# gkm2708/gym-lmaze

Measured on AMD Instinct MI355X. Metric: env steps/sec (whole node), 1M parallel 11x11 mazes at 1/2/4/8 MI355X, higher is better.
Workload: dtype int32

## Files before the change

### gym-lmaze_amd/_abi.py

```python
import ctypes as C
import os

import torch

HERE = os.path.dirname(os.path.abspath(__file__))
LIB_PATH = os.environ.get("LMAZE_HIP_LIB") or os.path.join(HERE, "liblmaze_hip.so")

ABI_VERSION = 4
VARIANT_V0, VARIANT_V3 = 0, 3
VARIANT_V1, VARIANT_V2, VARIANT_V4, VARIANT_V5, VARIANT_V6 = 1, 2, 4, 5, 6
FOVEA = 5
LAYOUT_SHARED, LAYOUT_PER_ENV = 0, 1
OBS_BALL, OBS_WALL, OBS_GOAL, OBS_FREE = 1, 2, 4, 8
MAX_GRID, MAX_CHANNELS = 64, 8

SYMBOLS = ("lmaze_abi_version", "lmaze_strerror", "lmaze_device_info", "lmaze_step_v0", "lmaze_step_v3",
           "lmaze_step_v0_autoreset", "lmaze_step_v3_autoreset", "lmaze_observe", "lmaze_reset",
           "lmaze_episode_stats", "lmaze_bandwidth_probe", "lmaze_render_expanded", "lmaze_foveal_step", "lmaze_foveal_step_autoreset", "lmaze_foveal_reset", "lmaze_v1_set_foveal_goal",
           "lmaze_v5_planner_step", "lmaze_v5_hier_step", "lmaze_v6_safe_foveal_goal", "lmaze_expand_planes",
           "lmaze_foveal_visit_bytes", "lmaze_foveal_materialise_visit", "lmaze_foveal_load_visit",
           "lmaze_describe_step", "lmaze_describe_foveal_step", "lmaze_rollout",
           "lmaze_step_u8", "lmaze_observe_u8", "lmaze_foveal_rollout", "lmaze_describe_foveal_rollout",
           "lmaze_rollout_obs", "lmaze_foveal_rollout_obs", "lmaze_rollout_u8", "lmaze_rollout_obs_u8",
           "lmaze_describe_rollout", "lmaze_rollout_policy", "lmaze_rollout_policy_u8", "lmaze_describe_rollout_policy",
           "lmaze_rollout_sample", "lmaze_rollout_sample_u8", "lmaze_describe_rollout_sample", "lmaze_returns",
           "lmaze_describe_foveal_rollout_obs")


class LmazeParams(C.Structure):
    _fields_ = [("variant", C.c_int32), ("grid", C.c_int32), ("layout_mode", C.c_int32),
                ("step_limit", C.c_int32), ("reward_wall", C.c_float), ("reward_move", C.c_float),
                ("reward_goal", C.c_float), ("launch_hint", C.c_int32)]


class LmazeFovealParams(C.Structure):
    _fields_ = [("variant", C.c_int32), ("grid", C.c_int32), ("n_layouts", C.c_int32), ("step_limit", C.c_int32),
                ("foveal_step_limit", C.c_int32), ("reward_wall", C.c_float), ("reward_move", C.c_float),
                ("reward_goal", C.c_float), ("launch_hint", C.c_int32)]


FOVEAL_BUFFER_FIELDS = ("ball_xy", "goal_xy", "fgoal_xy", "layout_id", "step_count", "foveal_step_count",
                        "reward", "foveal_reward", "done", "foveal_done", "visit", "obs",
                        "ball1_xy", "fovea_xy", "last_xy", "foveal_goal", "obs_local", "visit_clock")


class LmazeFovealBuffers(C.Structure):
    _fields_ = [(n, C.c_void_p) for n in FOVEAL_BUFFER_FIELDS]


class LmazeError(RuntimeError):
    def __init__(self, fn, code):
        self.code = code
        RuntimeError.__init__(self, "%s failed: %d (%s)" % (fn, code, strerror(code)))


def _sources():
    src = os.path.join(HERE, "csrc")
    out = [os.path.join(src, f) for f in sorted(os.listdir(src)) if f.endswith((".hip", ".h"))] if os.path.isdir(src) else []
    hdr = os.path.join(os.path.dirname(HERE), "include", "lmaze.h")
    return out + ([hdr] if os.path.exists(hdr) else [])


def _load():
    if not os.path.exists(LIB_PATH):
        raise ImportError(
            "gym-lmaze_amd: %s is missing. The HIP library is the only compute path (no CPU fallback); "
            "build it with `make -C %s` (hipcc, --offload-arch=gfx950) or `python -c 'import __graft_entry__ as g; "
            "g.build()'`." % (LIB_PATH, os.path.join(HERE, "csrc")))
    if "LMAZE_HIP_LIB" not in os.environ:
        stale = [f for f in _sources() if os.path.getmtime(f) > os.path.getmtime(LIB_PATH)]
        if stale:
            import warnings
            warnings.warn("gym-lmaze_amd: %s is older than %s -- rebuild with `make -C %s`"
                          % (os.path.basename(LIB_PATH), ", ".join(os.path.basename(f) for f in stale),
                             os.path.join(HERE, "csrc")), RuntimeWarning, stacklevel=3)
    lib = C.CDLL(LIB_PATH)
    vp, i32, i64, u64 = C.c_void_p, C.c_int32, C.c_int64, C.c_uint64
    P = C.POINTER(LmazeParams)
    lib.lmaze_abi_version.restype = C.c_int
    lib.lmaze_abi_version.argtypes = []
    lib.lmaze_strerror.restype = C.c_char_p
    lib.lmaze_strerror.argtypes = [C.c_int]
    lib.lmaze_device_info.restype = C.c_int
    lib.lmaze_device_info.argtypes = [C.c_int, C.POINTER(i32), C.c_char_p, i32]
    lib.lmaze_step_v0.restype = C.c_int
    lib.lmaze_step_v0.argtypes = [P, vp, vp, vp, vp, vp, vp, vp, vp, i64, vp]
    lib.lmaze_step_v3.restype = C.c_int
    lib.lmaze_step_v3.argtypes = [P, vp, vp, vp, vp, vp, vp, vp, vp, i64, vp]
    lib.lmaze_step_v0_autoreset.restype = C.c_int
    lib.lmaze_step_v0_autoreset.argtypes = [P, vp, vp, vp, vp, vp, vp, vp, vp, i64, u64, u64, i64, vp, vp, vp]
    lib.lmaze_step_v3_autoreset.restype = C.c_int
    lib.lmaze_step_v3_autoreset.argtypes = [P, vp, vp, vp, vp, vp, vp, vp, vp, i64, u64, u64, i64, vp, vp, vp]
    lib.lmaze_observe.restype = C.c_int
    lib.lmaze_observe.argtypes = [P, vp, vp, vp, vp, i64, vp]
    lib.lmaze_reset.restype = C.c_int
    lib.lmaze_reset.argtypes = [P, vp, vp, u64, u64, i64, vp, vp, vp, vp, vp, vp, i64, vp]
    lib.lmaze_render_expanded.restype = C.c_int
    lib.lmaze_render_expanded.argtypes = [vp, i32, i32, C.POINTER(i32), i32, vp, i64, vp]
    lib.lmaze_bandwidth_probe.restype = C.c_int
    lib.lmaze_bandwidth_probe.argtypes = [vp, vp, i64, vp]
    lib.lmaze_episode_stats.restype = C.c_int
    lib.lmaze_episode_stats.argtypes = [vp, vp, vp, vp, C.c_float, i64, vp, vp]
    FP, FB = C.POINTER(LmazeFovealParams), C.POINTER(LmazeFovealBuffers)
    lib.lmaze_foveal_step.restype = C.c_int
    lib.lmaze_foveal_step.argtypes = [FP, vp, vp, FB, i64, vp]
    lib.lmaze_foveal_step_autoreset.restype = C.c_int
    lib.lmaze_foveal_step_autoreset.argtypes = [FP, vp, vp, FB, i64, u64, u64, i64, vp, vp, vp]
    lib.lmaze_foveal_reset.restype = C.c_int
    lib.lmaze_foveal_reset.argtypes = [FP, vp, vp, i32, u64, u64, i64, FB, i64, vp]
    lib.lmaze_v1_set_foveal_goal.restype = C.c_int
    lib.lmaze_v1_set_foveal_goal.argtypes = [FP, vp, vp, vp, FB, i64, vp]
    lib.lmaze_v5_planner_step.restype = C.c_int
    lib.lmaze_v5_planner_step.argtypes = [FP, vp, vp, vp, FB, i64, vp]
    lib.lmaze_v5_hier_step.restype = C.c_int
    lib.lmaze_v5_hier_step.argtypes = [FP, vp, vp, vp, FB, i64, u64, u64, i64, vp, vp, vp]
    lib.lmaze_v6_safe_foveal_goal.restype = C.c_int
    lib.lmaze_v6_safe_foveal_goal.argtypes = [FP, vp, u64, u64, i64, FB, vp, i64, vp]
    lib.lmaze_expand_planes.restype = C.c_int
    lib.lmaze_expand_planes.argtypes = [vp, i32, i32, i32, vp, i64, vp]
    lib.lmaze_foveal_visit_bytes.restype = i64
    lib.lmaze_foveal_visit_bytes.argtypes = [i32, i64]
    lib.lmaze_foveal_materialise_visit.restype = C.c_int
    lib.lmaze_foveal_materialise_visit.argtypes = [FP, FB, vp, i64, vp]
    lib.lmaze_foveal_load_visit.restype = C.c_int
    lib.lmaze_foveal_load_visit.argtypes = [FP, FB, vp, i64, vp]
    lib.lmaze_step_u8.restype = C.c_int
    lib.lmaze_step_u8.argtypes = [P, vp, vp, vp, vp, vp, vp, vp, vp, vp, i64, i32, u64, u64, i64, vp, vp, vp]
    lib.lmaze_observe_u8.restype = C.c_int
    lib.lmaze_observe_u8.argtypes = [P, vp, vp, vp, vp, vp, i64, vp]
    lib.lmaze_rollout.restype = C.c_int
    lib.lmaze_rollout.argtypes = [P, vp, vp, i32, vp, vp, vp, vp, vp, vp, vp, vp, vp, i64, i32, u64, u64, i64, vp]
    lib.lmaze_describe_step.restype = C.c_int
    lib.lmaze_describe_step.argtypes = [P, i64, i32, i32, C.c_char_p, i32]
    lib.lmaze_describe_foveal_step.restype = C.c_int
    lib.lmaze_describe_foveal_step.argtypes = [FP, i64, i32, C.c_char_p, i32]
    lib.lmaze_foveal_rollout.restype = C.c_int
    lib.lmaze_foveal_rollout.argtypes = [FP, vp, vp, vp, i32, FB, i64, i32, u64, u64, i64, vp, vp, vp, vp, vp]
    lib.lmaze_rollout_obs.restype = C.c_int
    lib.lmaze_rollout_obs.argtypes = [P, vp, vp, i32, vp, vp, vp, vp, vp, vp, vp, vp, vp, i64, i32, u64, u64, i64, vp, i32, vp]
    lib.lmaze_foveal_rollout_obs.restype = C.c_int
    lib.lmaze_foveal_rollout_obs.argtypes = [FP, vp, vp, vp, i32, FB, i64, i32, u64, u64, i64, vp, vp, vp, vp, vp, vp, i32, vp]
    lib.lmaze_rollout_u8.restype = C.c_int
    lib.lmaze_rollout_u8.argtypes = [P, vp, vp, i32, vp, vp, vp, vp, vp, vp, vp, vp, vp, i64, i32, u64, u64, i64, vp]
    lib.lmaze_rollout_obs_u8.restype = C.c_int
    lib.lmaze_rollout_obs_u8.argtypes = [P, vp, vp, i32, vp, vp, vp, vp, vp, vp, vp, vp, vp, i64, i32, u64, u64, i64, vp, i32, vp]
    lib.lmaze_describe_rollout.restype = C.c_int
    lib.lmaze_describe_rollout.argtypes = [P, i64, i32, i32, i32, i32, C.c_char_p, i32]
    for name in ("lmaze_rollout_policy", "lmaze_rollout_policy_u8"):
        getattr(lib, name).restype = C.c_int
        getattr(lib, name).argtypes = [P, vp, vp, i32, C.c_uint32, i32, vp, vp, vp, vp, vp, vp, vp, vp, vp, vp, vp, i64, i32, u64, u64,
                                       i64, vp, i32, vp]
    lib.lmaze_describe_rollout_policy.restype = C.c_int
    lib.lmaze_describe_rollout_policy.argtypes = [P, i64, i32, i32, i32, i32, i32, C.c_char_p, i32]
    for name in ("lmaze_rollout_sample", "lmaze_rollout_sample_u8"):
        getattr(lib, name).restype = C.c_int
        getattr(lib, name).argtypes = [P, vp, vp, i32, i32, vp, vp, vp, vp, vp, vp, vp, vp, vp, vp, vp, i64, i32, u64, u64, i64, vp, i32, vp]
    lib.lmaze_describe_rollout_sample.restype = C.c_int
    lib.lmaze_describe_rollout_sample.argtypes = [P, i64, i32, i32, i32, i32, i32, C.c_char_p, i32]
    lib.lmaze_returns.restype = C.c_int
    lib.lmaze_returns.argtypes = [vp, vp, vp, C.c_float, vp, i32, i64, vp]
    lib.lmaze_describe_foveal_rollout.restype = C.c_int
    lib.lmaze_describe_foveal_rollout.argtypes = [FP, i64, i32, i32, i32, C.c_char_p, i32]
    lib.lmaze_describe_foveal_rollout_obs.restype = C.c_int
    lib.lmaze_describe_foveal_rollout_obs.argtypes = [FP, i64, i32, i32, i32, i32, C.c_char_p, i32]
    if lib.lmaze_abi_version() != ABI_VERSION:
        raise ImportError("liblmaze_hip.so ABI %d != binding %d: rebuild" % (lib.lmaze_abi_version(), ABI_VERSION))
    return lib


lib = _load()


def strerror(code):
    return lib.lmaze_strerror(int(code)).decode("ascii", "replace")


def check(fn, code):
    if code != 0:
        raise LmazeError(fn, code)


def device_info(device=0):
    cu = C.c_int32(0)
    name = C.create_string_buffer(64)
    check("lmaze_device_info", lib.lmaze_device_info(int(device), C.byref(cu), name, 64))
    return {"cu_count": cu.value, "arch": name.value.decode("ascii", "replace")}


def describe_step(params, n, auto_reset=False, with_obs=True):
    buf = C.create_string_buffer(256)
    check("lmaze_describe_step", lib.lmaze_describe_step(C.byref(params), int(n), 1 if auto_reset else 0,
                                                         2 if with_obs == "u8" else (1 if with_obs else 0), buf, 256))
    return buf.value.decode("ascii", "replace")


def describe_rollout(params, n, T, auto_reset=False, with_obs=True, obs_every=None):
    buf = C.create_string_buffer(256)
    check("lmaze_describe_rollout", lib.lmaze_describe_rollout(C.byref(params), int(n), int(T), 1 if auto_reset else 0,
                                                               2 if with_obs == "u8" else (1 if with_obs else 0),
                                                               -1 if obs_every is None else int(obs_every), buf, 256))
    return buf.value.decode("ascii", "replace")


def describe_foveal_step(params, n, auto_reset=False):
    buf = C.create_string_buffer(256)
    check("lmaze_describe_foveal_step", lib.lmaze_describe_foveal_step(C.byref(params), int(n), 1 if auto_reset else 0, buf, 256))
    return buf.value.decode("ascii", "replace")


KEY_MODES = {"ball": 0, "goal": 1}


def epsilon_u32(epsilon):
    eps = float(epsilon)
    if not 0.0 <= eps <= 1.0:
        raise ValueError("epsilon must be in [0, 1]")
    return min(int(eps * 4294967296.0), 4294967295)


def describe_rollout_policy(params, n, T, auto_reset=True, with_obs=True, obs_every=0, key="ball"):
    buf = C.create_string_buffer(256)
    check("lmaze_describe_rollout_policy",
          lib.lmaze_describe_rollout_policy(C.byref(params), int(n), int(T), 1 if auto_reset else 0,
                                            2 if with_obs == "u8" else (1 if with_obs else 0), int(obs_every),
                                            KEY_MODES[key] if key in KEY_MODES else int(key), buf, 256))
    return buf.value.decode("ascii", "replace")


def describe_rollout_sample(params, n, T, auto_reset=True, with_obs=True, obs_every=0, key="ball"):
    buf = C.create_string_buffer(256)
    check("lmaze_describe_rollout_sample",
          lib.lmaze_describe_rollout_sample(C.byref(params), int(n), int(T), 1 if auto_reset else 0,
                                            2 if with_obs == "u8" else (1 if with_obs else 0), int(obs_every),
                                            KEY_MODES[key] if key in KEY_MODES else int(key), buf, 256))
    return buf.value.decode("ascii", "replace")


def sampling_thresholds(probs):
    if not (isinstance(probs, torch.Tensor) and probs.dim() == 2 and probs.shape[1] == 4 and probs.is_floating_point()):
        raise ValueError("probs must be a float tensor [S, 4]")
    p = probs.detach().to(torch.float64)
    if not bool(torch.isfinite(p).all()) or bool((p < 0).any()):
        raise ValueError("probs must be finite and non-negative")
    a0 = p[:, 0]
    a1 = a0 + p[:, 1]
    a2 = a1 + p[:, 2]
    s = a2 + p[:, 3]
    if not bool(torch.isfinite(s).all()) or bool((s <= 0).any()):
        raise ValueError("every row of probs must have a positive, finite sum")
    c = torch.stack([torch.floor(a / s * 4294967296.0 + 0.5) for a in (a0, a1, a2)] + [torch.zeros_like(s)], dim=1)
    c = c.clamp_(max=4294967295.0).to(torch.int64)
    return torch.where(c >= 2147483648, c - 4294967296, c).to(torch.int32).view(torch.uint32)


def describe_foveal_rollout(params, n, T, auto_reset=False, two_level=False, obs_every=None):
    buf = C.create_string_buffer(256)
    if obs_every is None:
        check("lmaze_describe_foveal_rollout", lib.lmaze_describe_foveal_rollout(C.byref(params), int(n), int(T),
                                                                                 1 if auto_reset else 0, 1 if two_level else 0,
                                                                                 buf, 256))
    else:
        check("lmaze_describe_foveal_rollout_obs",
              lib.lmaze_describe_foveal_rollout_obs(C.byref(params), int(n), int(T), 1 if auto_reset else 0,
                                                    1 if two_level else 0, int(obs_every), buf, 256))
    return buf.value.decode("ascii", "replace")


def make_params(variant, grid, layout_mode, step_limit, reward_wall, reward_move, reward_goal):
    return LmazeParams(int(variant), int(grid), int(layout_mode), int(step_limit), float(reward_wall),
                       float(reward_move), float(reward_goal), 0)
```

### gym-lmaze_amd/csrc/lmaze_abi.hip

```cpp
#include <stdio.h>
#include <string.h>

#include "lmaze_common.h"


using namespace lmaze;

static int check_params(const LmazeParams* p, int64_t n) {
    if (!p) return LMAZE_E_NULL;
    if (p->grid < 3 || p->grid > LMAZE_MAX_GRID) return LMAZE_E_GRID;
    if (p->layout_mode != LMAZE_LAYOUT_SHARED && p->layout_mode != LMAZE_LAYOUT_PER_ENV) return LMAZE_E_LAYOUT;
    if (n < 0 || n > LMAZE_MAX_ENVS) return LMAZE_E_COUNT;
    return 0;
}

static bool misaligned(const void* p, uintptr_t a) { return ((uintptr_t)p & (a - 1)) != 0; }

static StepArgs make_args(const LmazeParams* p, const uint8_t* layout, const int32_t* action, int32_t* ball_xy,
                          const int32_t* goal_xy, int32_t* step_count, float* reward, uint8_t* done,
                          int32_t* goal_count, int32_t* obs, int64_t n) {
    StepArgs a;
    a.layout = layout;
    a.action = action;
    a.ball = reinterpret_cast<int2*>(ball_xy);
    a.goal = reinterpret_cast<const int2*>(goal_xy);
    a.step_count = step_count;
    a.reward = reward;
    a.done = done;
    a.goal_count = goal_count;
    a.obs = obs;
    a.obs8 = nullptr;
    a.n = n;
    a.grid = p->grid;
    a.step_limit = p->step_limit;
    a.reward_wall = p->reward_wall;
    a.reward_move = p->reward_move;
    a.reward_goal = p->reward_goal;
    a.envs_per_block = 0;
    a.auto_reset = 0;
    a.seed = 0;
    a.epoch = 0;
    a.env_base = 0;
    a.epoch_in = nullptr;
    a.epoch_out = nullptr;
    a.goal_rw = nullptr;
    a.mask = nullptr;
    a.launch_hint = p->launch_hint;
    a.info = nullptr;
    return a;
}

namespace lmaze {
void describe_launch(LaunchInfo* info, const char* kernel, int epb, int per_cu, int chunks, bool nt, int64_t grid, int block, size_t lds) {
    snprintf(info->kernel, sizeof(info->kernel), "%s", kernel);
    info->envs_per_workgroup = epb;
    info->workgroups_per_cu = per_cu;
    info->chunks = chunks;
    info->non_temporal = nt ? 1 : 0;
    info->grid = grid;
    info->block = block;
    info->lds = (int64_t)lds;
}
}

static int format_launch(const LaunchInfo& i, char* text, int32_t len) {
    if (!text || len < 1) return LMAZE_E_NULL;
    snprintf(text, (size_t)len, "%s grid=%lld block=%d lds=%lld envs_per_workgroup=%d workgroups_per_cu=%d chunks=%d", i.kernel,
             (long long)i.grid, i.block, (long long)i.lds, i.envs_per_workgroup, i.workgroups_per_cu, i.chunks);
    return 0;
}

static int check_recording(int32_t T, const void* slots, int32_t every) {
    if (every < 0 || (every == 0 && slots)) return LMAZE_E_COUNT;
    if (every > 0 && T / every > 0 && !slots) return LMAZE_E_NULL;
    if (misaligned(slots, 16)) return LMAZE_E_ALIGN;
    return 0;
}

static RolloutRec recording(int32_t T, void* slots, int32_t every) {
    return RolloutRec{every > 0 && T / every > 0 ? slots : nullptr, every};
}

static StepArgs rollout_args(const LmazeParams* p, const uint8_t* layout, const int32_t* actions, int32_t* ball_xy, int32_t* goal_xy,
                             int32_t* step_count, float* reward, uint8_t* done, int32_t* goal_count, void* obs, bool u8, int64_t n,
                             int32_t auto_reset, uint64_t seed, uint64_t epoch, int64_t env_base) {
    const bool v3 = p->variant == LMAZE_VARIANT_V3;
    StepArgs a = make_args(p, layout, actions, ball_xy, v3 ? goal_xy : nullptr, step_count, reward, done, v3 ? nullptr : goal_count,
                           u8 ? nullptr : static_cast<int32_t*>(obs), n);
    a.obs8 = u8 ? static_cast<uint8_t*>(obs) : nullptr;
    a.auto_reset = auto_reset ? 1 : 0;
    a.seed = seed;
    a.epoch = epoch;
    a.env_base = env_base;
    a.goal_rw = v3 ? reinterpret_cast<int2*>(goal_xy) : nullptr;
    return a;
}

static int grid_rollout(const LmazeParams* params, const uint8_t* layout, const int32_t* actions, int32_t T, int32_t* ball_xy,
                        int32_t* goal_xy, int32_t* step_count, float* reward, uint8_t* done, int32_t* goal_count, void* obs, bool u8,
                        float* reward_t, uint8_t* done_t, int64_t n, int32_t auto_reset, uint64_t seed, uint64_t epoch,
                        int64_t env_base, const RolloutRec* rec, void* stream) {
    int rc = check_params(params, n);
    if (rc) return rc;
    const bool v3 = params->variant == LMAZE_VARIANT_V3;
    if (params->variant != LMAZE_VARIANT_V0 && !v3) return LMAZE_E_VARIANT;
    if (u8 && params->layout_mode != LMAZE_LAYOUT_SHARED) return LMAZE_E_LAYOUT;
    if (u8 && params->grid < 4) return LMAZE_E_GRID;
    if (T < 0) return LMAZE_E_COUNT;
    if (T == 0 || n == 0) return 0;
    if (!layout || !actions || !ball_xy || !step_count || !reward || !done || (v3 && !goal_xy)) return LMAZE_E_NULL;
    if (misaligned(ball_xy, 8) || misaligned(goal_xy, 8) || misaligned(obs, 16) || (!u8 && misaligned(layout, 16))) return LMAZE_E_ALIGN;
    const StepArgs a = rollout_args(params, layout, actions, ball_xy, goal_xy, step_count, reward, done, goal_count, obs, u8, n,
                                    auto_reset, seed, epoch, env_base);
    return (int)launch_rollout(params->variant, a, params->layout_mode, actions, T, reward_t, done_t, (hipStream_t)stream, rec, u8);
}

static int check_closed_loop(const LmazeParams* params, const uint8_t* layout, const void* table, uintptr_t table_align,
                             int32_t key_mode, int32_t T, const int32_t* ball_xy, const int32_t* goal_xy, const int32_t* step_count,
                             const float* reward, const uint8_t* done, const void* obs, bool u8, int64_t n, bool describing, bool* go) {
    *go = false;
    int rc = check_params(params, n);
    if (rc) return rc;
    const bool v3 = params->variant == LMAZE_VARIANT_V3;
    if (params->variant != LMAZE_VARIANT_V0 && !v3) return LMAZE_E_VARIANT;
    if (u8 && params->layout_mode != LMAZE_LAYOUT_SHARED) return LMAZE_E_LAYOUT;
    if (u8 && params->grid < 4) return LMAZE_E_GRID;
    if (T < 0) return LMAZE_E_COUNT;
    if (key_mode != 0 && key_mode != 1) return LMAZE_E_COUNT;
    if (key_mode == 1 && !v3) return LMAZE_E_VARIANT;
    if (T == 0 || n == 0) return 0;
    if (!describing) {
        if (!layout || !table || !ball_xy || !step_count || !reward || !done || (v3 && !goal_xy)) return LMAZE_E_NULL;
        if (misaligned(ball_xy, 8) || misaligned(goal_xy, 8) || misaligned(obs, 16) || (!u8 && misaligned(layout, 16)) ||
            misaligned(table, table_align))
            return LMAZE_E_ALIGN;
    }
    *go = true;
    return 0;
}

static int grid_rollout_policy(const LmazeParams* params, const uint8_t* layout, const RolloutPolicy& pol, int32_t T, int32_t* ball_xy,
                               int32_t* goal_xy, int32_t* step_count, float* reward, uint8_t* done, int32_t* goal_count, void* obs,
                               bool u8, float* reward_t, uint8_t* done_t, int64_t n, int32_t auto_reset, uint64_t seed,
                               uint64_t epoch, int64_t env_base, const RolloutRec& rec, LaunchInfo* info, void* stream) {
    bool go;
    const int rc = check_closed_loop(params, layout, pol.table, 1, pol.key_mode, T, ball_xy, goal_xy, step_count, reward, done, obs, u8,
                                     n, info != nullptr, &go);
    if (!go) return rc;
    StepArgs a = rollout_args(params, layout, nullptr, ball_xy, goal_xy, step_count, reward, done, goal_count, obs, u8, n, auto_reset,
                              seed, epoch, env_base);
    a.info = info;
    return (int)launch_rollout_policy(params->variant, a, params->layout_mode, pol, T, reward_t, done_t, (hipStream_t)stream, rec, u8);
}

static int grid_rollout_sample(const LmazeParams* params, const uint8_t* layout, const RolloutSample& smp, int32_t T, int32_t* ball_xy,
                               int32_t* goal_xy, int32_t* step_count, float* reward, uint8_t* done, int32_t* goal_count, void* obs,
                               bool u8, float* reward_t, uint8_t* done_t, int64_t n, int32_t auto_reset, uint64_t seed,
                               uint64_t epoch, int64_t env_base, const RolloutRec& rec, LaunchInfo* info, void* stream) {
    bool go;
    const int rc = check_closed_loop(params, layout, smp.thresholds, 16, smp.key_mode, T, ball_xy, goal_xy, step_count, reward, done, obs,
                                     u8, n, info != nullptr, &go);
    if (!go) return rc;
    StepArgs a = rollout_args(params, layout, nullptr, ball_xy, goal_xy, step_count, reward, done, goal_count, obs, u8, n, auto_reset,
                              seed, epoch, env_base);
    a.info = info;
    return (int)launch_rollout_sample(params->variant, a, params->layout_mode, smp, T, reward_t, done_t, (hipStream_t)stream, rec, u8);
}

extern "C" {

int lmaze_abi_version(void) { return LMAZE_ABI_VERSION; }

const char* lmaze_strerror(int code) {
    switch (code) {
        case 0: return "ok";
        case LMAZE_E_NULL: return "a required pointer is NULL";
        case LMAZE_E_GRID: return "grid outside [3, 64]";
        case LMAZE_E_VARIANT: return "params.variant does not match the entry point";
        case LMAZE_E_LAYOUT: return "unknown layout_mode";
        case LMAZE_E_COUNT: return "env count out of range";
        case LMAZE_E_ALIGN: return "buffer not aligned as documented";
        case LMAZE_E_EXPANSION: return "expansion ratio / channel count out of range";
        case LMAZE_E_NODEVICE: return "no usable HIP device";
        default: return code > 0 ? hipGetErrorString((hipError_t)code) : "unknown lmaze error";
    }
}

int lmaze_device_info(int device, int32_t* cu_count_host, char* name_host, int32_t name_len) {
    int count = 0;
    if (hipGetDeviceCount(&count) != hipSuccess || count <= 0 || device < 0 || device >= count) {
        (void)hipGetLastError();
        return LMAZE_E_NODEVICE;
    }
    hipDeviceProp_t prop;
    if (hipGetDeviceProperties(&prop, device) != hipSuccess) return LMAZE_E_NODEVICE;
    if (cu_count_host) *cu_count_host = prop.multiProcessorCount;
    if (name_host && name_len > 0) {
        strncpy(name_host, prop.gcnArchName, (size_t)name_len - 1);
        name_host[name_len - 1] = 0;
    }
    return 0;
}

int lmaze_describe_step(const LmazeParams* params, int64_t n, int32_t auto_reset, int32_t with_obs, char* text_host,
                        int32_t len) {
    int rc = check_params(params, n);
    if (rc) return rc;
    if (params->variant != LMAZE_VARIANT_V0 && params->variant != LMAZE_VARIANT_V3) return LMAZE_E_VARIANT;
    if (!text_host || len < 1) return LMAZE_E_NULL;
    text_host[0] = 0;
    if (n == 0) return 0;
    LaunchInfo info;
    memset(&info, 0, sizeof(info));
    StepArgs a = make_args(params, nullptr, nullptr, nullptr, nullptr, nullptr, nullptr, nullptr, nullptr,
                           with_obs ? reinterpret_cast<int32_t*>(16) : nullptr, n);
    a.auto_reset = auto_reset ? 1 : 0;
    a.info = &info;
    if (with_obs == 2) {
        if (params->layout_mode != LMAZE_LAYOUT_SHARED) return LMAZE_E_LAYOUT;
        if (params->grid < 4) return LMAZE_E_GRID;
        a.obs = nullptr;
        a.obs8 = reinterpret_cast<uint8_t*>(16);
        rc = (int)launch_step_u8(params->variant, true, a, nullptr);
        if (rc) return rc;
        return format_launch(info, text_host, len);
    }
    rc = (int)launch_step(params->variant, true, a, params->layout_mode, nullptr);
    if (rc) return rc;
    return format_launch(info, text_host, len);
}

int lmaze_step_v0(const LmazeParams* params, const uint8_t* layout, const int32_t* action, int32_t* ball_xy,
                  int32_t* step_count, float* reward, uint8_t* done, int32_t* goal_count, int32_t* obs,
                  int64_t n, void* stream) {
    int rc = check_params(params, n);
    if (rc) return rc;
    if (params->variant != LMAZE_VARIANT_V0) return LMAZE_E_VARIANT;
    if (!layout || !action || !ball_xy || !step_count || !reward || !done) return LMAZE_E_NULL;
    if (misaligned(ball_xy, 8) || misaligned(obs, 16) || misaligned(layout, 16)) return LMAZE_E_ALIGN;
    StepArgs a = make_args(params, layout, action, ball_xy, nullptr, step_count, reward, done, goal_count, obs, n);
    return (int)launch_step(LMAZE_VARIANT_V0, true, a, params->layout_mode, (hipStream_t)stream);
}

int lmaze_step_v3(const LmazeParams* params, const uint8_t* layout, const int32_t* action, int32_t* ball_xy,
                  const int32_t* goal_xy, int32_t* step_count, float* reward, uint8_t* done, int32_t* obs,
                  int64_t n, void* stream) {
    int rc = check_params(params, n);
    if (rc) return rc;
    if (params->variant != LMAZE_VARIANT_V3) return LMAZE_E_VARIANT;
    if (!layout || !action || !ball_xy || !goal_xy || !step_count || !reward || !done) return LMAZE_E_NULL;
    if (misaligned(ball_xy, 8) || misaligned(goal_xy, 8) || misaligned(obs, 16) || misaligned(layout, 16))
        return LMAZE_E_ALIGN;
    StepArgs a = make_args(params, layout, action, ball_xy, goal_xy, step_count, reward, done, nullptr, obs, n);
    return (int)launch_step(LMAZE_VARIANT_V3, true, a, params->layout_mode, (hipStream_t)stream);
}

int lmaze_step_v0_autoreset(const LmazeParams* params, const uint8_t* layout, const int32_t* action,
                            int32_t* ball_xy, int32_t* step_count, float* reward, uint8_t* done,
                            int32_t* goal_count, int32_t* obs, int64_t n, uint64_t seed, uint64_t epoch,
                            int64_t env_base, const uint64_t* epoch_in_dev, uint64_t* epoch_out_dev, void* stream) {
    int rc = check_params(params, n);
    if (rc) return rc;
    if (params->variant != LMAZE_VARIANT_V0) return LMAZE_E_VARIANT;
    if (!layout || !action || !ball_xy || !step_count || !reward || !done) return LMAZE_E_NULL;
    if (misaligned(ball_xy, 8) || misaligned(obs, 16) || misaligned(layout, 16)) return LMAZE_E_ALIGN;
    StepArgs a = make_args(params, layout, action, ball_xy, nullptr, step_count, reward, done, goal_count, obs, n);
    if (bad_epoch_words(epoch_in_dev, epoch_out_dev)) return LMAZE_E_ALIGN;
    a.auto_reset = 1;
    a.seed = seed;
    a.epoch = epoch;
    a.env_base = env_base;
    a.epoch_in = epoch_in_dev;
    a.epoch_out = epoch_out_dev;
    return (int)launch_step(LMAZE_VARIANT_V0, true, a, params->layout_mode, (hipStream_t)stream);
}

int lmaze_step_u8(const LmazeParams* params, const uint8_t* layout, const int32_t* action, int32_t* ball_xy, int32_t* goal_xy,
                  int32_t* step_count, float* reward, uint8_t* done, int32_t* goal_count, uint8_t* obs8, int64_t n,
                  int32_t auto_reset, uint64_t seed, uint64_t epoch, int64_t env_base, const uint64_t* epoch_in_dev,
                  uint64_t* epoch_out_dev, void* stream) {
    int rc = check_params(params, n);
    if (rc) return rc;
    const bool v3 = params->variant == LMAZE_VARIANT_V3;
    if (params->variant != LMAZE_VARIANT_V0 && !v3) return LMAZE_E_VARIANT;
    if (params->layout_mode != LMAZE_LAYOUT_SHARED) return LMAZE_E_LAYOUT;
    if (params->grid < 4) return LMAZE_E_GRID;
    if (!layout || !action || !ball_xy || !step_count || !reward || !done || (v3 && !goal_xy)) return LMAZE_E_NULL;
    if (misaligned(ball_xy, 8) || misaligned(goal_xy, 8) || misaligned(obs8, 16)) return LMAZE_E_ALIGN;
    if (bad_epoch_words(epoch_in_dev, epoch_out_dev)) return LMAZE_E_ALIGN;
    StepArgs a = make_args(params, layout, action, ball_xy, v3 ? goal_xy : nullptr, step_count, reward, done, v3 ? nullptr : goal_count, nullptr, n);
    a.obs8 = obs8;
    a.auto_reset = auto_reset ? 1 : 0;
    a.seed = seed;
    a.epoch = epoch;
    a.env_base = env_base;
    a.epoch_in = epoch_in_dev;
    a.epoch_out = epoch_out_dev;
    a.goal_rw = v3 ? reinterpret_cast<int2*>(goal_xy) : nullptr;
    return (int)launch_step_u8(params->variant, true, a, (hipStream_t)stream);
}

int lmaze_observe_u8(const LmazeParams* params, const uint8_t* layout, const int32_t* ball_xy, const int32_t* goal_xy,
                     const uint8_t* mask, uint8_t* obs8, int64_t n, void* stream) {
    int rc = check_params(params, n);
    if (rc) return rc;
    const bool v3 = params->variant == LMAZE_VARIANT_V3;
    if (params->variant != LMAZE_VARIANT_V0 && !v3) return LMAZE_E_VARIANT;
    if (params->layout_mode != LMAZE_LAYOUT_SHARED) return LMAZE_E_LAYOUT;
    if (params->grid < 4) return LMAZE_E_GRID;
    if (!layout || !ball_xy || !obs8 || (v3 && !goal_xy)) return LMAZE_E_NULL;
    if (misaligned(ball_xy, 8) || misaligned(goal_xy, 8) || misaligned(obs8, 16)) return LMAZE_E_ALIGN;
    StepArgs a = make_args(params, layout, nullptr, const_cast<int32_t*>(ball_xy), v3 ? goal_xy : nullptr, nullptr, nullptr, nullptr,
                           nullptr, nullptr, n);
    a.obs8 = obs8;
    a.mask = mask;
    return (int)launch_step_u8(params->variant, false, a, (hipStream_t)stream);
}

int lmaze_rollout(const LmazeParams* params, const uint8_t* layout, const int32_t* actions, int32_t T, int32_t* ball_xy,
                  int32_t* goal_xy, int32_t* step_count, float* reward, uint8_t* done, int32_t* goal_count, int32_t* obs,
                  float* reward_t, uint8_t* done_t, int64_t n, int32_t auto_reset, uint64_t seed, uint64_t epoch,
                  int64_t env_base, void* stream) {
    return grid_rollout(params, layout, actions, T, ball_xy, goal_xy, step_count, reward, done, goal_count, obs, false, reward_t,
                        done_t, n, auto_reset, seed, epoch, env_base, nullptr, stream);
}

int lmaze_rollout_obs(const LmazeParams* params, const uint8_t* layout, const int32_t* actions, int32_t T, int32_t* ball_xy,
                      int32_t* goal_xy, int32_t* step_count, float* reward, uint8_t* done, int32_t* goal_count, int32_t* obs,
                      float* reward_t, uint8_t* done_t, int64_t n, int32_t auto_reset, uint64_t seed, uint64_t epoch,
                      int64_t env_base, int32_t* obs_t, int32_t obs_every, void* stream) {
    const int rc = check_recording(T, obs_t, obs_every);
    const RolloutRec rec = recording(T, obs_t, obs_every);
    return rc ? rc : grid_rollout(params, layout, actions, T, ball_xy, goal_xy, step_count, reward, done, goal_count, obs, false,
                                  reward_t, done_t, n, auto_reset, seed, epoch, env_base, &rec, stream);
}

int lmaze_rollout_u8(const LmazeParams* params, const uint8_t* layout, const int32_t* actions, int32_t T, int32_t* ball_xy,
                     int32_t* goal_xy, int32_t* step_count, float* reward, uint8_t* done, int32_t* goal_count, uint8_t* obs8,
                     float* reward_t, uint8_t* done_t, int64_t n, int32_t auto_reset, uint64_t seed, uint64_t epoch,
                     int64_t env_base, void* stream) {
    return grid_rollout(params, layout, actions, T, ball_xy, goal_xy, step_count, reward, done, goal_count, obs8, true, reward_t,
                        done_t, n, auto_reset, seed, epoch, env_base, nullptr, stream);
}

int lmaze_rollout_obs_u8(const LmazeParams* params, const uint8_t* layout, const int32_t* actions, int32_t T, int32_t* ball_xy,
                         int32_t* goal_xy, int32_t* step_count, float* reward, uint8_t* done, int32_t* goal_count, uint8_t* obs8,
                         float* reward_t, uint8_t* done_t, int64_t n, int32_t auto_reset, uint64_t seed, uint64_t epoch,
                         int64_t env_base, uint8_t* obs_t8, int32_t obs_every, void* stream) {
    const int rc = check_recording(T, obs_t8, obs_every);
    const RolloutRec rec = recording(T, obs_t8, obs_every);
    return rc ? rc : grid_rollout(params, layout, actions, T, ball_xy, goal_xy, step_count, reward, done, goal_count, obs8, true,
                                  reward_t, done_t, n, auto_reset, seed, epoch, env_base, &rec, stream);
}

int lmaze_rollout_policy(const LmazeParams* params, const uint8_t* layout, const uint8_t* policy, int32_t key_mode,
                         uint32_t epsilon_u32, int32_t T, int32_t* ball_xy, int32_t* goal_xy, int32_t* step_count, float* reward,
                         uint8_t* done, int32_t* goal_count, int32_t* obs, float* reward_t, uint8_t* done_t, int32_t* actions_t,
                         int32_t* key_t, int64_t n, int32_t auto_reset, uint64_t seed, uint64_t epoch, int64_t env_base,
                         int32_t* obs_t, int32_t obs_every, void* stream) {
    const int rc = check_recording(T, obs_t, obs_every);
    const RolloutPolicy pol{policy, key_mode, epsilon_u32, actions_t, key_t};
    return rc ? rc : grid_rollout_policy(params, layout, pol, T, ball_xy, goal_xy, step_count, reward, done, goal_count, obs, false,
                                         reward_t, done_t, n, auto_reset, seed, epoch, env_base, recording(T, obs_t, obs_every),
                                         nullptr, stream);
}

int lmaze_rollout_policy_u8(const LmazeParams* params, const uint8_t* layout, const uint8_t* policy, int32_t key_mode,
                            uint32_t epsilon_u32, int32_t T, int32_t* ball_xy, int32_t* goal_xy, int32_t* step_count, float* reward,
                            uint8_t* done, int32_t* goal_count, uint8_t* obs8, float* reward_t, uint8_t* done_t, int32_t* actions_t,
                            int32_t* key_t, int64_t n, int32_t auto_reset, uint64_t seed, uint64_t epoch, int64_t env_base,
                            uint8_t* obs_t8, int32_t obs_every, void* stream) {
    const int rc = check_recording(T, obs_t8, obs_every);
    const RolloutPolicy pol{policy, key_mode, epsilon_u32, actions_t, key_t};
    return rc ? rc : grid_rollout_policy(params, layout, pol, T, ball_xy, goal_xy, step_count, reward, done, goal_count, obs8, true,
                                         reward_t, done_t, n, auto_reset, seed, epoch, env_base, recording(T, obs_t8, obs_every),
                                         nullptr, stream);
}

int lmaze_describe_rollout_policy(const LmazeParams* params, int64_t n, int32_t T, int32_t auto_reset, int32_t with_obs,
                                  int32_t obs_every, int32_t key_mode, char* text_host, int32_t len) {
    if (obs_every < 0) return LMAZE_E_COUNT;
    if (!text_host || len < 1) return LMAZE_E_NULL;
    text_host[0] = 0;
    const bool u8 = with_obs == 2;
    LaunchInfo info;
    memset(&info, 0, sizeof(info));
    const RolloutPolicy pol{nullptr, key_mode, 0, nullptr, nullptr};
    const int rc = grid_rollout_policy(params, nullptr, pol, T, nullptr, nullptr, nullptr, nullptr, nullptr, nullptr,
                                       with_obs == 1 || u8 ? reinterpret_cast<void*>(16) : nullptr, u8, nullptr, nullptr, n, auto_reset,
                                       0, 0, 0, recording(T, reinterpret_cast<void*>(32), obs_every), &info, nullptr);
    if (rc || n == 0 || T == 0) return rc;
    return format_launch(info, text_host, len);
}

int lmaze_rollout_sample(const LmazeParams* params, const uint8_t* layout, const uint32_t* thresholds, int32_t key_mode, int32_t T,
                         int32_t* ball_xy, int32_t* goal_xy, int32_t* step_count, float* reward, uint8_t* done, int32_t* goal_count,
                         int32_t* obs, float* reward_t, uint8_t* done_t, int32_t* actions_t, int32_t* key_t, int64_t n,
                         int32_t auto_reset, uint64_t seed, uint64_t epoch, int64_t env_base, int32_t* obs_t, int32_t obs_every,
                         void* stream) {
    const int rc = check_recording(T, obs_t, obs_every);
    const RolloutSample smp{thresholds, key_mode, actions_t, key_t};
    return rc ? rc : grid_rollout_sample(params, layout, smp, T, ball_xy, goal_xy, step_count, reward, done, goal_count, obs, false,
                                         reward_t, done_t, n, auto_reset, seed, epoch, env_base, recording(T, obs_t, obs_every),
                                         nullptr, stream);
}

int lmaze_rollout_sample_u8(const LmazeParams* params, const uint8_t* layout, const uint32_t* thresholds, int32_t key_mode, int32_t T,
                            int32_t* ball_xy, int32_t* goal_xy, int32_t* step_count, float* reward, uint8_t* done,
                            int32_t* goal_count, uint8_t* obs8, float* reward_t, uint8_t* done_t, int32_t* actions_t, int32_t* key_t,
                            int64_t n, int32_t auto_reset, uint64_t seed, uint64_t epoch, int64_t env_base, uint8_t* obs_t8,
                            int32_t obs_every, void* stream) {
    const int rc = check_recording(T, obs_t8, obs_every);
    const RolloutSample smp{thresholds, key_mode, actions_t, key_t};
    return rc ? rc : grid_rollout_sample(params, layout, smp, T, ball_xy, goal_xy, step_count, reward, done, goal_count, obs8, true,
                                         reward_t, done_t, n, auto_reset, seed, epoch, env_base, recording(T, obs_t8, obs_every),
                                         nullptr, stream);
}

int lmaze_describe_rollout_sample(const LmazeParams* params, int64_t n, int32_t T, int32_t auto_reset, int32_t with_obs,
                                  int32_t obs_every, int32_t key_mode, char* text_host, int32_t len) {
    if (obs_every < 0) return LMAZE_E_COUNT;
    if (!text_host || len < 1) return LMAZE_E_NULL;
    text_host[0] = 0;
    const bool u8 = with_obs == 2;
    LaunchInfo info;
    memset(&info, 0, sizeof(info));
    const RolloutSample smp{nullptr, key_mode, nullptr, nullptr};
    const int rc = grid_rollout_sample(params, nullptr, smp, T, nullptr, nullptr, nullptr, nullptr, nullptr, nullptr,
                                       with_obs == 1 || u8 ? reinterpret_cast<void*>(16) : nullptr, u8, nullptr, nullptr, n, auto_reset,
                                       0, 0, 0, recording(T, reinterpret_cast<void*>(32), obs_every), &info, nullptr);
    if (rc || n == 0 || T == 0) return rc;
    return format_launch(info, text_host, len);
}

int lmaze_returns(const float* reward_t, const uint8_t* done_t, const float* tail, float gamma, float* returns_t, int32_t T,
                  int64_t n, void* stream) {
    if (!reward_t || !done_t || !returns_t) return LMAZE_E_NULL;
    if (T < 0 || n < 0 || n > LMAZE_MAX_ENVS) return LMAZE_E_COUNT;
    return (int)launch_returns(reward_t, done_t, tail, gamma, returns_t, T, n, (hipStream_t)stream);
}

int lmaze_describe_rollout(const LmazeParams* params, int64_t n, int32_t T, int32_t auto_reset, int32_t with_obs, int32_t obs_every,
                           char* text_host, int32_t len) {
    int rc = check_params(params, n);
    if (rc) return rc;
    if (params->variant != LMAZE_VARIANT_V0 && params->variant != LMAZE_VARIANT_V3) return LMAZE_E_VARIANT;
    if (T < 0) return LMAZE_E_COUNT;
    if (!text_host || len < 1) return LMAZE_E_NULL;
    text_host[0] = 0;
    if (n == 0 || T == 0) return 0;
    const bool u8 = with_obs == 2;
    if (u8 && params->layout_mode != LMAZE_LAYOUT_SHARED) return LMAZE_E_LAYOUT;
    if (u8 && params->grid < 4) return LMAZE_E_GRID;
    LaunchInfo info;
    memset(&info, 0, sizeof(info));
    StepArgs a = rollout_args(params, nullptr, nullptr, nullptr, nullptr, nullptr, nullptr, nullptr, nullptr,
                              with_obs == 1 || u8 ? reinterpret_cast<void*>(16) : nullptr, u8, n, auto_reset, 0, 0, 0);
    a.info = &info;
    const RolloutRec rec = recording(T, reinterpret_cast<void*>(32), obs_every);
    rc = (int)launch_rollout(params->variant, a, params->layout_mode, nullptr, T, nullptr, nullptr, nullptr,
                             obs_every >= 0 ? &rec : nullptr, u8);
    if (rc) return rc;
    return format_launch(info, text_host, len);
}

int lmaze_step_v3_autoreset(const LmazeParams* params, const uint8_t* layout, const int32_t* action,
                            int32_t* ball_xy, int32_t* goal_xy, int32_t* step_count, float* reward,
                            uint8_t* done, int32_t* obs, int64_t n, uint64_t seed, uint64_t epoch,
                            int64_t env_base, const uint64_t* epoch_in_dev, uint64_t* epoch_out_dev, void* stream) {
    int rc = check_params(params, n);
    if (rc) return rc;
    if (params->variant != LMAZE_VARIANT_V3) return LMAZE_E_VARIANT;
    if (!layout || !action || !ball_xy || !goal_xy || !step_count || !reward || !done) return LMAZE_E_NULL;
    if (misaligned(ball_xy, 8) || misaligned(goal_xy, 8) || misaligned(obs, 16) || misaligned(layout, 16))
        return LMAZE_E_ALIGN;
    StepArgs a = make_args(params, layout, action, ball_xy, goal_xy, step_count, reward, done, nullptr, obs, n);
    if (bad_epoch_words(epoch_in_dev, epoch_out_dev)) return LMAZE_E_ALIGN;
    a.auto_reset = 1;
    a.seed = seed;
    a.epoch = epoch;
    a.env_base = env_base;
    a.epoch_in = epoch_in_dev;
    a.epoch_out = epoch_out_dev;
    a.goal_rw = reinterpret_cast<int2*>(goal_xy);
    return (int)launch_step(LMAZE_VARIANT_V3, true, a, params->layout_mode, (hipStream_t)stream);
}

int lmaze_observe(const LmazeParams* params, const uint8_t* layout, const int32_t* ball_xy,
                  const int32_t* goal_xy, int32_t* obs, int64_t n, void* stream) {
    int rc = check_params(params, n);
    if (rc) return rc;
    if (params->variant != LMAZE_VARIANT_V0 && params->variant != LMAZE_VARIANT_V3) return LMAZE_E_VARIANT;
    if (!layout || !ball_xy || !obs) return LMAZE_E_NULL;
    if (params->variant == LMAZE_VARIANT_V3 && !goal_xy) return LMAZE_E_NULL;
    if (misaligned(ball_xy, 8) || misaligned(goal_xy, 8) || misaligned(obs, 16) || misaligned(layout, 16))
        return LMAZE_E_ALIGN;
    StepArgs a = make_args(params, layout, nullptr, const_cast<int32_t*>(ball_xy), goal_xy, nullptr, nullptr,
                           nullptr, nullptr, obs, n);
    return (int)launch_step(params->variant, false, a, params->layout_mode, (hipStream_t)stream);
}

int lmaze_reset(const LmazeParams* params, const uint8_t* layout, const uint8_t* mask, uint64_t seed,
                uint64_t epoch, int64_t env_base, int32_t* ball_xy, int32_t* goal_xy, int32_t* step_count, float* reward,
                uint8_t* done, int32_t* obs, int64_t n, void* stream) {
    int rc = check_params(params, n);
    if (rc) return rc;
    if (params->variant != LMAZE_VARIANT_V0 && params->variant != LMAZE_VARIANT_V3) return LMAZE_E_VARIANT;
    if (!layout || !ball_xy || !step_count || !reward || !done) return LMAZE_E_NULL;
    if (params->variant == LMAZE_VARIANT_V3 && !goal_xy) return LMAZE_E_NULL;
    if (misaligned(ball_xy, 8) || misaligned(goal_xy, 8) || misaligned(obs, 16) || misaligned(layout, 16))
        return LMAZE_E_ALIGN;
    ResetArgs r;
    r.layout = layout;
    r.mask = mask;
    r.ball = reinterpret_cast<int2*>(ball_xy);
    r.goal = reinterpret_cast<int2*>(goal_xy);
    r.step_count = step_count;
    r.reward = reward;
    r.done = done;
    r.n = n;
    r.seed = seed;
    r.epoch = epoch;
    r.env_base = env_base;
    r.grid = params->grid;
    hipError_t e = launch_reset(params->variant, r, params->layout_mode, (hipStream_t)stream);
    if (e != hipSuccess || !obs) return (int)e;
    StepArgs a = make_args(params, layout, nullptr, ball_xy, goal_xy, nullptr, nullptr, nullptr, nullptr, obs, n);
    a.mask = mask;
    return (int)launch_step(params->variant, false, a, params->layout_mode, (hipStream_t)stream);
}

int lmaze_episode_stats(const uint8_t* done, const float* reward, const int32_t* step_count,
                        const int32_t* goal_count, float reward_goal, int64_t n, int64_t* out4, void* stream) {
    if (!done || !reward || !step_count || !out4) return LMAZE_E_NULL;
    if (n < 0 || n > LMAZE_MAX_ENVS) return LMAZE_E_COUNT;
    if (misaligned(out4, 8)) return LMAZE_E_ALIGN;
    return (int)launch_episode_stats(done, reward, step_count, goal_count, reward_goal, n, out4, (hipStream_t)stream);
}

int lmaze_bandwidth_probe(const void* src, void* dst, int64_t bytes, void* stream) {
    if (!dst) return LMAZE_E_NULL;
    if (bytes < 0 || bytes > ((int64_t)1 << 36) || (bytes & 15)) return LMAZE_E_COUNT;
    if (misaligned(dst, 16) || (src && misaligned(src, 16))) return LMAZE_E_ALIGN;
    return (int)launch_probe(src, dst, bytes, (hipStream_t)stream);
}

int lmaze_render_expanded(const int32_t* obs, int32_t grid, int32_t expansion, const int32_t* channel_mask_host,
                          int32_t channels, float* out, int64_t n, void* stream) {
    if (!obs || !channel_mask_host || !out) return LMAZE_E_NULL;
    if (grid < 1 || grid > LMAZE_MAX_GRID) return LMAZE_E_GRID;
    if (expansion < 1 || expansion > 16 || channels < 1 || channels > LMAZE_MAX_CHANNELS) return LMAZE_E_EXPANSION;
    if (n < 0 || n > LMAZE_MAX_ENVS) return LMAZE_E_COUNT;
    if (misaligned(out, 16) || misaligned(obs, 4)) return LMAZE_E_ALIGN;
    ExpandArgs a;
    a.obs = obs;
    a.out = out;
    a.n = n;
    a.grid = grid;
    a.expansion = expansion;
    a.channels = channels;
    a.chunk_floats = 0;
    a.inv_l = a.inv_cells = 0;
    for (int c = 0; c < LMAZE_MAX_CHANNELS; ++c) a.mask[c] = c < channels ? channel_mask_host[c] : 0;
    return (int)launch_expand(a, (hipStream_t)stream);
}

}
```

### gym-lmaze_amd/csrc/lmaze_common.h

```cpp
#ifndef LMAZE_COMMON_H_
#define LMAZE_COMMON_H_

#include <hip/hip_runtime.h>
#include <stdint.h>

#include "../../include/lmaze.h"

#define LMAZE_BLOCK 256

namespace lmaze {

template <int BITS = 0, typename V4>
__device__ __forceinline__ void stream_store16(V4* p, V4 t) {
    static_assert(sizeof(V4) == 16, "one dwordx4");
    if constexpr (BITS == 2) asm volatile("global_store_dwordx4 %0, %1, off sc0 sc1 nt" ::"v"(p), "v"(t));
    else __builtin_nontemporal_store(t, p);
}


struct LaunchInfo {
    char kernel[96];
    int32_t envs_per_workgroup, workgroups_per_cu, chunks, non_temporal, block;
    int64_t grid, lds;
};
void describe_launch(LaunchInfo* info, const char* kernel, int epb, int per_cu, int chunks, bool nt, int64_t grid, int block, size_t lds);

struct StepArgs {
    const uint8_t* layout;
    const int32_t* action;
    int2* ball;
    const int2* goal;
    int32_t* step_count;
    float* reward;
    uint8_t* done;
    int32_t* goal_count;
    int32_t* obs;
    uint8_t* obs8;
    int64_t n;
    int32_t grid;
    int32_t step_limit;
    float reward_wall, reward_move, reward_goal;
    int32_t envs_per_block;
    int32_t auto_reset;
    uint64_t seed, epoch;
    int64_t env_base;
    const uint64_t* epoch_in;
    uint64_t* epoch_out;
    int2* goal_rw;
    const uint8_t* mask;
    int32_t launch_hint;
    LaunchInfo* info;
};

struct ResetArgs {
    const uint8_t* layout;
    const uint8_t* mask;
    int2* ball;
    int2* goal;
    int32_t* step_count;
    float* reward;
    uint8_t* done;
    int64_t n;
    uint64_t seed, epoch;
    int64_t env_base;
    int32_t grid;
};

struct ExpandArgs {
    const int32_t* obs;
    float* out;
    int64_t n;
    int32_t grid, expansion, channels;
    int32_t mask[LMAZE_MAX_CHANNELS];
    int32_t chunk_floats;
    uint64_t inv_l, inv_cells;
};

inline bool bad_epoch_words(const uint64_t* in, const uint64_t* out) {
    return ((((uintptr_t)in) | ((uintptr_t)out)) & 7) != 0 || (in && in == out) || (!in && out);
}

inline bool grid_ok(int64_t blocks) { return blocks >= 1 && blocks <= (int64_t)0xFFFFFF; }

hipError_t launch_step(int variant, bool do_step, const StepArgs& a, int layout_mode, hipStream_t s);
hipError_t launch_step_u8(int variant, bool do_step, const StepArgs& a, hipStream_t s);
struct RolloutRec {
    void* obs_t;
    int32_t every;
};
hipError_t launch_rollout(int variant, const StepArgs& a, int layout_mode, const int32_t* actions, int32_t T, float* reward_t,
                          uint8_t* done_t, hipStream_t s, const RolloutRec* rec, bool u8);
struct RolloutPolicy {
    const uint8_t* table;
    int32_t key_mode;
    uint32_t epsilon;
    int32_t* actions_t;
    int32_t* key_t;
};
hipError_t launch_rollout_policy(int variant, const StepArgs& a, int layout_mode, const RolloutPolicy& pol, int32_t T,
                                 float* reward_t, uint8_t* done_t, hipStream_t s, const RolloutRec& rec, bool u8);
struct RolloutSample {
    const uint32_t* thresholds;
    int32_t key_mode;
    int32_t* actions_t;
    int32_t* key_t;
};
hipError_t launch_rollout_sample(int variant, const StepArgs& a, int layout_mode, const RolloutSample& smp, int32_t T,
                                 float* reward_t, uint8_t* done_t, hipStream_t s, const RolloutRec& rec, bool u8);
hipError_t launch_returns(const float* reward_t, const uint8_t* done_t, const float* tail, float gamma, float* returns_t,
                          int32_t T, int64_t n, hipStream_t s);
hipError_t launch_reset(int variant, const ResetArgs& a, int layout_mode, hipStream_t s);
hipError_t launch_expand(const ExpandArgs& a, hipStream_t s);
hipError_t launch_probe(const void* src, void* dst, int64_t bytes, hipStream_t s);
hipError_t launch_episode_stats(const uint8_t* done, const float* reward, const int32_t* step_count,
                                const int32_t* goal_count, float reward_goal, int64_t n, int64_t* out4, hipStream_t s);

template <int VARIANT>
__device__ __forceinline__ int cell_bits(uint8_t c) {
    if (VARIANT == LMAZE_VARIANT_V3) {
        return c == 'W' ? LMAZE_OBS_WALL : ((c == 'B' || c == 'S' || c == 'X') ? LMAZE_OBS_FREE : 0);
    }
    return c == 'W' ? LMAZE_OBS_WALL : (c == 'X' ? LMAZE_OBS_GOAL : (c == 'B' ? LMAZE_OBS_FREE : 0));
}

__device__ __forceinline__ void decode_action(int a, int& ox, int& oy) {
    ox = (a == 1) - (a == 0);
    oy = (a == 3) - (a == 2);
}

__device__ __forceinline__ int clampi(int v, int lo, int hi) { return v < lo ? lo : (v > hi ? hi : v); }

template <int VARIANT>
__device__ __forceinline__ bool transition_rule(const StepArgs& a, uint8_t c, int ox, int oy, int tx, int ty, int sc,
                                                float r_in, int gx, int gy, int& bx, int& by, float& r, bool& dn) {
    bool hit = false;
    if (VARIANT == LMAZE_VARIANT_V3) {
        r = -0.0f;
        if (c == 'W') {
            r = a.reward_wall;
        } else {
            bx = tx; by = ty;
            r = (bx + ox == gx && by + oy == gy) ? a.reward_goal : a.reward_move;
        }
        dn = (r == a.reward_goal) || (sc > a.step_limit);
    } else {
        r = r_in;
        if (c == 'W') {
            r = a.reward_wall;
        } else if (c == 'B') {
            bx = tx; by = ty;
            r = a.reward_move;
        } else if (c == 'X') {
            bx = tx; by = ty;
            r = a.reward_goal;
            hit = true;
        }
        dn = (r == a.reward_goal) || (sc == a.step_limit);
    }
    return hit;
}

__device__ __forceinline__ uint4 philox4x32_10(uint4 c, uint2 k) {
#pragma unroll
    for (int r = 0; r < 10; ++r) {
        const uint32_t hi0 = __umulhi(0xD2511F53u, c.x), lo0 = 0xD2511F53u * c.x;
        const uint32_t hi1 = __umulhi(0xCD9E8D57u, c.z), lo1 = 0xCD9E8D57u * c.z;
        c = make_uint4(hi1 ^ c.y ^ k.x, lo1, hi0 ^ c.w ^ k.y, lo0);
        k.x += 0x9E3779B9u;
        k.y += 0xBB67AE85u;
    }
    return c;
}

__device__ __forceinline__ int warm_lines(const void* p, int64_t bytes, int blocks) {
    int acc = 0;
    if (p == nullptr || (int)blockIdx.x >= blocks) return 0;
    const uintptr_t lo = reinterpret_cast<uintptr_t>(p) & ~(uintptr_t)3;
    const int64_t dwords = (int64_t)((reinterpret_cast<uintptr_t>(p) + (uintptr_t)bytes - lo) / 4);
    if (dwords < 1) return 0;
    const int64_t lines = (dwords + 15) / 16;
    const int* q = reinterpret_cast<const int*>(lo);
    for (int64_t l = (int64_t)blockIdx.x * blockDim.x + threadIdx.x; l < lines; l += (int64_t)blocks * blockDim.x)
        acc += q[min(l * 16, dwords - 1)];
    return acc;
}

__device__ __forceinline__ uint64_t launch_epoch(uint64_t epoch, const uint64_t* epoch_in) {
    return epoch_in ? epoch + *epoch_in : epoch;
}

__device__ __forceinline__ void pass_epoch_on(const uint64_t* epoch_in, uint64_t* epoch_out) {
    if (epoch_in && epoch_out && blockIdx.x == 0 && threadIdx.x == 0) *epoch_out = *epoch_in + 1;
}

__device__ __forceinline__ uint4 env_draw(uint64_t seed, uint64_t epoch, int64_t env_global) {
    const uint64_t e = (uint64_t)env_global;
    return philox4x32_10(make_uint4((uint32_t)e, (uint32_t)(e >> 32), (uint32_t)epoch, (uint32_t)(epoch >> 32)),
                         make_uint2((uint32_t)seed, (uint32_t)(seed >> 32)));
}

template <int VARIANT>
__device__ __forceinline__ bool spawn_ok(uint8_t c) {
    return VARIANT == LMAZE_VARIANT_V3 ? (c != 'W') : (c != 'W' && c != 'X');
}

__device__ __forceinline__ bool interior(int cell, int G) {
    const int x = cell / G, y = cell - x * G;
    return x >= 1 && x <= G - 2 && y >= 1 && y <= G - 2;
}

template <int VARIANT>
__device__ __forceinline__ int wave_build_spawn_list(const uint8_t* lay, int G, int CELLS, uint16_t* list, int lane) {
    int count = 0;
    for (int base = 0; base < CELLS; base += 64) {
        const int cell = base + lane;
        const bool ok = cell < CELLS && interior(cell, G) && spawn_ok<VARIANT>(lay[cell]);
        const unsigned long long m = __ballot(ok);
        if (ok) list[count + __popcll(m & ((1ull << lane) - 1ull))] = (uint16_t)cell;
        count += __popcll(m);
    }
    return count;
}

template <int VARIANT>
__device__ __forceinline__ void place_from_list(const uint16_t* list, int count, uint4 r, int& ball_cell, int& goal_cell) {
    ball_cell = -1;
    goal_cell = -1;
    if (VARIANT == LMAZE_VARIANT_V3) {
        int kg = -1;
        if (count > 0) {
            kg = (int)__umulhi(r.x, (uint32_t)count);
            goal_cell = list[kg];
        }
        if (count > 1) {
            int kb = (int)__umulhi(r.y, (uint32_t)(count - 1));
            kb += (kb >= kg);
            ball_cell = list[kb];
        }
    } else if (count > 0) {
        ball_cell = list[__umulhi(r.y, (uint32_t)count)];
    }
}

__device__ __forceinline__ int kth_set_bit(unsigned long long m, int k) {
    int pos = 0;
#pragma unroll
    for (int sh = 32; sh > 0; sh >>= 1) {
        const unsigned long long low = m & ((1ull << sh) - 1ull);
        const int c = __popcll(low);
        if (k >= c) { k -= c; m >>= sh; pos += sh; } else { m = low; }
    }
    return pos;
}

template <int NS>
__device__ __forceinline__ int kth_cell_of_masks(const unsigned long long (&m)[NS], int k) {
    unsigned long long sel = m[0];
    int base = 0;
    bool found = false;
#pragma unroll
    for (int j = 0; j < NS; ++j) {
        const int c = __popcll(m[j]);
        if (!found) {
            if (k < c) { sel = m[j]; base = j * 64; found = true; }
            else k -= c;
        }
    }
    return found ? base + kth_set_bit(sel, k) : -1;
}

template <int VARIANT, int NS>
__device__ __forceinline__ void place_from_masks(const unsigned long long (&m)[NS], int count, uint4 r, int& ball_cell, int& goal_cell) {
    ball_cell = -1;
    goal_cell = -1;
    if (VARIANT == LMAZE_VARIANT_V3) {
        int kg = -1;
        if (count > 0) {
            kg = (int)__umulhi(r.x, (uint32_t)count);
            goal_cell = kth_cell_of_masks<NS>(m, kg);
        }
        if (count > 1) {
            int kb = (int)__umulhi(r.y, (uint32_t)(count - 1));
            kb += (kb >= kg);
            ball_cell = kth_cell_of_masks<NS>(m, kb);
        }
    } else if (count > 0) {
        ball_cell = kth_cell_of_masks<NS>(m, (int)__umulhi(r.y, (uint32_t)count));
    }
}

template <int VARIANT>
__device__ __forceinline__ int wave_kth_cell(const uint8_t* lay, int G, int CELLS, int k, int lane) {
    int seen = 0, found = -1;
    for (int base = 0; base < CELLS; base += 64) {
        const int cell = base + lane;
        const bool ok = cell < CELLS && interior(cell, G) && spawn_ok<VARIANT>(lay[cell]);
        const unsigned long long m = __ballot(ok);
        const int rank = seen + __popcll(m & ((1ull << lane) - 1ull));
        const unsigned long long hit = __ballot(ok && rank == k);
        if (hit) found = base + __ffsll((long long)hit) - 1;
        seen += __popcll(m);
    }
    return found;
}

template <int VARIANT>
__device__ __forceinline__ int wave_count_cells(const uint8_t* lay, int G, int CELLS, int lane) {
    int count = 0;
    for (int base = 0; base < CELLS; base += 64) {
        const int cell = base + lane;
        const bool ok = cell < CELLS && interior(cell, G) && spawn_ok<VARIANT>(lay[cell]);
        count += __popcll(__ballot(ok));
    }
    return count;
}

template <int VARIANT>
__device__ __forceinline__ void wave_place(const uint8_t* lay, int G, int CELLS, uint4 r, int lane,
                                           int& ball_cell, int& goal_cell) {
    ball_cell = -1;
    goal_cell = -1;
    const int count = wave_count_cells<VARIANT>(lay, G, CELLS, lane);
    if (VARIANT == LMAZE_VARIANT_V3) {
        int kg = -1;
        if (count > 0) {
            kg = (int)__umulhi(r.x, (uint32_t)count);
            goal_cell = wave_kth_cell<VARIANT>(lay, G, CELLS, kg, lane);
        }
        if (count > 1) {
            int kb = (int)__umulhi(r.y, (uint32_t)(count - 1));
            kb += (kb >= kg);
            ball_cell = wave_kth_cell<VARIANT>(lay, G, CELLS, kb, lane);
        }
    } else if (count > 0) {
        ball_cell = wave_kth_cell<VARIANT>(lay, G, CELLS, (int)__umulhi(r.y, (uint32_t)count), lane);
    }
}

template <int VARIANT, int G, int NJ>
__device__ __forceinline__ void lane_spawn_masks(const uint32_t (&w)[NJ], int lane, uint32_t (&ok)[NJ]) {
#pragma unroll
    for (int j = 0; j < NJ; ++j) {
        uint32_t m = 0;
#pragma unroll
        for (int q = 0; q < 4; ++q) {
            const int cell = ((j * 64 + lane) << 2) + q;
            const int x = cell / G, y = cell - x * G;
            const bool in = x >= 1 && x <= G - 2 && y >= 1 && y <= G - 2;
            m |= (uint32_t)(in && spawn_ok<VARIANT>((uint8_t)(w[j] >> (8 * q)))) << q;
        }
        ok[j] = m;
    }
}

__device__ __forceinline__ int wave_sum(int v) {
#pragma unroll
    for (int off = 32; off > 0; off >>= 1) v += __shfl_xor(v, off, 64);
    return v;
}

template <int NJ>
__device__ __forceinline__ int wave_kth_from_masks(const uint32_t (&ok)[NJ], int k, int lane) {
    int running = 0;
#pragma unroll
    for (int j = 0; j < NJ; ++j) {
        const int c = __popc(ok[j]);
        int incl = c;
#pragma unroll
        for (int off = 1; off < 64; off <<= 1) {
            const int up = __shfl_up(incl, off, 64);
            if (lane >= off) incl += up;
        }
        const int total = __shfl(incl, 63, 64);
        if (k < running + total) {
            const int excl = incl - c;
            const bool mine = k >= running + excl && k < running + incl;
            int r = k - running - excl, cell = -1;
            if (mine) {
                uint32_t m = ok[j];
                for (; r > 0; --r) m &= m - 1;
                cell = ((j * 64 + lane) << 2) + (__ffs((int)m) - 1);
            }
            const unsigned long long who = __ballot(mine);
            return __shfl(cell, __ffsll((long long)who) - 1, 64);
        }
        running += total;
    }
    return -1;
}

template <int VARIANT, int G, int NJ>
__device__ __forceinline__ void wave_place_regs(const uint32_t (&w)[NJ], uint4 r, int lane, int& ball_cell, int& goal_cell) {
    uint32_t ok[NJ];
    lane_spawn_masks<VARIANT, G, NJ>(w, lane, ok);
    int cnt = 0;
#pragma unroll
    for (int j = 0; j < NJ; ++j) cnt += __popc(ok[j]);
    const int count = wave_sum(cnt);
    ball_cell = -1;
    goal_cell = -1;
    if (VARIANT == LMAZE_VARIANT_V3) {
        int kg = -1;
        if (count > 0) {
            kg = (int)__umulhi(r.x, (uint32_t)count);
            goal_cell = wave_kth_from_masks<NJ>(ok, kg, lane);
        }
        if (count > 1) {
            int kb = (int)__umulhi(r.y, (uint32_t)(count - 1));
            kb += (kb >= kg);
            ball_cell = wave_kth_from_masks<NJ>(ok, kb, lane);
        }
    } else if (count > 0) {
        ball_cell = wave_kth_from_masks<NJ>(ok, (int)__umulhi(r.y, (uint32_t)count), lane);
    }
}

__device__ __forceinline__ void or_at(int4& v, int d, int bit) {
    v.x |= (d == 0) ? bit : 0;
    v.y |= (d == 1) ? bit : 0;
    v.z |= (d == 2) ? bit : 0;
    v.w |= (d == 3) ? bit : 0;
}

}
#endif
```

### gym-lmaze_amd/csrc/lmaze_step.hip

```cpp
#include <cstdio>

#include <cmath>
#include <cstdlib>

#include "lmaze_common.h"
#include "lmaze_policy_table.h"

namespace lmaze {

static constexpr size_t kNonTemporalObsBytes = (size_t)192 << 20;

template <bool NT, int BITS = 0>
__device__ __forceinline__ void store16(int4* p, const int4& v) {
    typedef int v4i __attribute__((ext_vector_type(4)));
    if (NT) {
        v4i t = {v.x, v.y, v.z, v.w};
        stream_store16<BITS>(reinterpret_cast<v4i*>(p), t);
    } else {
        *p = v;
    }
}

__device__ __forceinline__ void count_goal(int32_t* p) { __hip_atomic_fetch_add(p, 1, __ATOMIC_RELAXED, __HIP_MEMORY_SCOPE_AGENT); }

// ... 211 lines not shown
                if (V3 && gc >= 0) atomicOr(&mk[NGW + gi + (gf >> 5)], 1u << (gf & 31));
            }
        }
        ballflat[le] = bf;
        if (V3) goalflat[le] = gf;
        if (masked) maskflag[le] = mf;
    }
    if (a.obs != nullptr) {
    __syncthreads();

    int32_t* obs = a.obs + (size_t)blockbase * CELLS;
    int4* obs4 = reinterpret_cast<int4*>(obs);
    const int R = nb * CELLS;
    const int nq = R >> 2;

    if (GT != 0) {
        const int V4G = PAT >> 2;
        const int4* pat4 = reinterpret_cast<const int4*>(pat);
        if (MARKS && has_next)
            for (int i = tid; i < NPL * NGW; i += LMAZE_BLOCK) marks[(buf ^ 1) * NPL * NGW + i] = 0u;
        for (int q = tid; q < nq; q += LMAZE_BLOCK) {
            const int grp = q / V4G;
            const int p = q - grp * V4G;
            int4 v = pat4[p];
            const int p4 = p << 2;
            if (masked) {
                if (GRP == 4) {
                    const int4 m = reinterpret_cast<const int4*>(maskflag)[grp];
                    if (!(m.x | m.y | m.z | m.w)) continue;
                } else if (!maskflag[grp]) {
                    continue;
                }
            }
            if (MARKS) {
                const int w = grp * WPG + (p4 >> 5), sh = p4 & 31;
                const uint32_t b4 = mk[w] >> sh, g4 = mk[NGW + w] >> sh;
                v.x |= (int)(b4 & 1u) * LMAZE_OBS_BALL | (int)(g4 & 1u) * LMAZE_OBS_GOAL;
                v.y |= (int)((b4 >> 1) & 1u) * LMAZE_OBS_BALL | (int)((g4 >> 1) & 1u) * LMAZE_OBS_GOAL;
                v.z |= (int)((b4 >> 2) & 1u) * LMAZE_OBS_BALL | (int)((g4 >> 2) & 1u) * LMAZE_OBS_GOAL;
                v.w |= (int)((b4 >> 3) & 1u) * LMAZE_OBS_BALL | (int)((g4 >> 3) & 1u) * LMAZE_OBS_GOAL;
            } else if (GRP == 4) {
                const int4 bf = reinterpret_cast<const int4*>(ballflat)[grp];
                or_at(v, bf.x - p4, LMAZE_OBS_BALL);
                or_at(v, bf.y - p4, LMAZE_OBS_BALL);
                or_at(v, bf.z - p4, LMAZE_OBS_BALL);
                or_at(v, bf.w - p4, LMAZE_OBS_BALL);
            } else {
                or_at(v, ballflat[grp] - p4, LMAZE_OBS_BALL);
            }
            store16<NT>(obs4 + q, v);
        }
    } else {
        for (int q = tid; q < nq; q += LMAZE_BLOCK) {
            const int f0 = q << 2;
            int le = f0 / CELLS;
            int c = f0 - le * CELLS;
            if (masked) {
                const int le1 = (f0 + 3) / CELLS;
                if (!(maskflag[le] | maskflag[le1 < EPB ? le1 : le])) continue;
            }
            int vals[4];
#pragma unroll
            for (int j = 0; j < 4; ++j) {
                int v = pat[c];
                v |= (ballflat[le] == c) ? LMAZE_OBS_BALL : 0;
                if (V3) v |= (goalflat[le] == c) ? LMAZE_OBS_GOAL : 0;
                vals[j] = v;
                if (++c == CELLS) { c = 0; ++le; }
            }
            store16<NT>(obs4 + q, make_int4(vals[0], vals[1], vals[2], vals[3]));
        }
    }
    const int f = (nq << 2) + tid;
    if (f < R) {
        const int le = f / CELLS;
        const int c = f - le * CELLS;
        const int off = (GT != 0) ? (le % GRP) * CELLS : 0;
        int v = pat[(GT != 0 && GRP > 1) ? off + c : c];
        v |= (ballflat[le] == off + c) ? LMAZE_OBS_BALL : 0;
        if (V3) v |= (goalflat[le] == off + c) ? LMAZE_OBS_GOAL : 0;
        if (!masked || maskflag[le]) obs[f] = v;
    }
    }
    if (!has_next) break;
    __syncthreads();
    chunk = next;
    blockbase = chunk * EPB;
    nb = nb_next;
    in = in_next;
    buf ^= 1;
  }
  if (warmed == 0x7fedcba9 && a.n < 0) a.done[0] = 1;
}

template <int GT, int VARIANT, bool DO_STEP>
__global__ __launch_bounds__(LMAZE_BLOCK) void step_perenv_kernel(const StepArgs a) {
    constexpr bool V3 = VARIANT == LMAZE_VARIANT_V3;
    const int G = GT ? GT : a.grid;
    const int CELLS = G * G;
    const int EPB = a.envs_per_block;

    extern __shared__ int4 lds4[];
    uint8_t* tile = reinterpret_cast<uint8_t*>(lds4);
    const int tile_bytes = (EPB * CELLS + 15) & ~15;
    int* ballcell = reinterpret_cast<int*>(tile + tile_bytes);
    int* goalcell = ballcell + EPB + 1;
    int* flag = goalcell + EPB + 1;
    int* newball = flag + EPB + 1;
    int* newgoal = newball + EPB;

    const int tid = threadIdx.x;
    const int64_t blockbase = (int64_t)blockIdx.x * EPB;
    const int nb = (int)min((int64_t)EPB, a.n - blockbase);
    const int R = nb * CELLS;
    const bool autoreset = DO_STEP && a.auto_reset;
    const bool masked = !DO_STEP && a.mask != nullptr;
    const uint64_t epoch = step_epoch(a, autoreset);

    EnvState s{};
    if (tid < nb) s = load_env<VARIANT, DO_STEP>(a, blockbase + tid);
    if (tid <= EPB) {
        int f = 0;
        if (tid < nb) {
            if (autoreset) f = s.done != 0;
            if (masked) f = a.mask[blockbase + tid] != 0;
        }
        flag[tid] = f;
    }
    const uint8_t* src = a.layout + (size_t)blockbase * CELLS;
    const int n16 = R >> 4;
    for (int i = tid; i < n16; i += LMAZE_BLOCK) lds4[i] = reinterpret_cast<const int4*>(src)[i];
    for (int i = (n16 << 4) + tid; i < R; i += LMAZE_BLOCK) tile[i] = src[i];
    __syncthreads();

    if (autoreset) {
        const int lane = tid & 63;
        for (int le = tid >> 6; le < nb; le += LMAZE_BLOCK / 64) {
            if (!flag[le]) continue;
            int bc, gc;
            wave_place<VARIANT>(tile + le * CELLS, G, CELLS, env_draw(a.seed, epoch, a.env_base + blockbase + le), lane,
                                bc, gc);
            if (lane == 0) { newball[le] = bc; newgoal[le] = gc; }
        }
        __syncthreads();
    }

    if (tid <= EPB) {
        int bcell = -8, gcell = -8;
        if (tid < nb) {
            const int64_t e = blockbase + tid;
            if (DO_STEP) {
                if (autoreset && flag[tid]) {
                    const int gc = newgoal[tid];
                    env_reset<VARIANT>(newball[tid], gc, G, s);
                    if (V3 && gc >= 0) a.goal_rw[e] = s.g;
                }
                if (env_advance<VARIANT>(a, G, [&](int tx, int ty) { return tile[tid * CELLS + tx * G + ty]; }, s) && a.goal_count)
                    count_goal(a.goal_count + e);
                store_state(a, e, s);
            } else {
                clamp_ball(s, G);
            }
            bcell = ball_cell_of(s.b, G);
            gcell = goal_cell_of<VARIANT>(s.g, G);
        }
        ballcell[tid] = bcell;
        if (V3) goalcell[tid] = gcell;
    }
    if (a.obs == nullptr) return;
    const bool stream = beyond_caches(a.n, CELLS);
    __syncthreads();

    int32_t* obs = a.obs + (size_t)blockbase * CELLS;
    int4* obs4 = reinterpret_cast<int4*>(obs);
    const int nq = R >> 2;
    const uint32_t* tile32 = reinterpret_cast<const uint32_t*>(tile);
    const bool whole = (CELLS & 3) == 0;
    for (int q = tid; q < nq; q += LMAZE_BLOCK) {
        const uint32_t w = tile32[q];
        const int f0 = q << 2;
        int le = f0 / CELLS;
        int c = f0 - le * CELLS;
        int vals[4];
        if (whole) {
            if (masked && !flag[le]) continue;
            const int bc = ballcell[le] - c;
            const int gc = V3 ? goalcell[le] - c : -8;
#pragma unroll
            for (int j = 0; j < 4; ++j) {
                int v = cell_bits<VARIANT>((uint8_t)(w >> (8 * j)));
                v |= (bc == j) ? LMAZE_OBS_BALL : 0;
                if (V3) v |= (gc == j) ? LMAZE_OBS_GOAL : 0;
                vals[j] = v;
            }
        } else {
            if (masked && !(flag[le] | flag[(f0 + 3) / CELLS])) continue;
#pragma unroll
            for (int j = 0; j < 4; ++j) {
                int v = cell_bits<VARIANT>((uint8_t)(w >> (8 * j)));
                v |= (ballcell[le] == c) ? LMAZE_OBS_BALL : 0;
                if (V3) v |= (goalcell[le] == c) ? LMAZE_OBS_GOAL : 0;
                vals[j] = v;
                if (++c == CELLS) { c = 0; ++le; }
            }
        }
        if (stream) store16<true>(obs4 + q, make_int4(vals[0], vals[1], vals[2], vals[3]));
        else obs4[q] = make_int4(vals[0], vals[1], vals[2], vals[3]);
    }
    const int f = (nq << 2) + tid;
    if (f < R) {
        const int le = f / CELLS;
        const int c = f - le * CELLS;
        int v = cell_bits<VARIANT>(tile[f]);
        v |= (ballcell[le] == c) ? LMAZE_OBS_BALL : 0;
        if (V3) v |= (goalcell[le] == c) ? LMAZE_OBS_GOAL : 0;
        if (!masked || flag[le]) obs[f] = v;
    }
}

template <int G, int VARIANT, bool DO_STEP, bool NT>
__global__ __launch_bounds__(LMAZE_BLOCK) void step_perenv_wave_kernel(const StepArgs a) {
    constexpr bool V3 = VARIANT == LMAZE_VARIANT_V3;
    constexpr int CELLS = G * G, NJ = CELLS / 256;
    static_assert(CELLS % 256 == 0, "whole dwords per lane");
    const int lane = threadIdx.x & 63;
    const int EPW = a.envs_per_block;
    const int64_t wave = (int64_t)blockIdx.x * (LMAZE_BLOCK / 64) + (threadIdx.x >> 6);
    const bool autoreset = DO_STEP && a.auto_reset;
    const bool masked = !DO_STEP && a.mask != nullptr;
    const uint64_t epoch = autoreset ? launch_epoch(a.epoch, a.epoch_in) : 0;
    if (autoreset) pass_epoch_on(a.epoch_in, a.epoch_out);

#pragma unroll 1
    for (int k = 0; k < EPW; ++k) {
        const int64_t e = wave * EPW + k;
        if (e >= a.n) break;
        if (masked && !a.mask[e]) continue;
        const uint32_t* lay32 = reinterpret_cast<const uint32_t*>(a.layout + (size_t)e * CELLS);
        uint32_t w[NJ];
#pragma unroll
        for (int j = 0; j < NJ; ++j) w[j] = lay32[j * 64 + lane];

        int2 b = a.ball[e];
        int2 g = make_int2(-1, -1);
        if (V3) g = a.goal[e];
        if (DO_STEP) {
            const int act = a.action[e];
            int sc_in = a.step_count[e];
            float r_in = V3 ? 0.0f : a.reward[e];
            if (autoreset && a.done[e]) {
                int bc, gc;
                wave_place_regs<VARIANT, G, NJ>(w, env_draw(a.seed, epoch, a.env_base + e), lane, bc, gc);
                if (bc >= 0) b = make_int2(bc / G, bc % G);
                if (V3 && gc >= 0) {
                    g = make_int2(gc / G, gc % G);
                    if (lane == 0) a.goal_rw[e] = g;
                }
                sc_in = 0;
                r_in = -0.0f;
            }
            int bx = clampi(b.x, 0, G - 1), by = clampi(b.y, 0, G - 1);
            int ox, oy;
            decode_action(act, ox, oy);
            const int tx = clampi(bx + ox, 0, G - 1), ty = clampi(by + oy, 0, G - 1);
            const int t = __builtin_amdgcn_readfirstlane(tx * G + ty);
            const int tw = t >> 2;
            uint32_t word = 0;
#pragma unroll
            for (int j = 0; j < NJ; ++j)
                if ((tw >> 6) == j) word = __builtin_amdgcn_readlane(w[j], tw & 63);
            const uint8_t c = (uint8_t)(word >> (8 * (t & 3)));
            float r;
            bool dn;
            const int sc = sc_in + 1;
            const bool hit = transition_rule<VARIANT>(a, c, ox, oy, tx, ty, sc, r_in, g.x, g.y, bx, by, r, dn);
            if (lane == 0) {
                if (hit && a.goal_count) count_goal(a.goal_count + e);
                a.ball[e] = make_int2(bx, by);
                a.step_count[e] = sc;
                a.reward[e] = r;
                a.done[e] = dn ? 1 : 0;
            }
            b = make_int2(bx, by);
        } else {
            b = make_int2(clampi(b.x, 0, G - 1), clampi(b.y, 0, G - 1));
        }
        if (a.obs == nullptr) continue;
        const int bcell = b.x * G + b.y;
        const int gcell = (V3 && g.x >= 0 && g.x < G && g.y >= 0 && g.y < G) ? g.x * G + g.y : -8;
        int4* obs4 = reinterpret_cast<int4*>(a.obs + (size_t)e * CELLS);
#pragma unroll
        for (int j = 0; j < NJ; ++j) {
            const int c0 = (j * 64 + lane) << 2;
            int vals[4];
#pragma unroll
            for (int q = 0; q < 4; ++q) {
                int v = cell_bits<VARIANT>((uint8_t)(w[j] >> (8 * q)));
                v |= (bcell == c0 + q) ? LMAZE_OBS_BALL : 0;
                if (V3) v |= (gcell == c0 + q) ? LMAZE_OBS_GOAL : 0;
                vals[q] = v;
            }
            store16<NT, 2>(obs4 + j * 64 + lane, make_int4(vals[0], vals[1], vals[2], vals[3]));
        }
    }
}


template <int VARIANT, bool DO_STEP, int EPW>
__global__ __launch_bounds__(LMAZE_BLOCK) void step_shared_wave8_kernel(const StepArgs a) {
    constexpr bool V3 = VARIANT == LMAZE_VARIANT_V3;
    constexpr int G = 8, CELLS = 64;
    const int lane = threadIdx.x & 63;
    const int64_t base = ((int64_t)blockIdx.x * (blockDim.x >> 6) + (threadIdx.x >> 6)) * EPW;
    if (base >= a.n) return;
    const int nb = (int)min((int64_t)EPW, a.n - base);
    const bool autoreset = DO_STEP && a.auto_reset;
    const uint64_t epoch = step_epoch(a, autoreset);
    const bool live = lane < nb;
    const int myc = a.layout[lane];
    EnvState s{};
    s.b = make_int2(1, 1); s.g = make_int2(-1, -1);
    if (live) s = load_env<VARIANT, DO_STEP>(a, base + lane);
    const int mypat = cell_bits<VARIANT>((uint8_t)myc);
    const int p4 = (lane & 15) << 2;
    const int4 pat4 = make_int4(__shfl(mypat, p4, 64), __shfl(mypat, p4 + 1, 64), __shfl(mypat, p4 + 2, 64),
                                __shfl(mypat, p4 + 3, 64));
    int4* obs4 = reinterpret_cast<int4*>(a.obs + (size_t)base * CELLS);
    if (DO_STEP) {
        if (autoreset) {
            const unsigned long long ok[1] = {__ballot(interior(lane, G) && spawn_ok<VARIANT>((uint8_t)myc))};
            if (s.done) {
                int bc, gc;
                place_from_masks<VARIANT, 1>(ok, __popcll(ok[0]), env_draw(a.seed, epoch, a.env_base + base + lane), bc, gc);
                env_reset<VARIANT>(bc, gc, G, s);
                if (V3 && gc >= 0 && live) a.goal_rw[base + lane] = s.g;
            }
        }
        const bool hit = env_advance<VARIANT>(a, G, [&](int tx, int ty) { return (uint8_t)__shfl(myc, tx * G + ty, 64); }, s);
        if (live) {
            const int64_t e = base + lane;
            if (hit && a.goal_count) count_goal(a.goal_count + e);
            store_state(a, e, s);
        }
    } else {
        clamp_ball(s, G);
    }
    if (a.obs == nullptr) return;
    const int ball_cell = ball_cell_of(s.b, G);
    const int goal_cell = goal_cell_of<VARIANT>(s.g, G);
#pragma unroll
    for (int k = 0; k < EPW / 4; ++k) {
        const int le = (lane >> 4) + 4 * k;
        const int bc = __shfl(ball_cell, le, 64);
        const int gc = V3 ? __shfl(goal_cell, le, 64) : -8;
        int4 v = pat4;
        or_at(v, bc - p4, LMAZE_OBS_BALL);
        if (V3) or_at(v, gc - p4, LMAZE_OBS_GOAL);
        if (le < nb) obs4[lane + 64 * k] = v;
    }
}

template <int VARIANT, bool DO_STEP, int EPB>
__global__ __launch_bounds__(LMAZE_BLOCK) void step_shared_u8_kernel(const StepArgs a) {
    constexpr bool V3 = VARIANT == LMAZE_VARIANT_V3;
    static_assert(EPB % 16 == 0 && EPB <= LMAZE_BLOCK, "a workgroup's byte range starts on a 16-byte boundary; one lane per env");
    const int G = a.grid, CELLS = G * G;
    const int PW = (2 * CELLS + 16 + 3) >> 2;
    extern __shared__ int4 lds4[];
    uint32_t* patw = reinterpret_cast<uint32_t*>(lds4);
    int* ballflat = reinterpret_cast<int*>(patw + 4 * PW);
    int* goalflat = ballflat + EPB + 1;
    int* maskflag = goalflat + EPB + 1;
    uint16_t* spawn = reinterpret_cast<uint16_t*>(maskflag + EPB + 1);
    uint8_t* lay = reinterpret_cast<uint8_t*>(spawn + ((CELLS + 1) & ~1));
    __shared__ int spawn_count_s;
    const int tid = threadIdx.x;
    const int64_t nchunks = (a.n + EPB - 1) / EPB;
    int64_t chunk = blockIdx.x;
    int64_t blockbase = chunk * EPB;
    int nb = (int)min((int64_t)EPB, a.n - blockbase);
    const bool masked = !DO_STEP && a.mask != nullptr;
    const bool autoreset = DO_STEP && a.auto_reset;
    const uint64_t epoch = step_epoch(a, autoreset);
    EnvState in{};
    if (tid < nb) in = load_env<VARIANT, DO_STEP>(a, blockbase + tid);
    int warmed = 0;
    if (DO_STEP && (a.launch_hint & 0x100)) {
        warmed = warm_lines(a.action, a.n * 4, 256) + warm_lines(a.ball, a.n * 8, 256) + warm_lines(a.step_count, a.n * 4, 256);
        if (!V3) warmed += warm_lines(a.reward, a.n * 4, 256);
        if (V3) warmed += warm_lines(a.goal, a.n * 8, 256);
        if (autoreset) warmed += warm_lines(a.done, a.n, 256);
    }
    for (int i = tid; i < CELLS; i += LMAZE_BLOCK) lay[i] = a.layout[i];
    __syncthreads();
    uint8_t* patb = reinterpret_cast<uint8_t*>(patw);
    for (int i = tid; i < 4 * PW; i += LMAZE_BLOCK) {
        const int s = i / PW, k = (i - s * PW) << 2;
        uint32_t w = 0;
#pragma unroll
        for (int j = 0; j < 4; ++j) {
            int c = k + s + j;
            c -= c >= CELLS ? CELLS : 0;
            c -= c >= CELLS ? CELLS : 0;
            c = min(c, CELLS - 1);
            w |= (uint32_t)cell_bits<VARIANT>(lay[c]) << (8 * j);
        }
        patw[i] = w;
    }
    if (autoreset && tid < 64) {
        const int cnt = wave_build_spawn_list<VARIANT>(lay, G, CELLS, spawn, tid);
        if (tid == 0) spawn_count_s = cnt;
    }
    if (tid == 0) { ballflat[EPB] = -64; goalflat[EPB] = -64; maskflag[EPB] = 0; }
    __syncthreads();
  for (;;) {
    const int64_t next = chunk + gridDim.x;
    const bool has_next = next < nchunks;
    EnvState in_next{};
    int nb_next = 0;
    if (has_next) {
        nb_next = (int)min((int64_t)EPB, a.n - next * EPB);
        if (tid < nb_next) in_next = load_env<VARIANT, DO_STEP>(a, next * EPB + tid);
    }
    if (tid < EPB) {
        int bf = -64, gf = -64, mf = 0;
        if (tid < nb) {
            const int64_t e = blockbase + tid;
            int bc, gc;
            const int cnt = autoreset ? spawn_count_s : 0;
            env_phase1<VARIANT, DO_STEP>(a, lay, G, e, in, [&](uint4 d, int& pb, int& pg) { place_from_list<VARIANT>(spawn, cnt, d, pb, pg); }, epoch, bc, gc);
            bf = bc;
            if (V3 && gc >= 0) gf = gc;
            if (masked) mf = a.mask[e] != 0;
        }
        ballflat[tid] = bf;
        goalflat[tid] = gf;
        maskflag[tid] = mf;
    }
    if (a.obs8 != nullptr) {
    __syncthreads();
    uint8_t* obs = a.obs8 + (size_t)blockbase * CELLS;
    const int R = nb * CELLS;
    if (!masked) {
        const int nq = R >> 4;
        for (int q = tid; q < nq; q += LMAZE_BLOCK) {
            const int f0 = q << 4;
            const int le = f0 / CELLS, c = f0 - le * CELLS;
            const int sft = c & 3;
            const uint32_t* src = patw + sft * PW + ((c - sft) >> 2);
            uint32_t w[4] = {src[0], src[1], src[2], src[3]};
            const int b0 = ballflat[le] - c, b1 = CELLS - c + ballflat[min(le + 1, EPB)];
            if ((unsigned)b0 < 16u) w[b0 >> 2] |= (uint32_t)LMAZE_OBS_BALL << ((b0 & 3) << 3);
            if ((unsigned)b1 < 16u && le + 1 < nb) w[b1 >> 2] |= (uint32_t)LMAZE_OBS_BALL << ((b1 & 3) << 3);
            if (V3) {
                const int g0 = goalflat[le] - c, g1 = CELLS - c + goalflat[min(le + 1, EPB)];
                if ((unsigned)g0 < 16u) w[g0 >> 2] |= (uint32_t)LMAZE_OBS_GOAL << ((g0 & 3) << 3);
                if ((unsigned)g1 < 16u && le + 1 < nb) w[g1 >> 2] |= (uint32_t)LMAZE_OBS_GOAL << ((g1 & 3) << 3);
            }
            if (a.launch_hint & 0x100) {
                typedef unsigned v4u __attribute__((ext_vector_type(4)));
                v4u t = {w[0], w[1], w[2], w[3]};
                stream_store16(reinterpret_cast<v4u*>(obs) + q, t);
            } else {
                reinterpret_cast<uint4*>(obs)[q] = make_uint4(w[0], w[1], w[2], w[3]);
            }
        }
        for (int f = (nq << 4) + tid; f < R; f += LMAZE_BLOCK) {
            const int le = f / CELLS, c = f - le * CELLS;
            obs[f] = (uint8_t)(patb[c] | (ballflat[le] == c ? LMAZE_OBS_BALL : 0) | (V3 && goalflat[le] == c ? LMAZE_OBS_GOAL : 0));
        }
    } else {
        for (int f = tid; f < R; f += LMAZE_BLOCK) {
            const int le = f / CELLS, c = f - le * CELLS;
            if (!maskflag[le]) continue;
            obs[f] = (uint8_t)(patb[c] | (ballflat[le] == c ? LMAZE_OBS_BALL : 0) | (V3 && goalflat[le] == c ? LMAZE_OBS_GOAL : 0));
        }
    }
    }
    if (!has_next) break;
    __syncthreads();
    chunk = next;
    blockbase = chunk * EPB;
    nb = nb_next;
    in = in_next;
  }
    if (warmed == 0x7fedcba9 && a.n < 0) a.done[0] = 1;
}

struct RolloutArgs {
    const int32_t* actions;
    float* reward_t;
    uint8_t* done_t;
    int32_t T;
};

struct RolloutObsArgs : RolloutArgs {
    int32_t* obs_t;
    int32_t every;
    int32_t nt;
};

__device__ __forceinline__ int32_t* rollout_slot(const RolloutObsArgs& ro, int64_t n, int64_t base, int cells, int t) {
    if (ro.obs_t == nullptr || ro.every <= 0 || (t + 1) % ro.every != 0) return nullptr;
    return ro.obs_t + ((size_t)((t + 1) / ro.every - 1) * n + base) * cells;
}
__device__ __forceinline__ int32_t* rollout_slot(const RolloutArgs&, int64_t, int64_t, int, int) { return nullptr; }
__device__ __forceinline__ bool slot_nt(const RolloutArgs&) { return false; }
__device__ __forceinline__ bool slot_nt(const RolloutObsArgs& ro) { return ro.nt != 0; }

template <int VARIANT>
__device__ __forceinline__ EnvState rollout_load(const StepArgs& a, const RolloutArgs& ro, int64_t e, bool live) {
    EnvState s;
    s.b = make_int2(1, 1); s.g = make_int2(-1, -1);
    s.act = -1; s.sc = 0; s.done = 0; s.r = 0.0f;
    if (live) {
        s.b = a.ball[e];
        if (VARIANT == LMAZE_VARIANT_V3) s.g = a.goal[e];
        s.sc = a.step_count[e];
        if (VARIANT != LMAZE_VARIANT_V3) s.r = a.reward[e];
        if (a.auto_reset) s.done = a.done[e];
        s.act = ro.actions[e];
    }
    return s;
}

__device__ __forceinline__ void rollout_record(const RolloutArgs& ro, int64_t n, int t, int64_t e, const EnvState& s) {
    if (ro.reward_t) ro.reward_t[(size_t)t * n + e] = s.r;
    if (ro.done_t) ro.done_t[(size_t)t * n + e] = s.done;
}

template <int VARIANT>
__device__ __forceinline__ void rollout_store(const StepArgs& a, const RolloutArgs& ro, int64_t e, bool live, const EnvState& s,
                                              int hits) {
    if (live && ro.T > 0) {
        a.ball[e] = s.b;
        if (VARIANT == LMAZE_VARIANT_V3 && a.auto_reset) a.goal_rw[e] = s.g;
        a.step_count[e] = s.sc;
        a.reward[e] = s.r;
        a.done[e] = s.done;
        if (hits && a.goal_count) a.goal_count[e] += hits;
    }
}


template <int VARIANT, int EPW>
__global__ __launch_bounds__(LMAZE_BLOCK) void rollout_shared_wave8_kernel(const StepArgs a, const RolloutArgs ro) {
    constexpr bool REC = false;
#define LMAZE_ROLLOUT_BODY 1
#include "lmaze_rollout_body.h"
#undef LMAZE_ROLLOUT_BODY
}

template <int VARIANT, int EPW>
__global__ __launch_bounds__(LMAZE_BLOCK) __attribute__((amdgpu_waves_per_eu(6))) void rollout_shared_wave8_kernel(const StepArgs a, const RolloutObsArgs ro) {
    constexpr bool REC = true;
#define LMAZE_ROLLOUT_BODY 1
#include "lmaze_rollout_body.h"
#undef LMAZE_ROLLOUT_BODY
}

template <int VARIANT, class Bits>
__device__ __forceinline__ void rollout_render(int32_t* obs, int R, int CELLS, const int* ballflat, const int* goalflat, Bits bits,
                                               bool nt = false) {
    const int tid = threadIdx.x, nq = R >> 2;
    auto value = [&](int le, int c) {
        int v = bits(le, c);
        v |= (ballflat[le] == c) ? LMAZE_OBS_BALL : 0;
        if (VARIANT == LMAZE_VARIANT_V3) v |= (goalflat[le] == c) ? LMAZE_OBS_GOAL : 0;
        return v;
    };
    int le = (tid << 2) / CELLS, c = (tid << 2) - le * CELLS;
    const int dle = (LMAZE_BLOCK << 2) / CELLS, dc = (LMAZE_BLOCK << 2) - dle * CELLS;
    for (int q = tid; q < nq; q += LMAZE_BLOCK) {
        int vals[4], l2 = le, c2 = c;
#pragma unroll
        for (int j = 0; j < 4; ++j) {
            vals[j] = value(l2, c2);
            if (++c2 == CELLS) { c2 = 0; ++l2; }
        }
        if (nt) store16<true>(reinterpret_cast<int4*>(obs) + q, make_int4(vals[0], vals[1], vals[2], vals[3]));
        else reinterpret_cast<int4*>(obs)[q] = make_int4(vals[0], vals[1], vals[2], vals[3]);
        le += dle; c += dc;
        if (c >= CELLS) { c -= CELLS; ++le; }
    }
    const int f = (nq << 2) + tid;
    if (f < R) {
        const int l2 = f / CELLS;
        obs[f] = value(l2, f - l2 * CELLS);
    }
}


template <int VARIANT>
__global__ __launch_bounds__(LMAZE_BLOCK) void rollout_shared_kernel(const StepArgs a, const RolloutArgs ro) {
    constexpr bool REC = false;
#define LMAZE_ROLLOUT_BODY 2
#include "lmaze_rollout_body.h"
#undef LMAZE_ROLLOUT_BODY
}

template <int VARIANT>
__global__ __launch_bounds__(LMAZE_BLOCK) __attribute__((amdgpu_waves_per_eu(8))) void rollout_shared_kernel(const StepArgs a, const RolloutObsArgs ro) {
    constexpr bool REC = true;
#define LMAZE_ROLLOUT_BODY 2
#include "lmaze_rollout_body.h"
#undef LMAZE_ROLLOUT_BODY
// ... 55 lines not shown
                const int g1 = CELLS - c + goalflat[le + 1];
                if ((unsigned)g1 < 16u) w[g1 >> 2] |= (uint32_t)LMAZE_OBS_GOAL << ((g1 & 3) << 3);
            }
        }
        dst4[q] = make_uint4(w[0], w[1], w[2], w[3]);
    }
    const int t0 = h + (nq << 4);
    if (tid < h + (R - t0)) {
        const int f = tid < h ? tid : t0 + (tid - h);
        const int le = f / CELLS, c = f - le * CELLS;
        const uint8_t* patb = reinterpret_cast<const uint8_t*>(patw);
        dst[f] = (uint8_t)(patb[c] | (ballflat[le] == c ? LMAZE_OBS_BALL : 0) | (V3 && goalflat[le] == c ? LMAZE_OBS_GOAL : 0));
    }
}

template <int VARIANT>
__global__ __launch_bounds__(LMAZE_BLOCK) void rollout_shared_u8_kernel(const StepArgs a, const RolloutArgs ro) {
    constexpr bool REC = false;
#define LMAZE_ROLLOUT_BODY 4
#include "lmaze_rollout_body.h"
#undef LMAZE_ROLLOUT_BODY
}

template <int VARIANT>
__global__ __launch_bounds__(LMAZE_BLOCK) void rollout_shared_u8_kernel(const StepArgs a, const RolloutObs8Args ro) {
    constexpr bool REC = true;
#define LMAZE_ROLLOUT_BODY 4
#include "lmaze_rollout_body.h"
#undef LMAZE_ROLLOUT_BODY
}

struct PolicyTable {
    const uint8_t* table;
    int32_t* actions_t;
    int32_t* key_t;
    int32_t key_mode;
    uint32_t epsilon;
};
struct RolloutPolicyArgs : RolloutObsArgs { PolicyTable pol; };
struct RolloutPolicy8Args : RolloutObs8Args { PolicyTable pol; };

template <int VARIANT>
__device__ __forceinline__ EnvState policy_load(const StepArgs& a, int64_t e, bool live) {
    EnvState s;
    s.b = make_int2(1, 1); s.g = make_int2(-1, -1);
    s.act = -1; s.sc = 0; s.done = 0; s.r = 0.0f;
    if (live) {
        s.b = a.ball[e];
        if (VARIANT == LMAZE_VARIANT_V3) s.g = a.goal[e];
        s.sc = a.step_count[e];
        if (VARIANT != LMAZE_VARIANT_V3) s.r = a.reward[e];
        if (a.auto_reset) s.done = a.done[e];
    }
    return s;
}

__device__ __forceinline__ uint4 policy_draw(uint64_t seed, uint64_t epoch, int64_t env_global) {
    const uint64_t e = (uint64_t)env_global;
    return philox4x32_10(make_uint4((uint32_t)e, (uint32_t)(e >> 32), (uint32_t)epoch, (uint32_t)(epoch >> 32) ^ 0x80000000u),
                         make_uint2((uint32_t)seed, (uint32_t)(seed >> 32)));
}

template <int VARIANT>
__device__ __forceinline__ void policy_act(const StepArgs& a, const PolicyTable& p, const uint8_t* tab, int G, int t, int64_t e,
                                           EnvState& s) {
    int key = clampi(s.b.x, 0, G - 1) * G + clampi(s.b.y, 0, G - 1);
    int act;
    if (VARIANT == LMAZE_VARIANT_V3 && p.key_mode != 0) {
        key += (clampi(s.g.x, 0, G - 1) * G + clampi(s.g.y, 0, G - 1)) * G * G;
        act = p.table[key];
    } else {
        act = tab[key];
    }
    if (p.epsilon != 0) {
        const uint4 r = policy_draw(a.seed, a.epoch + (uint64_t)t, a.env_base + e);
        if (r.x < p.epsilon) act = (int)(r.y >> 30);
    }
    s.act = act;
    if (p.actions_t) p.actions_t[(size_t)t * a.n + e] = act;
    if (p.key_t) p.key_t[(size_t)t * a.n + e] = key;
}

#define LMAZE_ROLLOUT_POLICY 1
template <int VARIANT>
__global__ __launch_bounds__(LMAZE_BLOCK) __attribute__((amdgpu_waves_per_eu(8))) void rollout_shared_kernel(const StepArgs a, const RolloutPolicyArgs ro) {
    constexpr bool REC = true;
#define LMAZE_ROLLOUT_BODY 2
#include "lmaze_rollout_body.h"
#undef LMAZE_ROLLOUT_BODY
}

template <int VARIANT>
__global__ __launch_bounds__(LMAZE_BLOCK) __attribute__((amdgpu_waves_per_eu(7))) void rollout_perenv_kernel(const StepArgs a, const RolloutPolicyArgs ro) {
    constexpr bool REC = true;
#define LMAZE_ROLLOUT_BODY 3
#include "lmaze_rollout_body.h"
#undef LMAZE_ROLLOUT_BODY
}

template <int VARIANT, bool CLOSED>
__global__ __launch_bounds__(LMAZE_BLOCK) void rollout_shared_u8_kernel(const StepArgs a, const RolloutPolicy8Args ro) {
    constexpr bool REC = true;
#define LMAZE_ROLLOUT_BODY 4
#include "lmaze_rollout_body.h"
#undef LMAZE_ROLLOUT_BODY
}
#undef LMAZE_ROLLOUT_POLICY

typedef uint32_t sample_row_t __attribute__((ext_vector_type(4)));
struct SampleTable {
    const sample_row_t* table;
    int32_t* actions_t;
    int32_t* key_t;
    int32_t key_mode;
    int32_t staged;
};
struct RolloutSampleArgs : RolloutObsArgs { SampleTable pol; };
struct RolloutSample8Args : RolloutObs8Args { SampleTable pol; };

template <int VARIANT>
__device__ __forceinline__ void policy_act(const StepArgs& a, const SampleTable& p, const sample_row_t* tab, int G, int t, int64_t e,
                                           EnvState& s) {
    typedef const __attribute__((address_space(3))) sample_row_t* lds_rows;
    typedef const __attribute__((address_space(1))) sample_row_t* global_rows;
    int key = clampi(s.b.x, 0, G - 1) * G + clampi(s.b.y, 0, G - 1);
    sample_row_t c;
    if (VARIANT == LMAZE_VARIANT_V3 && p.key_mode != 0) {
        key += (clampi(s.g.x, 0, G - 1) * G + clampi(s.g.y, 0, G - 1)) * G * G;
        c = ((global_rows)p.table)[key];
    } else if (p.staged) {
        c = ((lds_rows)tab)[key];
    } else {
        c = ((global_rows)p.table)[key];
    }
    const uint32_t r = policy_draw(a.seed, a.epoch + (uint64_t)t, a.env_base + e).x;
    const int act = (int)(r >= c.x) + (int)(r >= c.y) + (int)(r >= c.z);
    asm volatile("" ::"v"(c.w));
    s.act = act;
    if (p.actions_t) p.actions_t[(size_t)t * a.n + e] = act;
    if (p.key_t) p.key_t[(size_t)t * a.n + e] = key;
}

#define LMAZE_ROLLOUT_POLICY 2
template <int VARIANT>
__global__ __launch_bounds__(LMAZE_BLOCK) __attribute__((amdgpu_waves_per_eu(8))) void rollout_shared_kernel(const StepArgs a, const RolloutSampleArgs ro) {
    constexpr bool REC = true;
#define LMAZE_ROLLOUT_BODY 2
#include "lmaze_rollout_body.h"
#undef LMAZE_ROLLOUT_BODY
}

template <int VARIANT>
__global__ __launch_bounds__(LMAZE_BLOCK) __attribute__((amdgpu_waves_per_eu(7))) void rollout_perenv_kernel(const StepArgs a, const RolloutSampleArgs ro) {
    constexpr bool REC = true;
#define LMAZE_ROLLOUT_BODY 3
#include "lmaze_rollout_body.h"
#undef LMAZE_ROLLOUT_BODY
}

template <int VARIANT, bool CLOSED>
__global__ __launch_bounds__(LMAZE_BLOCK) void rollout_shared_u8_kernel(const StepArgs a, const RolloutSample8Args ro) {
    constexpr bool REC = true;
#define LMAZE_ROLLOUT_BODY 4
#include "lmaze_rollout_body.h"
#undef LMAZE_ROLLOUT_BODY
}
#undef LMAZE_ROLLOUT_POLICY


static size_t shared_lds_bytes(int G, bool specialised, int epb, bool with_marks) {
    const int cells = G * G;
    const int pat = (specialised && (G & 1)) ? 4 * cells : cells;
    const int grp = (specialised && (G & 1)) ? 4 : 1;
    const size_t marks = (specialised && with_marks) ? (size_t)2 * 2 * (epb / grp) * ((grp * cells + 31) / 32) * 4 : 0;
    return (size_t)pat * 4 + 3 * (size_t)epb * 4 + (size_t)((cells + 15) & ~15) + (size_t)((cells * 2 + 15) & ~15) + marks;
}

int perenv_envs_per_block(int G, int layout_bytes) {
    const int cells = G * G;
    int epb = (layout_bytes / cells) & ~15;
    if (epb < 16) epb = 16;
    if (epb > LMAZE_BLOCK) epb = LMAZE_BLOCK;
    return epb;
}

static size_t perenv_lds_bytes(int G, int epb) {
    return (size_t)((epb * G * G + 15) & ~15) + (3 * (size_t)(epb + 1) + 2 * (size_t)epb) * 4;
}


static size_t lds_for_workgroups_per_cu(int k) {
    const size_t cap = 160 * 1024;
    return ((cap / k + cap / (k + 1)) / 2) & ~(size_t)255;
}

static bool specialised_grid(int g) { return g == 8 || g == 11 || g == 12 || g == 14 || g == 18 || g == 32; }

static const StepPolicyRow* step_policy_lookup(int g, int variant, bool auto_reset, int64_t n, int sel) {
    const StepPolicyRow* best = nullptr;
    long best_cost = 0;
    const int l2 = (int)lround(log2((double)(n < 1 ? 1 : n)) * 16.0);
    for (int i = 0; i < kStepPolicyRows; ++i) {
        const StepPolicyRow& r = kStepPolicy[i];
        if ((r.auto_reset != 0) != auto_reset) continue;
        if (sel == 0 ? !r.is_default : r.sel != sel) continue;
        if (specialised_grid(g) != specialised_grid(r.g)) continue;
        if (specialised_grid(g) && r.g != g) continue;
        const long cost = (long)abs(r.g - g) * 1000000 + (r.variant != variant ? 100000 : 0) + abs(r.log2n_x16 - l2);
        if (!best || cost < best_cost) { best = &r; best_cost = cost; }
    }
    return best;
}

template <int GT, int EPB>
constexpr int sel_of() {
    if (GT == 11 || GT == 12) return EPB == 64 ? 1 : (EPB == 32 ? 2 : 3);
    if (GT == 14 || GT == 18) return EPB == 32 ? 1 : 2;
    if (GT == 8) return EPB == 128 ? 1 : 2;
    if (GT == 32) return EPB == 8 ? 1 : 2;
    return EPB == 256 ? 1 : (EPB == 64 ? 2 : 3);
}

template <int GT, int VARIANT, bool DO_STEP, int EPB>
static hipError_t launch_shared(const StepArgs& a, hipStream_t s) {
    const int64_t blocks = (a.n + EPB - 1) / EPB;
    size_t lds = shared_lds_bytes(a.grid, GT != 0, EPB, VARIANT == LMAZE_VARIANT_V3);
    const bool nt = a.obs != nullptr && beyond_caches(a.n, a.grid * a.grid);
    int def_cu = 3, def_m = 2;
    if (const StepPolicyRow* r = step_policy_lookup(a.grid, VARIANT, a.auto_reset != 0, a.n, sel_of<GT, EPB>())) {
        def_cu = r->per_cu;
        def_m = r->chunks;
    }
    int per_cu = a.launch_hint & 15;
    if (per_cu == 0 && nt) per_cu = def_cu;
    if (per_cu >= 1 && per_cu < 8) {
        const size_t want = lds_for_workgroups_per_cu(per_cu);
        if (want > lds) lds = want;
    }
    int m = (a.launch_hint >> 4) & 15;
    if (m == 0) m = nt ? def_m : 1;
    const int64_t grid = (blocks + m - 1) / m;
    if (!grid_ok(grid)) return hipErrorInvalidConfiguration;
    if (a.info) {
        char name[96];
        snprintf(name, sizeof(name), "step_shared_kernel<%d, v%d, %s, %d, %s>", GT, VARIANT, DO_STEP ? "step" : "observe", EPB, nt ? "nt" : "plain");
        describe_launch(a.info, name, EPB, per_cu >= 1 && per_cu < 8 ? per_cu : 0, m, nt, grid, LMAZE_BLOCK, lds);
        return hipSuccess;
    }
    if (nt)
        hipLaunchKernelGGL((step_shared_kernel<GT, VARIANT, DO_STEP, EPB, true>), dim3((unsigned)grid),
                           dim3(LMAZE_BLOCK), lds, s, a);
    else
        hipLaunchKernelGGL((step_shared_kernel<GT, VARIANT, DO_STEP, EPB, false>), dim3((unsigned)grid),
                           dim3(LMAZE_BLOCK), lds, s, a);
    return hipGetLastError();
}

template <int G, int VARIANT, bool DO_STEP>
static hipError_t launch_perenv_wave(const StepArgs& a, hipStream_t s) {
    StepArgs b = a;
    b.envs_per_block = 1;
    const int64_t per_block = (int64_t)b.envs_per_block * (LMAZE_BLOCK / 64);
    const int64_t blocks = (a.n + per_block - 1) / per_block;
    const bool nt = a.obs != nullptr && beyond_caches(a.n, G * G);
    if (!grid_ok(blocks)) return hipErrorInvalidConfiguration;
    if (a.info) {
        char name[96];
        snprintf(name, sizeof(name), "step_perenv_wave_kernel<%d, v%d, %s, %s>", G, VARIANT, DO_STEP ? "step" : "observe", nt ? "nt" : "plain");
        describe_launch(a.info, name, (int)per_block, 0, 1, nt, blocks, LMAZE_BLOCK, 0);
        return hipSuccess;
    }
    if (nt)
        hipLaunchKernelGGL((step_perenv_wave_kernel<G, VARIANT, DO_STEP, true>), dim3((unsigned)blocks),
                           dim3(LMAZE_BLOCK), 0, s, b);
    else
        hipLaunchKernelGGL((step_perenv_wave_kernel<G, VARIANT, DO_STEP, false>), dim3((unsigned)blocks),
                           dim3(LMAZE_BLOCK), 0, s, b);
    return hipGetLastError();
}

template <int GT, int VARIANT, bool DO_STEP>
static hipError_t launch_perenv(const StepArgs& a, hipStream_t s) {
    if constexpr (GT == 32) return launch_perenv_wave<32, VARIANT, DO_STEP>(a, s);
    if constexpr (GT == 0) {
        if (a.grid == 16) return launch_perenv_wave<16, VARIANT, DO_STEP>(a, s);
        if (a.grid == 48) return launch_perenv_wave<48, VARIANT, DO_STEP>(a, s);
        if (a.grid == 64) return launch_perenv_wave<64, VARIANT, DO_STEP>(a, s);
    }
    StepArgs b = a;
    b.envs_per_block = perenv_envs_per_block(a.grid, 8192);
    const int64_t blocks = (a.n + b.envs_per_block - 1) / b.envs_per_block;
    if (!grid_ok(blocks)) return hipErrorInvalidConfiguration;
    if (a.info) {
        char name[96];
        snprintf(name, sizeof(name), "step_perenv_kernel<%d, v%d, %s>", GT, VARIANT, DO_STEP ? "step" : "observe");
        describe_launch(a.info, name, b.envs_per_block, 0, 1, false, blocks, LMAZE_BLOCK, perenv_lds_bytes(a.grid, b.envs_per_block));
        return hipSuccess;
    }
    hipLaunchKernelGGL((step_perenv_kernel<GT, VARIANT, DO_STEP>), dim3((unsigned)blocks), dim3(LMAZE_BLOCK),
                       perenv_lds_bytes(a.grid, b.envs_per_block), s, b);
    return hipGetLastError();
}

template <int VARIANT>
static int table_sel(const StepArgs& a, int fallback) {
    const StepPolicyRow* r = step_policy_lookup(a.grid, VARIANT, a.auto_reset != 0, a.n, 0);
    return r ? r->sel : fallback;
}

template <int GT, int VARIANT, bool DO_STEP>
static hipError_t launch_one(const StepArgs& a, int layout_mode, hipStream_t s) {
    if (a.n == 0) return hipSuccess;
    if (layout_mode != LMAZE_LAYOUT_SHARED) return launch_perenv<GT, VARIANT, DO_STEP>(a, s);
    if constexpr (GT == 8) {
        const bool small = a.obs == nullptr || !beyond_caches(a.n, 64);
        if (small && a.mask == nullptr && (a.launch_hint & 0x100) == 0) {
            int code = (a.launch_hint >> 4) & 15;
            if (code < 1 || code > 3) code = a.n >= 65536 ? 1 : 2;
            const int epw = 128 >> code;
            int wpb = a.launch_hint & 15;
            if (wpb != 1 && wpb != 2 && wpb != 4) wpb = a.n >= 65536 ? 4 : 1;
            const int64_t waves = (a.n + epw - 1) / epw;
            const int64_t blocks = (waves + wpb - 1) / wpb;
            if (!grid_ok(blocks)) return hipErrorInvalidConfiguration;
            const dim3 grid((unsigned)blocks), block(64 * wpb);
            if (a.info) {
                char name[96];
                snprintf(name, sizeof(name), "step_shared_wave8_kernel<v%d, %s, %d>", VARIANT, DO_STEP ? "step" : "observe", epw);
                describe_launch(a.info, name, epw * wpb, 0, 1, false, blocks, 64 * wpb, 0);
                return hipSuccess;
            }
            if (code == 1) hipLaunchKernelGGL((step_shared_wave8_kernel<VARIANT, DO_STEP, 64>), grid, block, 0, s, a);
            else if (code == 2) hipLaunchKernelGGL((step_shared_wave8_kernel<VARIANT, DO_STEP, 32>), grid, block, 0, s, a);
            else hipLaunchKernelGGL((step_shared_wave8_kernel<VARIANT, DO_STEP, 16>), grid, block, 0, s, a);
            return hipGetLastError();
        }
        int sel = (a.launch_hint >> 10) & 3;
        if (sel == 0) sel = table_sel<VARIANT>(a, a.obs != nullptr ? 2 : 1);
        if (sel == 2) return launch_shared<GT, VARIANT, DO_STEP, 64>(a, s);
        return launch_shared<GT, VARIANT, DO_STEP, 128>(a, s);
    } else if constexpr (GT == 11 || GT == 12) {
        int sel = (a.launch_hint >> 10) & 3;
        const bool streaming = a.obs != nullptr && beyond_caches(a.n, GT * GT);
        if (sel == 0) {
            if (GT == 11) sel = streaming ? 2 : 1;
            else sel = streaming ? 3 : 1;
            if (streaming) sel = table_sel<VARIANT>(a, sel);
        }
        if (sel == 2) return launch_shared<GT, VARIANT, DO_STEP, 32>(a, s);
        if (sel == 3) return launch_shared<GT, VARIANT, DO_STEP, 16>(a, s);
        return launch_shared<GT, VARIANT, DO_STEP, 64>(a, s);
    } else if constexpr (GT == 14 || GT == 18) {
        int sel = (a.launch_hint >> 10) & 3;
        const bool streaming = a.obs != nullptr && beyond_caches(a.n, GT * GT);
        if (sel == 0) sel = ((GT == 14 || VARIANT == LMAZE_VARIANT_V3) && streaming) ? 2 : 1;
        if (((a.launch_hint >> 10) & 3) == 0 && streaming) sel = table_sel<VARIANT>(a, sel);
        if (sel == 2) return launch_shared<GT, VARIANT, DO_STEP, 16>(a, s);
        return launch_shared<GT, VARIANT, DO_STEP, 32>(a, s);
    } else if constexpr (GT == 32) {
        int sel = (a.launch_hint >> 10) & 3;
        const bool streaming = a.obs != nullptr && beyond_caches(a.n, GT * GT);
        if (sel == 0) sel = streaming ? table_sel<VARIANT>(a, 2) : 1;
        if (sel == 2) return launch_shared<GT, VARIANT, DO_STEP, 4>(a, s);
        return launch_shared<GT, VARIANT, DO_STEP, 8>(a, s);
    } else {
        int sel = (a.launch_hint >> 10) & 3;
        if (sel == 0) {
            sel = a.grid >= 15 ? 3 : (a.grid >= 5 ? 2 : 1);
            if (a.obs != nullptr && beyond_caches(a.n, a.grid * a.grid) && a.grid >= 5) sel = table_sel<VARIANT>(a, sel);
        }
        if (sel == 3) return launch_shared<GT, VARIANT, DO_STEP, 16>(a, s);
        if (sel == 2) return launch_shared<GT, VARIANT, DO_STEP, 64>(a, s);
        return launch_shared<GT, VARIANT, DO_STEP, 256>(a, s);
    }
}

template <int VARIANT, bool DO_STEP>
static hipError_t dispatch_grid(const StepArgs& a, int layout_mode, hipStream_t s) {
    switch (a.grid) {
        case 8:  return launch_one<8, VARIANT, DO_STEP>(a, layout_mode, s);
        case 11: return launch_one<11, VARIANT, DO_STEP>(a, layout_mode, s);
        case 12: return launch_one<12, VARIANT, DO_STEP>(a, layout_mode, s);
        case 14: return launch_one<14, VARIANT, DO_STEP>(a, layout_mode, s);
        case 18: return launch_one<18, VARIANT, DO_STEP>(a, layout_mode, s);
        case 32: return launch_one<32, VARIANT, DO_STEP>(a, layout_mode, s);
        default: return launch_one<0, VARIANT, DO_STEP>(a, layout_mode, s);
    }
}

hipError_t launch_step(int variant, bool do_step, const StepArgs& a, int layout_mode, hipStream_t s);

#ifndef LMAZE_U8_DEFAULT_SEL
#define LMAZE_U8_DEFAULT_SEL 1
#endif
#ifndef LMAZE_U8_DEFAULT_CHUNKS
#define LMAZE_U8_DEFAULT_CHUNKS 2
#endif
template <int EPB>
static hipError_t launch_step_u8_epb(int variant, bool do_step, const StepArgs& a, hipStream_t s) {
    const int cells = a.grid * a.grid, pw = (2 * cells + 16 + 3) >> 2;
    const size_t lds = ((size_t)4 * pw * 4 + 3 * (size_t)(EPB + 1) * 4 + (size_t)((cells + 1) & ~1) * 2 + (size_t)cells + 15) & ~(size_t)15;
    int m = (a.launch_hint >> 4) & 15;
    if (m == 0) m = LMAZE_U8_DEFAULT_CHUNKS;
    const int64_t nchunks = (a.n + EPB - 1) / EPB;
    const int64_t blocks = (nchunks + m - 1) / m;
    if (!grid_ok(blocks)) return hipErrorInvalidConfiguration;
    if (a.info) {
        char name[96];
        snprintf(name, sizeof(name), "step_shared_u8_kernel<v%d, %s, %d>", variant, do_step ? "step" : "observe", EPB);
        describe_launch(a.info, name, EPB, 0, m, false, blocks, LMAZE_BLOCK, lds);
        return hipSuccess;
    }
    const dim3 grid((unsigned)blocks), block(LMAZE_BLOCK);
    StepArgs b = a;
    b.launch_hint = (a.launch_hint & ~0x100) | ((size_t)a.n * cells > ((size_t)64 << 20) ? 0x100 : 0);
    if (variant == LMAZE_VARIANT_V3) {
        if (do_step) hipLaunchKernelGGL((step_shared_u8_kernel<LMAZE_VARIANT_V3, true, EPB>), grid, block, lds, s, b);
        else hipLaunchKernelGGL((step_shared_u8_kernel<LMAZE_VARIANT_V3, false, EPB>), grid, block, lds, s, b);
    } else {
        if (do_step) hipLaunchKernelGGL((step_shared_u8_kernel<LMAZE_VARIANT_V0, true, EPB>), grid, block, lds, s, b);
        else hipLaunchKernelGGL((step_shared_u8_kernel<LMAZE_VARIANT_V0, false, EPB>), grid, block, lds, s, b);
    }
    return hipGetLastError();
}

hipError_t launch_step_u8(int variant, bool do_step, const StepArgs& a, hipStream_t s) {
    if (a.n == 0) return hipSuccess;
    int sel = (a.launch_hint >> 10) & 3;
    if (sel == 0) sel = LMAZE_U8_DEFAULT_SEL;
    if (sel == 1) return launch_step_u8_epb<256>(variant, do_step, a, s);
    if (sel == 2) return launch_step_u8_epb<128>(variant, do_step, a, s);
    return launch_step_u8_epb<64>(variant, do_step, a, s);
}

static bool slot_stores_nt(const StepArgs& a, const RolloutRec* rec) {
    return rec && rec->obs_t && ((a.launch_hint >> 15) & 1);
}

enum RolloutFamily { RO_WAVE8, RO_SHARED, RO_PERENV, RO_U8, RO_STEPS };
static const char* const kRolloutKernel[] = {"rollout_shared_wave8_kernel", "rollout_shared_kernel", "rollout_perenv_kernel",
                                             "rollout_shared_u8_kernel"};
struct RolloutPlan {
    RolloutFamily family;
    int epb;
    int block;
    int64_t blocks;
    size_t lds;
    bool nt;
};

static size_t rollout_u8_lds_bytes(int G, int epb) {
    const int cells = G * G, pw = (2 * cells + 16 + 3) >> 2;
    return ((size_t)4 * pw * 4 + 2 * (size_t)(epb + 1) * 4 + (size_t)((cells + 1) & ~1) * 2 + (size_t)cells + 15) & ~(size_t)15;
}

static size_t policy_table_lds_bytes(int G) { return (size_t)((G * G + 15) & ~15); }

enum { PLAN_OPEN = 0, PLAN_POLICY = 1, PLAN_SAMPLE_LDS = 2, PLAN_SAMPLE_GLOBAL = 3 };
static RolloutPlan rollout_plan(const StepArgs& a, int layout_mode, int32_t T, const RolloutRec* rec, bool u8, int pol = PLAN_OPEN) {
    const int cells = a.grid * a.grid;
    const bool sample = pol == PLAN_SAMPLE_LDS || pol == PLAN_SAMPLE_GLOBAL;
    const size_t tab = pol == PLAN_POLICY ? policy_table_lds_bytes(a.grid) : pol == PLAN_SAMPLE_LDS ? (size_t)16 * cells : 0;
    const int hint_epb = (a.launch_hint >> 12) & 7;
    const bool planes = a.obs != nullptr || (rec && rec->obs_t);
    RolloutPlan p{RO_STEPS, 0, LMAZE_BLOCK, 0, 0, false};
    if (u8) {
        int epb = a.n >= 65536 ? 64 : 16;
        if (rec && rec->obs_t && a.n >= 262144) epb = 256;
        if (hint_epb) epb = 4 << (hint_epb - 1);
        if (epb < 16) epb = 16;
        if (epb > LMAZE_BLOCK) epb = LMAZE_BLOCK;
        while (epb > 16 && rollout_u8_lds_bytes(a.grid, epb) + tab > ((size_t)64 << 10)) epb >>= 1;
        p.family = RO_U8;
        p.epb = epb;
        p.lds = rollout_u8_lds_bytes(a.grid, epb) + tab;
    } else if (!pol && layout_mode == LMAZE_LAYOUT_SHARED && a.grid == 8 && (!planes || !beyond_caches(a.n, 64)) &&
               (a.launch_hint & 0x100) == 0) {
        p.family = RO_WAVE8;
        p.block = 64 * (a.n >= 65536 ? 4 : 1);
        p.epb = p.block;
    } else if (pol || (T > 1 && (a.launch_hint & 0x100) == 0)) {
        const bool perenv = layout_mode == LMAZE_LAYOUT_PER_ENV;
        p.family = perenv ? RO_PERENV : RO_SHARED;
        int epb = a.n >= 65536 ? 64 : (a.n >= 16384 ? 32 : 16);
        if (perenv)
            while (epb > 4 && (size_t)epb * cells > (size_t)32 << 10) epb >>= 1;
        if (!rec && beyond_caches(a.n, cells))
            while (epb > 8 && (size_t)epb * cells * 4 > 12288) epb >>= 1;
        if (perenv && rec && epb == 32 && a.n < 65536) epb = 16;
        if (hint_epb) epb = 4 << (hint_epb - 1);
        if (perenv && epb > 64) epb = 64;
        auto lds_of = [&](int k) {
            const size_t own = perenv ? 2 * (size_t)k * 4 + (((size_t)k * cells + 15) & ~(size_t)15)
                                      : (size_t)cells * 4 + 2 * (size_t)k * 4 + (size_t)((cells + 15) & ~15) + (size_t)((cells * 2 + 15) & ~15);
            return tab + (sample ? (own + 15) & ~(size_t)15 : own);
        };
        if (perenv)
            while (epb > 4 && lds_of(epb) > (size_t)160 * 1024) epb >>= 1;
        p.epb = epb;
        p.lds = lds_of(epb);
        p.nt = slot_stores_nt(a, rec);
    }
    if (p.family != RO_STEPS) p.blocks = (a.n + p.epb - 1) / p.epb;
    return p;
}

template <class F>
static const void* kernel_of(int variant, F v3, F v0) { return (const void*)(variant == LMAZE_VARIANT_V3 ? v3 : v0); }

static const void* rollout_kernel(RolloutFamily f, int variant, bool rec) {
    using P = void (*)(const StepArgs, const RolloutArgs);
    using R = void (*)(const StepArgs, const RolloutObsArgs);
    using R8 = void (*)(const StepArgs, const RolloutObs8Args);
    constexpr int V0 = LMAZE_VARIANT_V0, V3 = LMAZE_VARIANT_V3;
    switch (f) {
        case RO_WAVE8: return !rec ? kernel_of<P>(variant, rollout_shared_wave8_kernel<V3, 64>, rollout_shared_wave8_kernel<V0, 64>)
                                   : kernel_of<R>(variant, rollout_shared_wave8_kernel<V3, 64>, rollout_shared_wave8_kernel<V0, 64>);
        case RO_SHARED: return !rec ? kernel_of<P>(variant, rollout_shared_kernel<V3>, rollout_shared_kernel<V0>)
                                    : kernel_of<R>(variant, rollout_shared_kernel<V3>, rollout_shared_kernel<V0>);
        case RO_PERENV: return !rec ? kernel_of<P>(variant, rollout_perenv_kernel<V3>, rollout_perenv_kernel<V0>)
                                    : kernel_of<R>(variant, rollout_perenv_kernel<V3>, rollout_perenv_kernel<V0>);
        default: return rec ? kernel_of<R8>(variant, rollout_shared_u8_kernel<V3>, rollout_shared_u8_kernel<V0>)
                            : kernel_of<P>(variant, rollout_shared_u8_kernel<V3>, rollout_shared_u8_kernel<V0>);
    }
}

hipError_t launch_rollout(int variant, const StepArgs& a0, int layout_mode, const int32_t* actions, int32_t T, float* reward_t,
                          uint8_t* done_t, hipStream_t s, const RolloutRec* rec, bool u8) {
    if (T <= 0 || a0.n == 0) return hipSuccess;
    const RolloutPlan p = rollout_plan(a0, layout_mode, T, rec, u8);
    if (p.family == RO_STEPS) {
        int32_t* obs_t = rec ? static_cast<int32_t*>(rec->obs_t) : nullptr;
        const int64_t plane = (int64_t)a0.n * a0.grid * a0.grid;
        for (int32_t t = 0; t < T; ++t) {
            StepArgs a = a0;
            a.action = actions + (size_t)t * a0.n;
            a.epoch = a0.epoch + (uint64_t)t;
            int32_t* slot = nullptr;
            if (obs_t && rec->every > 0 && (t + 1) % rec->every == 0)
                slot = obs_t + (size_t)((t + 1) / rec->every - 1) * plane;
            if (rec) a.obs = t == T - 1 && a0.obs ? a0.obs : slot;
            hipError_t rc = launch_step(variant, true, a, layout_mode, s);
            if (rc != hipSuccess || a0.info) return rc;
            if (slot && a.obs != slot && (rc = hipMemcpyAsync(slot, a.obs, (size_t)plane * 4, hipMemcpyDeviceToDevice, s)) != hipSuccess)
                return rc;
            if (reward_t && (rc = hipMemcpyAsync(reward_t + (size_t)t * a0.n, a0.reward, (size_t)a0.n * 4, hipMemcpyDeviceToDevice, s)) != hipSuccess) return rc;
            if (done_t && (rc = hipMemcpyAsync(done_t + (size_t)t * a0.n, a0.done, (size_t)a0.n, hipMemcpyDeviceToDevice, s)) != hipSuccess) return rc;
        }
        return hipSuccess;
    }
    if (!grid_ok(p.blocks)) return hipErrorInvalidConfiguration;
    if (a0.info) {
        char name[96], every[24] = "";
        if (rec) snprintf(every, sizeof(every), " every=%d", rec->every);
        snprintf(name, sizeof(name), "%s<v%d%s%s%s> T=%d%s", kRolloutKernel[p.family], variant, p.family == RO_WAVE8 ? ", 64" : "",
                 rec ? ", obs_t" : "", p.nt ? ", nt" : "", T, every);
        describe_launch(a0.info, name, p.epb, 0, 1, p.nt, p.blocks, p.block, p.lds);
        return hipSuccess;
    }
    StepArgs a = a0;
    a.envs_per_block = p.epb;
    RolloutArgs plain{actions, reward_t, done_t, T};
    RolloutObsArgs ro{plain, rec ? static_cast<int32_t*>(rec->obs_t) : nullptr, rec ? rec->every : 0, p.nt ? 1 : 0};
    RolloutObs8Args ro8{plain, rec ? static_cast<uint8_t*>(rec->obs_t) : nullptr, rec ? rec->every : 0};
    void* args[] = {&a, !rec ? (void*)&plain : u8 ? (void*)&ro8 : (void*)&ro};
    const void* kernel = rollout_kernel(p.family, variant, rec != nullptr);
    (void)hipLaunchKernel(kernel, dim3((unsigned)p.blocks), dim3(p.block), args, p.lds, s);
    return hipGetLastError();
}

hipError_t launch_rollout_policy(int variant, const StepArgs& a0, int layout_mode, const RolloutPolicy& pol, int32_t T,
                                 float* reward_t, uint8_t* done_t, hipStream_t s, const RolloutRec& rec, bool u8) {
    if (T <= 0 || a0.n == 0) return hipSuccess;
    const RolloutPlan p = rollout_plan(a0, layout_mode, T, &rec, u8, PLAN_POLICY);
    if (!grid_ok(p.blocks)) return hipErrorInvalidConfiguration;
    if (a0.info) {
        char name[96];
        snprintf(name, sizeof(name), "%s<v%d, policy=%s%s%s> T=%d every=%d", kRolloutKernel[p.family], variant,
                 pol.key_mode ? "goal" : "ball", rec.obs_t ? ", obs_t" : "", p.nt ? ", nt" : "", T, rec.every);
        describe_launch(a0.info, name, p.epb, 0, 1, p.nt, p.blocks, p.block, p.lds);
        return hipSuccess;
    }
    StepArgs a = a0;
    a.envs_per_block = p.epb;
    const PolicyTable tab{pol.table, pol.actions_t, pol.key_t, pol.key_mode, pol.epsilon};
    RolloutArgs plain{nullptr, reward_t, done_t, T};
    RolloutPolicyArgs ro{{plain, static_cast<int32_t*>(rec.obs_t), rec.every, p.nt ? 1 : 0}, tab};
    RolloutPolicy8Args ro8{{plain, static_cast<uint8_t*>(rec.obs_t), rec.every}, tab};
    void* args[] = {&a, u8 ? (void*)&ro8 : (void*)&ro};
    using K = void (*)(const StepArgs, const RolloutPolicyArgs);
    using K8 = void (*)(const StepArgs, const RolloutPolicy8Args);
    constexpr int V0 = LMAZE_VARIANT_V0, V3 = LMAZE_VARIANT_V3;
    const void* kernel = p.family == RO_U8       ? kernel_of<K8>(variant, rollout_shared_u8_kernel<V3, true>, rollout_shared_u8_kernel<V0, true>)
                         : p.family == RO_PERENV ? kernel_of<K>(variant, rollout_perenv_kernel<V3>, rollout_perenv_kernel<V0>)
                                                 : kernel_of<K>(variant, rollout_shared_kernel<V3>, rollout_shared_kernel<V0>);
    (void)hipLaunchKernel(kernel, dim3((unsigned)p.blocks), dim3(p.block), args, p.lds, s);
    return hipGetLastError();
}

hipError_t launch_rollout_sample(int variant, const StepArgs& a0, int layout_mode, const RolloutSample& smp, int32_t T,
                                 float* reward_t, uint8_t* done_t, hipStream_t s, const RolloutRec& rec, bool u8) {
    if (T <= 0 || a0.n == 0) return hipSuccess;
    const bool staged = smp.key_mode == 0 && a0.grid <= 32;
    const RolloutPlan p = rollout_plan(a0, layout_mode, T, &rec, u8, staged ? PLAN_SAMPLE_LDS : PLAN_SAMPLE_GLOBAL);
    if (!grid_ok(p.blocks)) return hipErrorInvalidConfiguration;
    if (a0.info) {
        char name[96];
        snprintf(name, sizeof(name), "%s<v%d, sample=%s, table=%s%s%s> T=%d every=%d", kRolloutKernel[p.family], variant,
                 smp.key_mode ? "goal" : "ball", staged ? "lds" : "global", rec.obs_t ? ", obs_t" : "", p.nt ? ", nt" : "", T,
                 rec.every);
        describe_launch(a0.info, name, p.epb, 0, 1, p.nt, p.blocks, p.block, p.lds);
        return hipSuccess;
    }
    StepArgs a = a0;
    a.envs_per_block = p.epb;
// ... 25 lines not shown
```

### gym-lmaze_amd/vec_env.py

```python
import ctypes as C
import logging

import numpy as np
import torch

from . import _abi
from . import layouts as L
from ._base import VecEnvBase
from ._tuning import OnlineTuner

_log = logging.getLogger("gym_lmaze_amd")

VARIANTS = {
    "v0": dict(id=_abi.VARIANT_V0, layout=L.V0_GRID_12, expansion=7, step_limit=100,
               rewards=(-1.0, -0.01, 100.0), channel_mask=(_abi.OBS_BALL, _abi.OBS_WALL, _abi.OBS_GOAL, _abi.OBS_FREE),
               n_actions=4),
    "v3": dict(id=_abi.VARIANT_V3, layout=L.V3_GRID_18, expansion=4, step_limit=100,
               rewards=(-1.0, -0.01, 100.0), channel_mask=(_abi.OBS_FREE, _abi.OBS_BALL, _abi.OBS_GOAL),
               n_actions=4),
}


class LmazeVecEnv(VecEnvBase):
    _STATS_KEYS = VecEnvBase._STATS_KEYS + ("goal_count",)

    def __init__(self, num_envs, variant="v0", layout=None, per_env_layouts=None, device=None,
                 expansion=None, step_limit=None, rewards=None, seed=0, env_base=0, validate=True,
                 online_autotune=False, obs_dtype="int32"):
        if variant not in VARIANTS:
            raise ValueError("unknown variant %r (have %s)" % (variant, sorted(VARIANTS)))
        spec = VARIANTS[variant]
        self.variant = variant
        self._init_common(num_envs, device, seed, env_base)
        self.expansion = int(expansion if expansion is not None else spec["expansion"])
        self.step_limit = int(step_limit if step_limit is not None else spec["step_limit"])
        self.rewards = tuple(float(r) for r in (rewards if rewards is not None else spec["rewards"]))
        self.channel_mask = spec["channel_mask"]
        self._is_v3 = variant == "v3"

        N = self.num_envs
        if per_env_layouts is not None:
            lay = per_env_layouts
            if not isinstance(lay, torch.Tensor):
                lay = torch.from_numpy(L.to_codes(np.asarray(lay)))
            if lay.dtype != torch.uint8 or lay.dim() != 3 or lay.shape[0] != N or lay.shape[1] != lay.shape[2]:
                raise ValueError("per_env_layouts must be uint8[N,G,G]")
            lay = lay.to(self.device).contiguous()
            if validate:
                _validate_on_device(lay, need_goal=not self._is_v3)
            self.layout_mode = _abi.LAYOUT_PER_ENV
            self.layout = lay
        else:
            codes = L.to_codes(layout if layout is not None else spec["layout"])
            if codes.ndim != 2:
                raise ValueError("layout must be [G,G]; use per_env_layouts for [N,G,G]")
            if validate:
                L.validate(codes, need_goal_marker=not self._is_v3)
            self.layout_mode = _abi.LAYOUT_SHARED
            self.layout = torch.from_numpy(codes.copy()).to(self.device)
        self.grid = int(self.layout.shape[-1])
        if not (3 <= self.grid <= _abi.MAX_GRID):
            raise ValueError("grid side must be in [3, %d]" % _abi.MAX_GRID)
        G = self.grid

        self._alloc_state([("ball_xy", torch.int32, 2), ("goal_xy", torch.int32, 2), ("step_count", torch.int32, 1),
                           ("reward", torch.float32, 1), ("goal_count", torch.int32, 1), ("done", torch.uint8, 1)])
        if obs_dtype not in ("int32", "u8"):
            raise ValueError("obs_dtype must be 'int32' or 'u8'")
        self._u8 = obs_dtype == "u8"
        if self._u8 and (self.layout_mode != _abi.LAYOUT_SHARED or G < 4):
            raise ValueError("obs_dtype='u8' needs a shared layout with G >= 4")
        self.obs = torch.zeros((N, G, G), dtype=torch.uint8 if self._u8 else torch.int32, device=self.device)
        self._expanded = None

        self.params = _abi.make_params(spec["id"], G, self.layout_mode, self.step_limit, *self.rewards)
        self._pp = C.byref(self.params)
        self._cmask = (C.c_int32 * len(self.channel_mask))(*self.channel_mask)
        self._bind_pointers()
        streaming = self.layout_mode == _abi.LAYOUT_SHARED and N * G * G * 4 > (192 << 20) and not self._u8
        self._tuner = OnlineTuner(self.ONLINE_CANDIDATES) if (online_autotune and streaming) else None
        if self._tuner is not None:
            _log.info("gym-lmaze_amd: online launch-policy tuning on for the next ~%d steps of this %d-env batch",
                      self._tuner.warm + self._tuner.samples * len(self.ONLINE_CANDIDATES), N)

        if not self._is_v3:
            self._fill_goal_from_layout()
        self.reset()

    def _bind_pointers(self):
        self._p_layout = self.layout.data_ptr()
        self._p_ball = self.ball_xy.data_ptr()
        self._p_goal = self.goal_xy.data_ptr()
        self._p_step = self.step_count.data_ptr()
        self._p_reward = self.reward.data_ptr()
        self._p_done = self.done.data_ptr()
        self._p_gc = self.goal_count.data_ptr()
        self._p_obs = self.obs.data_ptr()
        self._gc_ptr = None if self._is_v3 else self._p_gc

    def _fill_goal_from_layout(self):
        G = self.grid
        flat = (self.layout.reshape(-1, G * G) == ord("X")).to(torch.int32)
        has = flat.sum(dim=1) > 0
        first = torch.argmax(flat, dim=1).to(torch.int32)
        first = torch.where(has, first, torch.full_like(first, -1))
        gx = torch.div(first, G, rounding_mode="floor")
        gy = first - gx * G
        g = torch.stack([gx, gy], dim=1).to(torch.int32)
        self.goal_xy.copy_(g.expand(self.num_envs, 2) if g.shape[0] == 1 else g)

    def step(self, actions, render=True, auto_reset=False):
        a = self._as_i32(actions, self.num_envs)
        with self._guard():
            self._launch_step(a.data_ptr(), self._p_obs if render else None, auto_reset)
        return self.obs, self.reward, self.done, actions

    def step_raw(self, action_ptr, auto_reset=False, epoch_slot=None):
        self._launch_step(action_ptr, self._p_obs, auto_reset, epoch_slot)

    def tuning_progress(self):
        t = self._tuner
        if t is None:
            return None
        return sum(len(v) for v in t.timings.values()), t.samples * len(t.candidates)

    def set_launch_policy(self, per_cu, chunks=1):
        self.params.launch_hint = self.launch_hint_of(per_cu, chunks)
        self._tuner = None

    def _launch_step(self, action_ptr, obs_ptr, auto_reset, epoch_slot=None):
        tuner = self._tuner
        if tuner is not None and obs_ptr is not None and not torch.cuda.is_current_stream_capturing():
            cand = tuner.next_candidate()
            self._set_policy(cand)
            best = tuner.time(cand, self._launch_step_raw, action_ptr, obs_ptr, auto_reset, epoch_slot)
            if best is not None:
                self._set_policy(best)
                self.tuned_policy, self._tuner = best, None
                _log.info("gym-lmaze_amd: online tuning done, launch policy (workgroups per CU, chunks) = %s", best)
            return
        self._launch_step_raw(action_ptr, obs_ptr, auto_reset, epoch_slot)

    def _launch_step_raw(self, action_ptr, obs_ptr, auto_reset, epoch_slot=None):
        lib, N, st = _abi.lib, self.num_envs, self._stream()
        if self._u8:
            epoch, e_in, e_out = self._epoch_args(auto_reset, epoch_slot)
            rc = lib.lmaze_step_u8(self._pp, self._p_layout, action_ptr, self._p_ball, self._p_goal if self._is_v3 else None,
                                   self._p_step, self._p_reward, self._p_done, None if self._is_v3 else self._p_gc, obs_ptr, N,
                                   1 if auto_reset else 0, self.seed & (2 ** 64 - 1), epoch, self.env_base, e_in, e_out, st)
            _abi.check("lmaze_step_u8", rc)
            return
        if auto_reset:
            seed = self.seed & (2 ** 64 - 1)
            epoch, e_in, e_out = self._epoch_args(True, epoch_slot)
            if self._is_v3:
                rc = lib.lmaze_step_v3_autoreset(self._pp, self._p_layout, action_ptr, self._p_ball, self._p_goal,
                                                 self._p_step, self._p_reward, self._p_done, obs_ptr, N,
                                                 seed, epoch, self.env_base, e_in, e_out, st)
            else:
                rc = lib.lmaze_step_v0_autoreset(self._pp, self._p_layout, action_ptr, self._p_ball, self._p_step,
                                                 self._p_reward, self._p_done, self._p_gc, obs_ptr, N,
                                                 seed, epoch, self.env_base, e_in, e_out, st)
        elif self._is_v3:
            rc = lib.lmaze_step_v3(self._pp, self._p_layout, action_ptr, self._p_ball, self._p_goal,
                                   self._p_step, self._p_reward, self._p_done, obs_ptr, N, st)
        else:
            rc = lib.lmaze_step_v0(self._pp, self._p_layout, action_ptr, self._p_ball, self._p_step,
                                   self._p_reward, self._p_done, self._p_gc, obs_ptr, N, st)
        _abi.check("lmaze_step_" + self.variant, rc)

    def _set_policy(self, policy):
        self.params.launch_hint = self.launch_hint_of(*policy)

    def _set_obs(self, ptr):
        self._p_obs = ptr

    DEFAULT_POLICY = (0, 0)
    CANDIDATES = ((0, 0), (2, 1), (2, 2), (3, 1), (3, 2), (4, 1), (4, 2), (5, 2), (6, 2), (7, 2), (8, 1), (8, 2),
                  (6, 1, 2), (8, 1, 2), (5, 1, 2), (4, 2, 2), (3, 1, 2), (4, 1, 2), (3, 2, 2), (4, 1, 1), (3, 2, 1), (2, 1, 1), (2, 2, 1), (8, 1, 3), (5, 2, 3))

    ONLINE_CANDIDATES = ((0, 0), (3, 1), (3, 2), (5, 2), (8, 1), (6, 1, 2), (8, 2, 2), (5, 2, 2))

    @staticmethod
    def launch_hint_of(per_cu, chunks=1, epb_sel=0, no_stagger=False):
        return (int(per_cu) & 15) | ((int(chunks) & 15) << 4) | ((int(epb_sel) & 3) << 10) | (0x200 if no_stagger else 0)

    def autotune(self, auto_reset=False, actions=None, steps=24, candidates=None, warm=150, between=None, rounds=3,
                 placement_trials=0):
        obs_bytes = self.num_envs * self.grid * self.grid * 4
        if self.layout_mode != _abi.LAYOUT_SHARED or obs_bytes <= (192 << 20) or self._u8:
            return {}
        cands = [tuple(c) if isinstance(c, (tuple, list)) else (int(c), 1) for c in (candidates or self.CANDIDATES)]
        N = self.num_envs
        if actions is None:
            rows = max(2, min(512, (320 << 20) // (4 * N) + 1))
            actions = torch.randint(0, 4, (rows, N), dtype=torch.int32, device=self.device)
        self._check_rows("autotune(actions=...)", actions)
        base, stride = actions.data_ptr(), N * 4
        timings = self._tune(int(actions.shape[0]),
                             lambda r: self._launch_step_raw(base + r * stride, self._p_obs, auto_reset),
                             candidates=cands, default=self.DEFAULT_POLICY, trial_policy=(5, 2), steps=steps, warm=warm,
                             rounds=rounds, placement_trials=placement_trials, between=between)
        self._tuner = None
        self.observe()
        return timings

    def rollout(self, actions, auto_reset=True, device_epoch=False, trajectory=False, obs_t=None, obs_every=None):
        self._check_rows("rollout()", actions)
        base, stride = actions.data_ptr(), self.num_envs * 4
        T, N = int(actions.shape[0]), self.num_envs
        k = None
        if obs_every is not None:
            if device_epoch or self._tuner is not None:
                raise ValueError("rollout(obs_every=...) is not available with a device-resident epoch or while the online tuner runs")
            k = self._obs_slots(T, obs_every, obs_t, self.obs, allow_final=True)
        elif obs_t is not None:
            raise ValueError("obs_t needs obs_every")
        if not device_epoch and self._tuner is None:
            rows = self._traj_rows(T) if trajectory else None
            args = (self._pp, self._p_layout, base, T, self._p_ball, self._p_goal if self._is_v3 else None, self._p_step,
                    self._p_reward, self._p_done, None if self._is_v3 else self._p_gc, self._p_obs,
                    rows[0].data_ptr() if rows else None, rows[1].data_ptr() if rows else None,
                    N, 1 if auto_reset else 0, self.seed & (2 ** 64 - 1), self._epoch, self.env_base)
            name = ("lmaze_rollout" if k is None else "lmaze_rollout_obs") + ("_u8" if self._u8 else "")
            with self._guard():
                if k is None:
                    rc = getattr(_abi.lib, name)(*args, self._stream())
                else:
                    slots = obs_t.data_ptr() if k > 0 and obs_t.shape[0] > 0 else None
                    rc = getattr(_abi.lib, name)(*args, slots, k, self._stream())
            _abi.check(name, rc)
            if auto_reset:
                self._epoch += T
            return self._rollout_result(rows)
        if trajectory:
            raise ValueError("rollout(trajectory=True) is not available with a device-resident epoch or while the online tuner runs")
        with self._guard():
            for t in range(actions.shape[0]):
                self._launch_step(base + t * stride, self._p_obs, auto_reset, t if device_epoch else None)
        return self.obs, self.reward, self.done

    @staticmethod
    def greedy_table(q):
        if not (isinstance(q, torch.Tensor) and q.dim() == 2 and q.is_floating_point() and 1 <= q.shape[1] <= 255):
            raise ValueError("q must be a float tensor [S, A] with 1 <= A <= 255")
        A = q.shape[1]
        idx = torch.arange(A, device=q.device, dtype=torch.int32).expand_as(q)
        first = torch.where(q == q.max(dim=1, keepdim=True).values, idx, torch.full_like(idx, A)).min(dim=1).values
        return first.to(torch.uint8)

    def rollout_policy(self, T, policy=None, q=None, epsilon=0.0, key="ball", auto_reset=True, trajectory=False,
                       actions_t=None, key_t=None, obs_t=None, obs_every=0):
        if self._tuner is not None or torch.cuda.is_current_stream_capturing():
            raise ValueError("rollout(obs_every=...) is not available with a device-resident epoch or while the online tuner runs")
        if isinstance(T, bool) or not isinstance(T, (int, np.integer)) or T < 0:
            raise ValueError("T must be an int >= 0")
        T, N, G = int(T), self.num_envs, self.grid
        if (policy is None) == (q is None):
            raise ValueError("rollout_policy() wants exactly one of policy= and q=")
        if key not in _abi.KEY_MODES:
            raise ValueError("key must be 'ball' or 'goal'")
        if key == "goal" and not self._is_v3:
            raise ValueError("key='goal' needs the v3 variant: v0 keeps no per-env goal")
        entries = G ** 4 if key == "goal" else G * G
        if q is not None:
            if not isinstance(q, torch.Tensor) or q.device != self.device:
                raise ValueError("q must be a float tensor [S, A] on %s" % self.device)
            policy = self.greedy_table(q)
        if not (isinstance(policy, torch.Tensor) and policy.dtype == torch.uint8 and policy.device == self.device
                and policy.is_contiguous() and policy.numel() == entries):
            raise ValueError("policy must be a contiguous uint8 tensor of %d entries on %s (key=%r, G=%d)"
                             % (entries, self.device, key, G))
        eps = _abi.epsilon_u32(epsilon)
        self._check_rows("rollout_policy()", actions_t, key_t)
        for name, t in (("actions_t", actions_t), ("key_t", key_t)):
            if t is not None and t.shape[0] != T:
                raise ValueError("%s must have T = %d rows" % (name, T))
        k = self._obs_slots(T, obs_every, obs_t, self.obs, allow_final=True)
        rows = self._traj_rows(T) if trajectory else None
        if trajectory:
            actions_t = torch.empty((T, N), dtype=torch.int32, device=self.device) if actions_t is None else actions_t
            key_t = torch.empty((T, N), dtype=torch.int32, device=self.device) if key_t is None else key_t
        name = "lmaze_rollout_policy" + ("_u8" if self._u8 else "")
        slots = obs_t.data_ptr() if k > 0 and obs_t.shape[0] > 0 else None
        with self._guard():
            rc = getattr(_abi.lib, name)(
                self._pp, self._p_layout, policy.data_ptr(), _abi.KEY_MODES[key], eps, T, self._p_ball,
                self._p_goal if self._is_v3 else None, self._p_step, self._p_reward, self._p_done,
                None if self._is_v3 else self._p_gc, self._p_obs, rows[0].data_ptr() if rows else None,
                rows[1].data_ptr() if rows else None, None if actions_t is None else actions_t.data_ptr(),
                None if key_t is None else key_t.data_ptr(), N, 1 if auto_reset else 0, self.seed & (2 ** 64 - 1), self._epoch,
                self.env_base, slots, k, self._stream())
        _abi.check(name, rc)
        self._epoch += T
        out = self._rollout_result(rows)
        return out + (actions_t, key_t) if trajectory else out

    def rollout_sample(self, T, probs=None, logits=None, temperature=1.0, thresholds=None, key="ball", auto_reset=True,
                       trajectory=False, actions_t=None, key_t=None, obs_t=None, obs_every=0):
        if self._tuner is not None or torch.cuda.is_current_stream_capturing():
            raise ValueError("rollout_sample() is not available with a device-resident epoch or while the online tuner runs")
        if isinstance(T, bool) or not isinstance(T, (int, np.integer)) or T < 0:
            raise ValueError("T must be an int >= 0")
        T, N, G = int(T), self.num_envs, self.grid
        if sum(x is not None for x in (probs, logits, thresholds)) != 1:
            raise ValueError("rollout_sample() wants exactly one of probs=, logits= and thresholds=")
        if key not in _abi.KEY_MODES:
            raise ValueError("key must be 'ball' or 'goal'")
        if key == "goal" and not self._is_v3:
            raise ValueError("key='goal' needs the v3 variant: v0 keeps no per-env goal")
        entries = G ** 4 if key == "goal" else G * G
        if thresholds is None:
            src, name = (probs, "probs") if logits is None else (logits, "logits")
            if not (isinstance(src, torch.Tensor) and src.is_floating_point() and src.device == self.device
                    and tuple(src.shape) == (entries, 4)):
                raise ValueError("%s must be a float tensor [%d, 4] on %s (key=%r, G=%d)" % (name, entries, self.device, key, G))
            if logits is not None:
                if not float(temperature) > 0.0:
                    raise ValueError("temperature must be > 0")
                src = torch.softmax(logits.double() / float(temperature), -1)
            thresholds = _abi.sampling_thresholds(src)
        if not (isinstance(thresholds, torch.Tensor) and thresholds.dtype in (torch.uint32, torch.int32)
                and thresholds.device == self.device and thresholds.is_contiguous() and tuple(thresholds.shape) == (entries, 4)
                and thresholds.data_ptr() % 16 == 0):
            raise ValueError("thresholds must be a contiguous, 16-byte aligned uint32 tensor [%d, 4] on %s (key=%r, G=%d)"
                             % (entries, self.device, key, G))
        self._check_rows("rollout_sample()", actions_t, key_t)
        for name, t in (("actions_t", actions_t), ("key_t", key_t)):
            if t is not None and t.shape[0] != T:
                raise ValueError("%s must have T = %d rows" % (name, T))
        k = self._obs_slots(T, obs_every, obs_t, self.obs, allow_final=True)
        rows = self._traj_rows(T) if trajectory else None
        if trajectory:
            actions_t = torch.empty((T, N), dtype=torch.int32, device=self.device) if actions_t is None else actions_t
            key_t = torch.empty((T, N), dtype=torch.int32, device=self.device) if key_t is None else key_t
        name = "lmaze_rollout_sample" + ("_u8" if self._u8 else "")
        slots = obs_t.data_ptr() if k > 0 and obs_t.shape[0] > 0 else None
        with self._guard():
            rc = getattr(_abi.lib, name)(
                self._pp, self._p_layout, thresholds.data_ptr(), _abi.KEY_MODES[key], T, self._p_ball,
                self._p_goal if self._is_v3 else None, self._p_step, self._p_reward, self._p_done,
                None if self._is_v3 else self._p_gc, self._p_obs, rows[0].data_ptr() if rows else None,
                rows[1].data_ptr() if rows else None, None if actions_t is None else actions_t.data_ptr(),
                None if key_t is None else key_t.data_ptr(), N, 1 if auto_reset else 0, self.seed & (2 ** 64 - 1), self._epoch,
                self.env_base, slots, k, self._stream())
        _abi.check(name, rc)
        self._epoch += T
        out = self._rollout_result(rows)
        return out + (actions_t, key_t) if trajectory else out

    def observe(self, mask_ptr=None):
        if self._u8:
            with self._guard():
                rc = _abi.lib.lmaze_observe_u8(self._pp, self._p_layout, self._p_ball, self._p_goal if self._is_v3 else None,
                                               mask_ptr, self._p_obs, self.num_envs, self._stream())
            _abi.check("lmaze_observe_u8", rc)
            return self.obs
        with self._guard():
            rc = _abi.lib.lmaze_observe(self._pp, self._p_layout, self._p_ball,
                                        self._p_goal if self._is_v3 else None, self._p_obs,
                                        self.num_envs, self._stream())
        _abi.check("lmaze_observe", rc)
        return self.obs

    def reset(self, mask=None, seed=None):
        if seed is not None:
            self.seed = int(seed)
            self._epoch = 0
        m, m_ptr = self._mask_ptr(mask)
        with self._guard():
            rc = _abi.lib.lmaze_reset(self._pp, self._p_layout, m_ptr, self.seed & (2 ** 64 - 1), self._epoch,
                                      self.env_base, self._p_ball, self._p_goal if self._is_v3 else None,
                                      self._p_step, self._p_reward, self._p_done, None if self._u8 else self._p_obs,
                                      self.num_envs, self._stream())
        _abi.check("lmaze_reset", rc)
        self._epoch += 1
        if self._u8:
            self.observe(mask_ptr=m_ptr)
        return self.obs

    def set_state(self, ball_xy=None, goal_xy=None, step_count=None, reward=None, goal_count=None, done=None):
        for name, src in (("ball_xy", ball_xy), ("goal_xy", goal_xy), ("step_count", step_count), ("reward", reward),
                          ("goal_count", goal_count), ("done", done)):
            if src is not None:
                self._write_state(name, src)

    def expanded(self, out=None):
        N, G, E, Cn = self.num_envs, self.grid, self.expansion, len(self.channel_mask)
        if out is None:
            if self._expanded is None:
                self._expanded = torch.empty((N, Cn, G * E, G * E), dtype=torch.float32, device=self.device)
            out = self._expanded
        src = self.obs.to(torch.int32) if self._u8 else self.obs
        with self._guard():
            rc = _abi.lib.lmaze_render_expanded(src.data_ptr(), G, E, self._cmask, Cn, out.data_ptr(), N,
                                                self._stream())
        _abi.check("lmaze_render_expanded", rc)
        return out

    def capture_rollout(self, actions, auto_reset=False, obs_t=None, obs_every=None):
        if obs_t is not None or obs_every is not None:
            raise ValueError("capture_rollout() does not record observations: call rollout(obs_t=..., obs_every=...)")
        return self._capture(actions.shape[0], auto_reset,
                             lambda: self.rollout(actions, auto_reset=auto_reset, device_epoch=auto_reset))

    def planes(self, out=None):
        N, G, Cn = self.num_envs, self.grid, len(self.channel_mask)
        if out is None:
            out = torch.empty((N, Cn, G, G), dtype=torch.float32, device=self.device)
        with self._guard():
            rc = _abi.lib.lmaze_render_expanded(self._p_obs, G, 1, self._cmask, Cn, out.data_ptr(), N, self._stream())
        _abi.check("lmaze_render_expanded", rc)
        return out


def discounted_returns(reward_t, done_t, gamma, tail=None, out=None):
    def rows(t, dtypes):
        return (isinstance(t, torch.Tensor) and t.dtype in dtypes and t.dim() == 2 and t.is_cuda and t.is_contiguous()
                and t.device == reward_t.device and tuple(t.shape) == tuple(reward_t.shape))
    if not (isinstance(reward_t, torch.Tensor) and rows(reward_t, (torch.float32,))):
        raise ValueError("reward_t must be a contiguous float32[T,N] tensor on a GPU")
    if not rows(done_t, (torch.bool, torch.uint8)):
        raise ValueError("done_t must be a contiguous bool or uint8 tensor of reward_t's shape, on its device")
    T, N = reward_t.shape
    if tail is not None and not (isinstance(tail, torch.Tensor) and tail.dtype == torch.float32 and tail.device == reward_t.device
                                 and tail.is_contiguous() and tuple(tail.shape) == (N,)):
        raise ValueError("tail must be a contiguous float32[N] tensor on reward_t's device")
    if out is None:
        out = torch.empty_like(reward_t)
    elif not rows(out, (torch.float32,)):
        raise ValueError("out must be a contiguous float32 tensor of reward_t's shape, on its device")
    if T == 0 or N == 0:
        return out
    with torch.cuda.device(reward_t.device):
        rc = _abi.lib.lmaze_returns(reward_t.data_ptr(), done_t.data_ptr(), None if tail is None else tail.data_ptr(), float(gamma),
                                    out.data_ptr(), T, N, torch.cuda.current_stream(reward_t.device).cuda_stream)
    _abi.check("lmaze_returns", rc)
    return out


def _validate_on_device(lay, need_goal=True):
    W = ord("W")
    ok = ((lay[:, 0, :] == W).all() & (lay[:, -1, :] == W).all() & (lay[:, :, 0] == W).all()
          & (lay[:, :, -1] == W).all())
    if not bool(ok):
        raise ValueError("every layout needs a full 'W' border")
    codes = torch.tensor([ord(c) for c in "WBSX"], dtype=torch.uint8, device=lay.device)
    if not bool(torch.isin(lay, codes).all()):
        raise ValueError("layout cells must be one of 'W', 'B', 'S', 'X'")
    if need_goal and not bool((lay == ord("X")).flatten(1).any(dim=1).all()):
        raise ValueError("a layout has no 'X' cell")
```

### include/lmaze.h

```cpp
#ifndef LMAZE_H_
#define LMAZE_H_

#include <stdint.h>

#ifdef __cplusplus
extern "C" {
#endif

#define LMAZE_ABI_VERSION 4

enum {
    LMAZE_VARIANT_V0 = 0,
    LMAZE_VARIANT_V3 = 3
};

enum {
    LMAZE_LAYOUT_SHARED = 0,
    LMAZE_LAYOUT_PER_ENV = 1
};

enum {
    LMAZE_OBS_BALL = 1,
    LMAZE_OBS_WALL = 2,
    LMAZE_OBS_GOAL = 4,
    LMAZE_OBS_FREE = 8
};

enum {
    LMAZE_E_NULL = -1,
    LMAZE_E_GRID = -2,
    LMAZE_E_VARIANT = -3,
    LMAZE_E_LAYOUT = -4,
    LMAZE_E_COUNT = -5,
    LMAZE_E_ALIGN = -6,
    LMAZE_E_EXPANSION = -7,
    LMAZE_E_NODEVICE = -8
};

#define LMAZE_MAX_GRID 64
#define LMAZE_MAX_ENVS ((int64_t)1 << 30)
#define LMAZE_MAX_CHANNELS 8

typedef struct LmazeParams {
    int32_t variant;
    int32_t grid;
    int32_t layout_mode;
    int32_t step_limit;
    float reward_wall;
    float reward_move;
    float reward_goal;
    int32_t launch_hint;
} LmazeParams;

int lmaze_abi_version(void);

const char* lmaze_strerror(int code);

int lmaze_device_info(int device, int32_t* cu_count_host, char* name_host, int32_t name_len);

int lmaze_describe_step(const LmazeParams* params, int64_t n, int32_t auto_reset, int32_t with_obs, char* text_host,
                        int32_t len);

int lmaze_step_v0(const LmazeParams* params, const uint8_t* layout, const int32_t* action,
                  int32_t* ball_xy, int32_t* step_count, float* reward, uint8_t* done,
                  int32_t* goal_count, int32_t* obs, int64_t n, void* stream);

int lmaze_step_v3(const LmazeParams* params, const uint8_t* layout, const int32_t* action,
                  int32_t* ball_xy, const int32_t* goal_xy, int32_t* step_count, float* reward,
                  uint8_t* done, int32_t* obs, int64_t n, void* stream);

int lmaze_observe(const LmazeParams* params, const uint8_t* layout, const int32_t* ball_xy,
                  const int32_t* goal_xy, int32_t* obs, int64_t n, void* stream);

int lmaze_reset(const LmazeParams* params, const uint8_t* layout, const uint8_t* mask,
                uint64_t seed, uint64_t epoch, int64_t env_base, int32_t* ball_xy, int32_t* goal_xy,
                int32_t* step_count, float* reward, uint8_t* done, int32_t* obs, int64_t n,
                void* stream);

int lmaze_step_v0_autoreset(const LmazeParams* params, const uint8_t* layout, const int32_t* action,
                            int32_t* ball_xy, int32_t* step_count, float* reward, uint8_t* done,
                            int32_t* goal_count, int32_t* obs, int64_t n, uint64_t seed,
                            uint64_t epoch, int64_t env_base, const uint64_t* epoch_in_dev,
                            uint64_t* epoch_out_dev, void* stream);

int lmaze_step_v3_autoreset(const LmazeParams* params, const uint8_t* layout, const int32_t* action,
                            int32_t* ball_xy, int32_t* goal_xy, int32_t* step_count, float* reward,
                            uint8_t* done, int32_t* obs, int64_t n, uint64_t seed, uint64_t epoch,
                            int64_t env_base, const uint64_t* epoch_in_dev, uint64_t* epoch_out_dev,
                            void* stream);

int lmaze_step_u8(const LmazeParams* params, const uint8_t* layout, const int32_t* action, int32_t* ball_xy, int32_t* goal_xy,
                  int32_t* step_count, float* reward, uint8_t* done, int32_t* goal_count, uint8_t* obs8, int64_t n,
                  int32_t auto_reset, uint64_t seed, uint64_t epoch, int64_t env_base, const uint64_t* epoch_in_dev,
                  uint64_t* epoch_out_dev, void* stream);
int lmaze_observe_u8(const LmazeParams* params, const uint8_t* layout, const int32_t* ball_xy, const int32_t* goal_xy,
                     const uint8_t* mask, uint8_t* obs8, int64_t n, void* stream);

int lmaze_rollout(const LmazeParams* params, const uint8_t* layout, const int32_t* actions, int32_t T, int32_t* ball_xy,
                  int32_t* goal_xy, int32_t* step_count, float* reward, uint8_t* done, int32_t* goal_count, int32_t* obs,
                  float* reward_t, uint8_t* done_t, int64_t n, int32_t auto_reset, uint64_t seed, uint64_t epoch,
                  int64_t env_base, void* stream);

int lmaze_rollout_obs(const LmazeParams* params, const uint8_t* layout, const int32_t* actions, int32_t T, int32_t* ball_xy,
                      int32_t* goal_xy, int32_t* step_count, float* reward, uint8_t* done, int32_t* goal_count, int32_t* obs,
                      float* reward_t, uint8_t* done_t, int64_t n, int32_t auto_reset, uint64_t seed, uint64_t epoch,
                      int64_t env_base, int32_t* obs_t, int32_t obs_every, void* stream);

int lmaze_rollout_u8(const LmazeParams* params, const uint8_t* layout, const int32_t* actions, int32_t T, int32_t* ball_xy,
                     int32_t* goal_xy, int32_t* step_count, float* reward, uint8_t* done, int32_t* goal_count, uint8_t* obs8,
                     float* reward_t, uint8_t* done_t, int64_t n, int32_t auto_reset, uint64_t seed, uint64_t epoch,
                     int64_t env_base, void* stream);

int lmaze_rollout_obs_u8(const LmazeParams* params, const uint8_t* layout, const int32_t* actions, int32_t T, int32_t* ball_xy,
                         int32_t* goal_xy, int32_t* step_count, float* reward, uint8_t* done, int32_t* goal_count, uint8_t* obs8,
                         float* reward_t, uint8_t* done_t, int64_t n, int32_t auto_reset, uint64_t seed, uint64_t epoch,
                         int64_t env_base, uint8_t* obs_t8, int32_t obs_every, void* stream);

int lmaze_describe_rollout(const LmazeParams* params, int64_t n, int32_t T, int32_t auto_reset, int32_t with_obs,
                           int32_t obs_every, char* text_host, int32_t len);

int lmaze_rollout_policy(const LmazeParams* params, const uint8_t* layout, const uint8_t* policy, int32_t key_mode,
                         uint32_t epsilon_u32, int32_t T, int32_t* ball_xy, int32_t* goal_xy, int32_t* step_count, float* reward,
                         uint8_t* done, int32_t* goal_count, int32_t* obs, float* reward_t, uint8_t* done_t, int32_t* actions_t,
                         int32_t* key_t, int64_t n, int32_t auto_reset, uint64_t seed, uint64_t epoch, int64_t env_base,
                         int32_t* obs_t, int32_t obs_every, void* stream);

int lmaze_rollout_policy_u8(const LmazeParams* params, const uint8_t* layout, const uint8_t* policy, int32_t key_mode,
                            uint32_t epsilon_u32, int32_t T, int32_t* ball_xy, int32_t* goal_xy, int32_t* step_count, float* reward,
                            uint8_t* done, int32_t* goal_count, uint8_t* obs8, float* reward_t, uint8_t* done_t, int32_t* actions_t,
                            int32_t* key_t, int64_t n, int32_t auto_reset, uint64_t seed, uint64_t epoch, int64_t env_base,
                            uint8_t* obs_t8, int32_t obs_every, void* stream);

int lmaze_describe_rollout_policy(const LmazeParams* params, int64_t n, int32_t T, int32_t auto_reset, int32_t with_obs,
                                  int32_t obs_every, int32_t key_mode, char* text_host, int32_t len);

int lmaze_rollout_sample(const LmazeParams* params, const uint8_t* layout, const uint32_t* thresholds, int32_t key_mode, int32_t T,
                         int32_t* ball_xy, int32_t* goal_xy, int32_t* step_count, float* reward, uint8_t* done, int32_t* goal_count,
                         int32_t* obs, float* reward_t, uint8_t* done_t, int32_t* actions_t, int32_t* key_t, int64_t n,
                         int32_t auto_reset, uint64_t seed, uint64_t epoch, int64_t env_base, int32_t* obs_t, int32_t obs_every,
                         void* stream);

int lmaze_rollout_sample_u8(const LmazeParams* params, const uint8_t* layout, const uint32_t* thresholds, int32_t key_mode, int32_t T,
                            int32_t* ball_xy, int32_t* goal_xy, int32_t* step_count, float* reward, uint8_t* done,
                            int32_t* goal_count, uint8_t* obs8, float* reward_t, uint8_t* done_t, int32_t* actions_t, int32_t* key_t,
                            int64_t n, int32_t auto_reset, uint64_t seed, uint64_t epoch, int64_t env_base, uint8_t* obs_t8,
                            int32_t obs_every, void* stream);

int lmaze_describe_rollout_sample(const LmazeParams* params, int64_t n, int32_t T, int32_t auto_reset, int32_t with_obs,
                                  int32_t obs_every, int32_t key_mode, char* text_host, int32_t len);

int lmaze_returns(const float* reward_t, const uint8_t* done_t, const float* tail, float gamma, float* returns_t, int32_t T,
                  int64_t n, void* stream);

int lmaze_render_expanded(const int32_t* obs, int32_t grid, int32_t expansion,
                          const int32_t* channel_mask_host, int32_t channels, float* out,
                          int64_t n, void* stream);

int lmaze_episode_stats(const uint8_t* done, const float* reward, const int32_t* step_count,
                        const int32_t* goal_count, float reward_goal, int64_t n, int64_t* out4, void* stream);

int lmaze_bandwidth_probe(const void* src, void* dst, int64_t bytes, void* stream);

enum {
    LMAZE_VARIANT_V1 = 1,
    LMAZE_VARIANT_V2 = 2,
    LMAZE_VARIANT_V4 = 4,
    LMAZE_VARIANT_V5 = 5,
    LMAZE_VARIANT_V6 = 6
};

#define LMAZE_FOVEA 5
#define LMAZE_MAX_LAYOUTS 16

typedef struct LmazeFovealParams {
    int32_t variant;
    int32_t grid;
    int32_t n_layouts;
    int32_t step_limit;
    int32_t foveal_step_limit;
    float reward_wall;
    float reward_move;
    float reward_goal;
    int32_t launch_hint;
} LmazeFovealParams;

typedef struct LmazeFovealBuffers {
    int32_t* ball_xy;
    int32_t* goal_xy;
    int32_t* fgoal_xy;
    int32_t* layout_id;
    int32_t* step_count;
    int32_t* foveal_step_count;
    float* reward;
    float* foveal_reward;
    uint8_t* done;
    uint8_t* foveal_done;
    float* visit;
    float* obs;
    int32_t* ball1_xy;
    int32_t* fovea_xy;
    int32_t* last_xy;
    int32_t* foveal_goal;
    float* obs_local;
    int32_t* visit_clock;
} LmazeFovealBuffers;

int64_t lmaze_foveal_visit_bytes(int32_t grid, int64_t n);

int lmaze_describe_foveal_step(const LmazeFovealParams* params, int64_t n, int32_t auto_reset, char* text_host, int32_t len);

int lmaze_foveal_materialise_visit(const LmazeFovealParams* params, const LmazeFovealBuffers* bufs, float* out,
                                   int64_t n, void* stream);

int lmaze_foveal_load_visit(const LmazeFovealParams* params, const LmazeFovealBuffers* bufs, const float* in,
                            int64_t n, void* stream);

int lmaze_foveal_step(const LmazeFovealParams* params, const uint8_t* layouts, const int32_t* action,
                      const LmazeFovealBuffers* bufs, int64_t n, void* stream);

int lmaze_foveal_step_autoreset(const LmazeFovealParams* params, const uint8_t* layouts, const int32_t* action,
                                const LmazeFovealBuffers* bufs, int64_t n, uint64_t seed, uint64_t epoch,
                                int64_t env_base, const uint64_t* epoch_in_dev, uint64_t* epoch_out_dev,
                                void* stream);

int lmaze_foveal_reset(const LmazeFovealParams* params, const uint8_t* layouts, const uint8_t* mask,
                       int32_t place, uint64_t seed, uint64_t epoch, int64_t env_base,
                       const LmazeFovealBuffers* bufs, int64_t n, void* stream);

int lmaze_v1_set_foveal_goal(const LmazeFovealParams* params, const uint8_t* layouts, const int32_t* ij,
                             const uint8_t* mask, const LmazeFovealBuffers* bufs, int64_t n, void* stream);

int lmaze_v5_planner_step(const LmazeFovealParams* params, const uint8_t* layouts, const int32_t* goal,
                          const uint8_t* mask, const LmazeFovealBuffers* bufs, int64_t n, void* stream);

int lmaze_v5_hier_step(const LmazeFovealParams* params, const uint8_t* layouts, const int32_t* action,
                       const int32_t* planner_goal, const LmazeFovealBuffers* bufs, int64_t n, uint64_t seed,
                       uint64_t epoch, int64_t env_base, const uint64_t* epoch_in_dev, uint64_t* epoch_out_dev,
                       void* stream);

int lmaze_foveal_rollout(const LmazeFovealParams* params, const uint8_t* layouts, const int32_t* actions,
                         const int32_t* planner_goals, int32_t T, const LmazeFovealBuffers* bufs, int64_t n,
                         int32_t auto_reset, uint64_t seed, uint64_t epoch, int64_t env_base,
                         float* reward_t, uint8_t* done_t, float* foveal_reward_t, uint8_t* foveal_done_t,
                         void* stream);

int lmaze_foveal_rollout_obs(const LmazeFovealParams* params, const uint8_t* layouts, const int32_t* actions,
                             const int32_t* planner_goals, int32_t T, const LmazeFovealBuffers* bufs, int64_t n,
                             int32_t auto_reset, uint64_t seed, uint64_t epoch, int64_t env_base,
                             float* reward_t, uint8_t* done_t, float* foveal_reward_t, uint8_t* foveal_done_t,
                             float* obs_t, float* obs_local_t, int32_t obs_every, void* stream);

int lmaze_describe_foveal_rollout(const LmazeFovealParams* params, int64_t n, int32_t T, int32_t auto_reset,
                                  int32_t two_level, char* text_host, int32_t len);

int lmaze_describe_foveal_rollout_obs(const LmazeFovealParams* params, int64_t n, int32_t T, int32_t auto_reset,
                                      int32_t two_level, int32_t obs_every, char* text_host, int32_t len);

int lmaze_v6_safe_foveal_goal(const LmazeFovealParams* params, const uint8_t* layouts, uint64_t seed,
                              uint64_t epoch, int64_t env_base, const LmazeFovealBuffers* bufs,
                              int32_t* out_goal, int64_t n, void* stream);

int lmaze_expand_planes(const float* planes, int32_t channels, int32_t g, int32_t expansion, float* out,
                        int64_t n, void* stream);

#ifdef __cplusplus
}
#endif
#endif
```

Measured before the change: 13.88 billion.

## Pack per-env maze layouts to 2 bits per cell for step kernels

```diff
diff --git a/gym-lmaze_amd/_abi.py b/gym-lmaze_amd/_abi.py
--- a/gym-lmaze_amd/_abi.py
+++ b/gym-lmaze_amd/_abi.py
@@ -10,7 +10,7 @@
 VARIANT_V0, VARIANT_V3 = 0, 3
 VARIANT_V1, VARIANT_V2, VARIANT_V4, VARIANT_V5, VARIANT_V6 = 1, 2, 4, 5, 6
 FOVEA = 5
-LAYOUT_SHARED, LAYOUT_PER_ENV = 0, 1
+LAYOUT_SHARED, LAYOUT_PER_ENV, LAYOUT_PER_ENV_PACKED = 0, 1, 2
 OBS_BALL, OBS_WALL, OBS_GOAL, OBS_FREE = 1, 2, 4, 8
 MAX_GRID, MAX_CHANNELS = 64, 8
 
@@ -24,7 +24,7 @@
            "lmaze_rollout_obs", "lmaze_foveal_rollout_obs", "lmaze_rollout_u8", "lmaze_rollout_obs_u8",
            "lmaze_describe_rollout", "lmaze_rollout_policy", "lmaze_rollout_policy_u8", "lmaze_describe_rollout_policy",
            "lmaze_rollout_sample", "lmaze_rollout_sample_u8", "lmaze_describe_rollout_sample", "lmaze_returns",
-           "lmaze_describe_foveal_rollout_obs")
+           "lmaze_describe_foveal_rollout_obs", "lmaze_pack_layouts", "lmaze_packed_layout_bytes")
 
 
 class LmazeParams(C.Structure):
@@ -95,6 +95,10 @@
     lib.lmaze_observe.argtypes = [P, vp, vp, vp, vp, i64, vp]
     lib.lmaze_reset.restype = C.c_int
     lib.lmaze_reset.argtypes = [P, vp, vp, u64, u64, i64, vp, vp, vp, vp, vp, vp, i64, vp]
+    lib.lmaze_packed_layout_bytes.restype = i64
+    lib.lmaze_packed_layout_bytes.argtypes = [i32, i64]
+    lib.lmaze_pack_layouts.restype = C.c_int
+    lib.lmaze_pack_layouts.argtypes = [P, vp, vp, i64, vp]
     lib.lmaze_render_expanded.restype = C.c_int
     lib.lmaze_render_expanded.argtypes = [vp, i32, i32, C.POINTER(i32), i32, vp, i64, vp]
     lib.lmaze_bandwidth_probe.restype = C.c_int
diff --git a/gym-lmaze_amd/csrc/lmaze_abi.hip b/gym-lmaze_amd/csrc/lmaze_abi.hip
--- a/gym-lmaze_amd/csrc/lmaze_abi.hip
+++ b/gym-lmaze_amd/csrc/lmaze_abi.hip
@@ -6,10 +6,12 @@
 
 using namespace lmaze;
 
-static int check_params(const LmazeParams* p, int64_t n) {
+static int check_params(const LmazeParams* p, int64_t n, bool packed_ok = false) {
     if (!p) return LMAZE_E_NULL;
     if (p->grid < 3 || p->grid > LMAZE_MAX_GRID) return LMAZE_E_GRID;
-    if (p->layout_mode != LMAZE_LAYOUT_SHARED && p->layout_mode != LMAZE_LAYOUT_PER_ENV) return LMAZE_E_LAYOUT;
+    if (p->layout_mode != LMAZE_LAYOUT_SHARED && p->layout_mode != LMAZE_LAYOUT_PER_ENV &&
+        !(packed_ok && p->layout_mode == LMAZE_LAYOUT_PER_ENV_PACKED))
+        return LMAZE_E_LAYOUT;
     if (n < 0 || n > LMAZE_MAX_ENVS) return LMAZE_E_COUNT;
     return 0;
 }
@@ -204,7 +206,7 @@
 
 int lmaze_describe_step(const LmazeParams* params, int64_t n, int32_t auto_reset, int32_t with_obs, char* text_host,
                         int32_t len) {
-    int rc = check_params(params, n);
+    int rc = check_params(params, n, true);
     if (rc) return rc;
     if (params->variant != LMAZE_VARIANT_V0 && params->variant != LMAZE_VARIANT_V3) return LMAZE_E_VARIANT;
     if (!text_host || len < 1) return LMAZE_E_NULL;
@@ -233,7 +235,7 @@
 int lmaze_step_v0(const LmazeParams* params, const uint8_t* layout, const int32_t* action, int32_t* ball_xy,
                   int32_t* step_count, float* reward, uint8_t* done, int32_t* goal_count, int32_t* obs,
                   int64_t n, void* stream) {
-    int rc = check_params(params, n);
+    int rc = check_params(params, n, true);
     if (rc) return rc;
     if (params->variant != LMAZE_VARIANT_V0) return LMAZE_E_VARIANT;
     if (!layout || !action || !ball_xy || !step_count || !reward || !done) return LMAZE_E_NULL;
@@ -245,7 +247,7 @@
 int lmaze_step_v3(const LmazeParams* params, const uint8_t* layout, const int32_t* action, int32_t* ball_xy,
                   const int32_t* goal_xy, int32_t* step_count, float* reward, uint8_t* done, int32_t* obs,
                   int64_t n, void* stream) {
-    int rc = check_params(params, n);
+    int rc = check_params(params, n, true);
     if (rc) return rc;
     if (params->variant != LMAZE_VARIANT_V3) return LMAZE_E_VARIANT;
     if (!layout || !action || !ball_xy || !goal_xy || !step_count || !reward || !done) return LMAZE_E_NULL;
@@ -259,7 +261,7 @@
                             int32_t* ball_xy, int32_t* step_count, float* reward, uint8_t* done,
                             int32_t* goal_count, int32_t* obs, int64_t n, uint64_t seed, uint64_t epoch,
                             int64_t env_base, const uint64_t* epoch_in_dev, uint64_t* epoch_out_dev, void* stream) {
-    int rc = check_params(params, n);
+    int rc = check_params(params, n, true);
     if (rc) return rc;
     if (params->variant != LMAZE_VARIANT_V0) return LMAZE_E_VARIANT;
     if (!layout || !action || !ball_xy || !step_count || !reward || !done) return LMAZE_E_NULL;
@@ -468,7 +470,7 @@
                             int32_t* ball_xy, int32_t* goal_xy, int32_t* step_count, float* reward,
                             uint8_t* done, int32_t* obs, int64_t n, uint64_t seed, uint64_t epoch,
                             int64_t env_base, const uint64_t* epoch_in_dev, uint64_t* epoch_out_dev, void* stream) {
-    int rc = check_params(params, n);
+    int rc = check_params(params, n, true);
     if (rc) return rc;
     if (params->variant != LMAZE_VARIANT_V3) return LMAZE_E_VARIANT;
     if (!layout || !action || !ball_xy || !goal_xy || !step_count || !reward || !done) return LMAZE_E_NULL;
@@ -488,7 +490,7 @@
 
 int lmaze_observe(const LmazeParams* params, const uint8_t* layout, const int32_t* ball_xy,
                   const int32_t* goal_xy, int32_t* obs, int64_t n, void* stream) {
-    int rc = check_params(params, n);
+    int rc = check_params(params, n, true);
     if (rc) return rc;
     if (params->variant != LMAZE_VARIANT_V0 && params->variant != LMAZE_VARIANT_V3) return LMAZE_E_VARIANT;
     if (!layout || !ball_xy || !obs) return LMAZE_E_NULL;
@@ -498,6 +500,23 @@
     StepArgs a = make_args(params, layout, nullptr, const_cast<int32_t*>(ball_xy), goal_xy, nullptr, nullptr,
                            nullptr, nullptr, obs, n);
     return (int)launch_step(params->variant, false, a, params->layout_mode, (hipStream_t)stream);
+}
+
+int64_t lmaze_packed_layout_bytes(int32_t grid, int64_t n) {
+    if (grid < 3 || grid > LMAZE_MAX_GRID) return LMAZE_E_GRID;
+    if (n < 0 || n > LMAZE_MAX_ENVS) return LMAZE_E_COUNT;
+    return packed_layout_bytes(grid, n);
+}
+
+int lmaze_pack_layouts(const LmazeParams* params, const uint8_t* layout, uint8_t* packed_out, int64_t n, void* stream) {
+    int rc = check_params(params, n);
+    if (rc) return rc;
+    if (params->variant != LMAZE_VARIANT_V0 && params->variant != LMAZE_VARIANT_V3) return LMAZE_E_VARIANT;
+    if (params->layout_mode != LMAZE_LAYOUT_PER_ENV) return LMAZE_E_LAYOUT;
+    if (n == 0) return 0;
+    if (!layout || !packed_out) return LMAZE_E_NULL;
+    if (misaligned(layout, 16) || misaligned(packed_out, 16)) return LMAZE_E_ALIGN;
+    return (int)launch_pack_layouts(params->variant, params->grid, layout, packed_out, n, (hipStream_t)stream);
 }
 
 int lmaze_reset(const LmazeParams* params, const uint8_t* layout, const uint8_t* mask, uint64_t seed,
diff --git a/gym-lmaze_amd/csrc/lmaze_common.h b/gym-lmaze_amd/csrc/lmaze_common.h
--- a/gym-lmaze_amd/csrc/lmaze_common.h
+++ b/gym-lmaze_amd/csrc/lmaze_common.h
@@ -14,6 +14,7 @@
 __device__ __forceinline__ void stream_store16(V4* p, V4 t) {
     static_assert(sizeof(V4) == 16, "one dwordx4");
     if constexpr (BITS == 2) asm volatile("global_store_dwordx4 %0, %1, off sc0 sc1 nt" ::"v"(p), "v"(t));
+    else if constexpr (BITS == 3) asm volatile("global_store_dwordx4 %0, %1, off sc0 sc1 nt\n\ts_nop 1" ::"v"(p), "v"(t));
     else __builtin_nontemporal_store(t, p);
 }
 
@@ -110,6 +111,17 @@
 hipError_t launch_returns(const float* reward_t, const uint8_t* done_t, const float* tail, float gamma, float* returns_t,
                           int32_t T, int64_t n, hipStream_t s);
 hipError_t launch_reset(int variant, const ResetArgs& a, int layout_mode, hipStream_t s);
+
+struct PackedLayouts {
+    const uint32_t* words;
+};
+inline bool packed_wave_grid(int g) { return g == 16 || g == 32 || g == 48 || g == 64; }
+inline int64_t packed_layout_bytes(int g, int64_t n) {
+    const int64_t cells = (int64_t)g * g;
+    if (packed_wave_grid(g)) return n * (g == 16 ? 64 : ((cells / 256 + 3) / 4) * 256);
+    return ((n * cells + 3) / 4 + 15) & ~(int64_t)15;
+}
+hipError_t launch_pack_layouts(int variant, int grid, const uint8_t* layout, uint8_t* packed, int64_t n, hipStream_t s);
 hipError_t launch_expand(const ExpandArgs& a, hipStream_t s);
 hipError_t launch_probe(const void* src, void* dst, int64_t bytes, hipStream_t s);
 hipError_t launch_episode_stats(const uint8_t* done, const float* reward, const int32_t* step_count,
@@ -122,6 +134,14 @@
     }
     return c == 'W' ? LMAZE_OBS_WALL : (c == 'X' ? LMAZE_OBS_GOAL : (c == 'B' ? LMAZE_OBS_FREE : 0));
 }
+
+template <int VARIANT>
+__device__ __forceinline__ uint32_t cell_code(uint8_t c) {
+    if (VARIANT == LMAZE_VARIANT_V3) return c == 'W' ? 1u : ((c == 'B' || c == 'S' || c == 'X') ? 3u : 0u);
+    return c == 'W' ? 1u : (c == 'X' ? 2u : (c == 'B' ? 3u : 0u));
+}
+__device__ __forceinline__ int code_bits(uint32_t code) { return (1 << code) & (LMAZE_OBS_WALL | LMAZE_OBS_GOAL | LMAZE_OBS_FREE); }
+__device__ __forceinline__ uint8_t code_char(uint32_t code) { return (uint8_t)(0x42585753u >> (8 * code)); }
 
 __device__ __forceinline__ void decode_action(int a, int& ox, int& oy) {
     ox = (a == 1) - (a == 0);
@@ -415,6 +435,85 @@
     }
 }
 
+template <int VARIANT, int G, int NJ, int NW>
+__device__ __forceinline__ void lane_spawn_masks_packed(const uint32_t (&pw)[NW], int lane, uint32_t (&ok)[NJ]) {
+#pragma unroll
+    for (int j = 0; j < NJ; ++j) {
+        uint32_t m = 0;
+#pragma unroll
+        for (int q = 0; q < 4; ++q) {
+            const int cell = ((j * 64 + lane) << 2) + q;
+            const int x = cell / G, y = cell - x * G;
+            const bool in = x >= 1 && x <= G - 2 && y >= 1 && y <= G - 2;
+            m |= (uint32_t)(in && spawn_ok<VARIANT>(code_char((pw[j >> 2] >> (8 * (j & 3) + 2 * q)) & 3u))) << q;
+        }
+        ok[j] = m;
+    }
+}
+
+template <int VARIANT, int G, int NJ, int NW>
+__device__ __forceinline__ void wave_place_packed(const uint32_t (&pw)[NW], uint4 r, int lane, int& ball_cell, int& goal_cell) {
+    uint32_t ok[NJ];
+    lane_spawn_masks_packed<VARIANT, G, NJ, NW>(pw, lane, ok);
+    int cnt = 0;
+#pragma unroll
+    for (int j = 0; j < NJ; ++j) cnt += __popc(ok[j]);
+    const int count = wave_sum(cnt);
+    ball_cell = -1;
+    goal_cell = -1;
+    if (VARIANT == LMAZE_VARIANT_V3) {
+        int kg = -1;
+        if (count > 0) {
+            kg = (int)__umulhi(r.x, (uint32_t)count);
+            goal_cell = wave_kth_from_masks<NJ>(ok, kg, lane);
+        }
+        if (count > 1) {
+            int kb = (int)__umulhi(r.y, (uint32_t)(count - 1));
+            kb += (kb >= kg);
+            ball_cell = wave_kth_from_masks<NJ>(ok, kb, lane);
+        }
+    } else if (count > 0) {
+        ball_cell = wave_kth_from_masks<NJ>(ok, (int)__umulhi(r.y, (uint32_t)count), lane);
+    }
+}
+
+template <class Accepted>
+__device__ __forceinline__ int wave_kth_cell_of(Accepted accepted, int CELLS, int k, int lane) {
+    int seen = 0, found = -1;
+    for (int base = 0; base < CELLS; base += 64) {
+        const int cell = base + lane;
+        const bool ok = cell < CELLS && accepted(cell);
+        const unsigned long long m = __ballot(ok);
+        const int rank = seen + __popcll(m & ((1ull << lane) - 1ull));
+        const unsigned long long hit = __ballot(ok && rank == k);
+        if (hit) found = base + __ffsll((long long)hit) - 1;
+        seen += __popcll(m);
+    }
+    return found;
+}
+
+template <int VARIANT, class Accepted>
+__device__ __forceinline__ void wave_place_of(Accepted accepted, int CELLS, uint4 r, int lane, int& ball_cell, int& goal_cell) {
+    ball_cell = -1;
+    goal_cell = -1;
+    int count = 0;
+    for (int base = 0; base < CELLS; base += 64) count += __popcll(__ballot(base + lane < CELLS && accepted(base + lane)));
+    if (VARIANT == LMAZE_VARIANT_V3) {
+        int kg = -1;
+        if (count > 0) {
+            kg = (int)__umulhi(r.x, (uint32_t)count);
+            goal_cell = wave_kth_cell_of(accepted, CELLS, kg, lane);
+        }
+        if (count > 1) {
+            int kb = (int)__umulhi(r.y, (uint32_t)(count - 1));
+            kb += (kb >= kg);
+            ball_cell = wave_kth_cell_of(accepted, CELLS, kb, lane);
+        }
+    } else if (count > 0) {
+        ball_cell = wave_kth_cell_of(accepted, CELLS, (int)__umulhi(r.y, (uint32_t)count), lane);
+    }
+}
+
 __device__ __forceinline__ void or_at(int4& v, int d, int bit) {
     v.x |= (d == 0) ? bit : 0;
     v.y |= (d == 1) ? bit : 0;
diff --git a/gym-lmaze_amd/csrc/lmaze_step.hip b/gym-lmaze_amd/csrc/lmaze_step.hip
--- a/gym-lmaze_amd/csrc/lmaze_step.hip
+++ b/gym-lmaze_amd/csrc/lmaze_step.hip
@@ -537,6 +537,253 @@
             }
             store16<NT, 2>(obs4 + j * 64 + lane, make_int4(vals[0], vals[1], vals[2], vals[3]));
         }
+    }
+}
+
+template <int G, int VARIANT, bool DO_STEP, bool NT>
+__global__ __launch_bounds__(LMAZE_BLOCK) void step_perenv_wave_kernel(const StepArgs a, const PackedLayouts pk) {
+    constexpr bool V3 = VARIANT == LMAZE_VARIANT_V3;
+    constexpr int CELLS = G * G, NJ = CELLS / 256, NW = (NJ + 3) / 4;
+    static_assert(CELLS % 256 == 0, "whole dwords per lane");
+    const int lane = threadIdx.x & 63;
+    const int EPW = a.envs_per_block;
+    const int64_t wave = (int64_t)blockIdx.x * (LMAZE_BLOCK / 64) + (threadIdx.x >> 6);
+    const bool autoreset = DO_STEP && a.auto_reset;
+    const uint64_t epoch = autoreset ? launch_epoch(a.epoch, a.epoch_in) : 0;
+    if (autoreset) pass_epoch_on(a.epoch_in, a.epoch_out);
+
+#pragma unroll 1
+    for (int k = 0; k < EPW; ++k) {
+        const int64_t e = wave * EPW + k;
+        if (e >= a.n) break;
+        uint32_t pw[NW];
+        if constexpr (NJ == 1) {
+            pw[0] = reinterpret_cast<const uint8_t*>(pk.words)[(size_t)e * 64 + lane];
+        } else {
+#pragma unroll
+            for (int j = 0; j < NW; ++j) pw[j] = pk.words[((size_t)e * NW + j) * 64 + lane];
+        }
+
+        int2 b = a.ball[e];
+        int2 g = make_int2(-1, -1);
+        if (V3) g = a.goal[e];
+        if (DO_STEP) {
+            const int act = a.action[e];
+            int sc_in = a.step_count[e];
+            float r_in = V3 ? 0.0f : a.reward[e];
+            if (autoreset && a.done[e]) {
+                int bc, gc;
+                wave_place_packed<VARIANT, G, NJ, NW>(pw, env_draw(a.seed, epoch, a.env_base + e), lane, bc, gc);
+                if (bc >= 0) b = make_int2(bc / G, bc % G);
+                if (V3 && gc >= 0) {
+                    g = make_int2(gc / G, gc % G);
+                    if (lane == 0) a.goal_rw[e] = g;
+                }
+                sc_in = 0;
+                r_in = -0.0f;
+            }
+            int bx = clampi(b.x, 0, G - 1), by = clampi(b.y, 0, G - 1);
+            int ox, oy;
+            decode_action(act, ox, oy);
+            const int tx = clampi(bx + ox, 0, G - 1), ty = clampi(by + oy, 0, G - 1);
+            const int t = __builtin_amdgcn_readfirstlane(tx * G + ty);
+            const int tw = t >> 2;
+            const int tj = tw >> 6;
+            uint32_t word = 0;
+#pragma unroll
+            for (int j = 0; j < NW; ++j)
+                if ((tj >> 2) == j) word = __builtin_amdgcn_readlane(pw[j], tw & 63);
+            const uint8_t c = code_char((word >> (8 * (tj & 3) + 2 * (t & 3))) & 3u);
+            float r;
+            bool dn;
+            const int sc = sc_in + 1;
+            const bool hit = transition_rule<VARIANT>(a, c, ox, oy, tx, ty, sc, r_in, g.x, g.y, bx, by, r, dn);
+            if (lane == 0) {
+                if (hit && a.goal_count) count_goal(a.goal_count + e);
+                a.ball[e] = make_int2(bx, by);
+                a.step_count[e] = sc;
+                a.reward[e] = r;
+                a.done[e] = dn ? 1 : 0;
+            }
+            b = make_int2(bx, by);
+        } else {
+            b = make_int2(clampi(b.x, 0, G - 1), clampi(b.y, 0, G - 1));
+        }
+        if (a.obs == nullptr) continue;
+        const int bcell = b.x * G + b.y;
+        const int gcell = (V3 && g.x >= 0 && g.x < G && g.y >= 0 && g.y < G) ? g.x * G + g.y : -8;
+        int4* obs4 = reinterpret_cast<int4*>(a.obs + (size_t)e * CELLS);
+#pragma unroll
+        for (int j = 0; j < NJ; ++j) {
+            const int c0 = (j * 64 + lane) << 2;
+            int vals[4];
+#pragma unroll
+            for (int q = 0; q < 4; ++q) {
+                int v = code_bits((pw[j >> 2] >> (8 * (j & 3) + 2 * q)) & 3u);
+                v |= (bcell == c0 + q) ? LMAZE_OBS_BALL : 0;
+                if (V3) v |= (gcell == c0 + q) ? LMAZE_OBS_GOAL : 0;
+                vals[q] = v;
+            }
+            store16<NT, 3>(obs4 + j * 64 + lane, make_int4(vals[0], vals[1], vals[2], vals[3]));
+        }
+    }
+}
+
+template <int GT, int VARIANT, bool DO_STEP>
+__global__ __launch_bounds__(LMAZE_BLOCK) void step_perenv_kernel(const StepArgs a, const PackedLayouts pk) {
+    constexpr bool V3 = VARIANT == LMAZE_VARIANT_V3;
+    const int G = GT ? GT : a.grid;
+    const int CELLS = G * G;
+    const int EPB = a.envs_per_block;
+
+    extern __shared__ int4 lds4[];
+    uint32_t* tile32 = reinterpret_cast<uint32_t*>(lds4);
+    const uint8_t* tile8 = reinterpret_cast<const uint8_t*>(lds4);
+    const int tile_bytes = (EPB * CELLS / 4 + 15) & ~15;
+    int* ballcell = reinterpret_cast<int*>(reinterpret_cast<uint8_t*>(lds4) + tile_bytes);
+    int* goalcell = ballcell + EPB + 1;
+    int* flag = goalcell + EPB + 1;
+    int* newball = flag + EPB + 1;
+    int* newgoal = newball + EPB;
+
+    const int tid = threadIdx.x;
+    const int64_t blockbase = (int64_t)blockIdx.x * EPB;
+    const int nb = (int)min((int64_t)EPB, a.n - blockbase);
+    const int R = nb * CELLS;
+    const bool autoreset = DO_STEP && a.auto_reset;
+    const uint64_t epoch = step_epoch(a, autoreset);
+    auto code_at = [&](int cell) { return (uint32_t)(tile8[cell >> 2] >> (2 * (cell & 3))) & 3u; };
+
+    EnvState s{};
+    if (tid < nb) {
+        s.b = a.ball[blockbase + tid];
+        s.g = make_int2(-1, -1);
+        if (V3) s.g = a.goal[blockbase + tid];
+        if (DO_STEP) {
+            s.act = a.action[blockbase + tid];
+            s.sc = a.step_count[blockbase + tid];
+            if (!V3) s.r = a.reward[blockbase + tid];
+            if (autoreset) s.done = a.done[blockbase + tid];
+        }
+    }
+    if (tid <= EPB) {
+        flag[tid] = tid < nb && autoreset && s.done != 0;
+    }
+    const uint32_t* src = pk.words + (size_t)blockbase * CELLS / 16;
+    const int nd = (R + 15) >> 4;
+    for (int i = tid; i < nd; i += LMAZE_BLOCK) tile32[i] = src[i];
+    __syncthreads();
+
+    if (autoreset) {
+        const int lane = tid & 63;
+        for (int le = tid >> 6; le < nb; le += LMAZE_BLOCK / 64) {
+            if (!flag[le]) continue;
+            int bc, gc;
+            wave_place_of<VARIANT>([&](int cell) { return interior(cell, G) && spawn_ok<VARIANT>(code_char(code_at(le * CELLS + cell))); },
+                                   CELLS, env_draw(a.seed, epoch, a.env_base + blockbase + le), lane, bc, gc);
+            if (lane == 0) { newball[le] = bc; newgoal[le] = gc; }
+        }
+        __syncthreads();
+    }
+
+    if (tid <= EPB) {
+        int bcell = -8, gcell = -8;
+        if (tid < nb) {
+            const int64_t e = blockbase + tid;
+            if (DO_STEP) {
+                if (autoreset && flag[tid]) {
+                    const int gc = newgoal[tid];
+                    env_reset<VARIANT>(newball[tid], gc, G, s);
+                    if (V3 && gc >= 0) a.goal_rw[e] = s.g;
+                }
+                if (env_advance<VARIANT>(a, G, [&](int tx, int ty) { return code_char(code_at(tid * CELLS + tx * G + ty)); }, s) && a.goal_count)
+                    count_goal(a.goal_count + e);
+                store_state(a, e, s);
+            } else {
+                clamp_ball(s, G);
+            }
+            bcell = ball_cell_of(s.b, G);
+            gcell = goal_cell_of<VARIANT>(s.g, G);
+        }
+        ballcell[tid] = bcell;
+        if (V3) goalcell[tid] = gcell;
+    }
+    if (a.obs == nullptr) return;
+    const bool stream = beyond_caches(a.n, CELLS);
+    __syncthreads();
+
+    int32_t* obs = a.obs + (size_t)blockbase * CELLS;
+    int4* obs4 = reinterpret_cast<int4*>(obs);
+    const int nq = R >> 2;
+    const bool whole = (CELLS & 3) == 0;
+    for (int q = tid; q < nq; q += LMAZE_BLOCK) {
+        const uint32_t w = tile8[q];
+        const int f0 = q << 2;
+        int le = f0 / CELLS;
+        int c = f0 - le * CELLS;
+        int vals[4];
+        if (whole) {
+            const int bc = ballcell[le] - c;
+            const int gc = V3 ? goalcell[le] - c : -8;
+#pragma unroll
+            for (int j = 0; j < 4; ++j) {
+                int v = code_bits((w >> (2 * j)) & 3u);
+                v |= (bc == j) ? LMAZE_OBS_BALL : 0;
+                if (V3) v |= (gc == j) ? LMAZE_OBS_GOAL : 0;
+                vals[j] = v;
+            }
+        } else {
+#pragma unroll
+            for (int j = 0; j < 4; ++j) {
+                int v = code_bits((w >> (2 * j)) & 3u);
+                v |= (ballcell[le] == c) ? LMAZE_OBS_BALL : 0;
+                if (V3) v |= (goalcell[le] == c) ? LMAZE_OBS_GOAL : 0;
+                vals[j] = v;
+                if (++c == CELLS) { c = 0; ++le; }
+            }
+        }
+        if (stream) store16<true>(obs4 + q, make_int4(vals[0], vals[1], vals[2], vals[3]));
+        else obs4[q] = make_int4(vals[0], vals[1], vals[2], vals[3]);
+    }
+    const int f = (nq << 2) + tid;
+    if (f < R) {
+        const int le = f / CELLS;
+        const int c = f - le * CELLS;
+        int v = code_bits(code_at(f));
+        v |= (ballcell[le] == c) ? LMAZE_OBS_BALL : 0;
+        if (V3) v |= (goalcell[le] == c) ? LMAZE_OBS_GOAL : 0;
+        obs[f] = v;
+    }
+}
+
+template <int VARIANT, bool WAVE>
+__global__ __launch_bounds__(LMAZE_BLOCK) void pack_layouts_kernel(const uint8_t* __restrict__ layout, uint8_t* __restrict__ packed,
+                                                                   int64_t n, int G, int64_t elems) {
+    const int64_t i = (int64_t)blockIdx.x * LMAZE_BLOCK + threadIdx.x;
+    if (i >= elems) return;
+    const int64_t cells = (int64_t)G * G;
+    if (WAVE) {
+        const int NJ = (int)(cells / 256), NW = (NJ + 3) / 4;
+        const int l = (int)(i & 63), k = (int)((i >> 6) % NW);
+        const int64_t e = (i >> 6) / NW;
+        const uint32_t* lay32 = reinterpret_cast<const uint32_t*>(layout + e * cells);
+        uint32_t word = 0;
+        for (int jj = 0; jj < 4; ++jj) {
+            const int j = 4 * k + jj;
+            if (j >= NJ) break;
+            const uint32_t w = lay32[j * 64 + l];
+            for (int q = 0; q < 4; ++q) word |= cell_code<VARIANT>((uint8_t)(w >> (8 * q))) << (8 * jj + 2 * q);
+        }
+        if (NJ == 1) packed[i] = (uint8_t)word;
+        else reinterpret_cast<uint32_t*>(packed)[i] = word;
+    } else {
+        const int64_t total = n * cells;
+        uint32_t byte = 0;
+        for (int q = 0; q < 4; ++q) {
+            const int64_t c = 4 * i + q;
+            if (c < total) byte |= cell_code<VARIANT>(layout[c]) << (2 * q);
+        }
+        packed[i] = (uint8_t)byte;
     }
 }
 
@@ -1198,6 +1445,76 @@
     return hipGetLastError();
 }
 
+static size_t perenv_packed_lds_bytes(int G, int epb) {
+    return (size_t)((epb * G * G / 4 + 15) & ~15) + (3 * (size_t)(epb + 1) + 2 * (size_t)epb) * 4;
+}
+
+template <int G, int VARIANT, bool DO_STEP>
+static hipError_t launch_perenv_wave_packed(const StepArgs& a, hipStream_t s) {
+    StepArgs b = a;
+    b.envs_per_block = 1;
+    b.layout = nullptr;
+    const PackedLayouts pk{reinterpret_cast<const uint32_t*>(a.layout)};
+    const int64_t per_block = (int64_t)b.envs_per_block * (LMAZE_BLOCK / 64);
+    const int64_t blocks = (a.n + per_block - 1) / per_block;
+    const bool nt = a.obs != nullptr && beyond_caches(a.n, G * G);
+    if (!grid_ok(blocks)) return hipErrorInvalidConfiguration;
+    if (a.info) {
+        char name[96];
+        snprintf(name, sizeof(name), "step_perenv_wave_kernel<%d, v%d, %s, %s, packed>", G, VARIANT, DO_STEP ? "step" : "observe", nt ? "nt" : "plain");
+        describe_launch(a.info, name, (int)per_block, 0, 1, nt, blocks, LMAZE_BLOCK, 0);
+        return hipSuccess;
+    }
+    if (nt)
+        hipLaunchKernelGGL((step_perenv_wave_kernel<G, VARIANT, DO_STEP, true>), dim3((unsigned)blocks),
+                           dim3(LMAZE_BLOCK), 0, s, b, pk);
+    else
+        hipLaunchKernelGGL((step_perenv_wave_kernel<G, VARIANT, DO_STEP, false>), dim3((unsigned)blocks),
+                           dim3(LMAZE_BLOCK), 0, s, b, pk);
+    return hipGetLastError();
+}
+
+template <int GT, int VARIANT, bool DO_STEP>
+static hipError_t launch_perenv_packed(const StepArgs& a, hipStream_t s) {
+    if constexpr (GT == 32) return launch_perenv_wave_packed<32, VARIANT, DO_STEP>(a, s);
+    if constexpr (GT == 0) {
+        if (a.grid == 16) return launch_perenv_wave_packed<16, VARIANT, DO_STEP>(a, s);
+        if (a.grid == 48) return launch_perenv_wave_packed<48, VARIANT, DO_STEP>(a, s);
+        if (a.grid == 64) return launch_perenv_wave_packed<64, VARIANT, DO_STEP>(a, s);
+    }
+    StepArgs b = a;
+    b.envs_per_block = perenv_envs_per_block(a.grid, 8192);
+    b.layout = nullptr;
+    const PackedLayouts pk{reinterpret_cast<const uint32_t*>(a.layout)};
+    const int64_t blocks = (a.n + b.envs_per_block - 1) / b.envs_per_block;
+    if (!grid_ok(blocks)) return hipErrorInvalidConfiguration;
+    const size_t lds = perenv_packed_lds_bytes(a.grid, b.envs_per_block);
+    if (a.info) {
+        char name[96];
+        snprintf(name, sizeof(name), "step_perenv_kernel<%d, v%d, %s, packed>", GT, VARIANT, DO_STEP ? "step" : "observe");
+        describe_launch(a.info, name, b.envs_per_block, 0, 1, false, blocks, LMAZE_BLOCK, lds);
+        return hipSuccess;
+    }
+    hipLaunchKernelGGL((step_perenv_kernel<GT, VARIANT, DO_STEP>), dim3((unsigned)blocks), dim3(LMAZE_BLOCK), lds, s, b, pk);
+    return hipGetLastError();
+}
+
+hipError_t launch_pack_layouts(int variant, int grid, const uint8_t* layout, uint8_t* packed, int64_t n, hipStream_t s) {
+    if (n == 0) return hipSuccess;
+    const bool wave = packed_wave_grid(grid);
+    const int64_t bytes = packed_layout_bytes(grid, n);
+    const int64_t elems = (wave && grid != 16) ? bytes / 4 : bytes;
+    const int64_t blocks = (elems + LMAZE_BLOCK - 1) / LMAZE_BLOCK;
+    if (!grid_ok(blocks)) return hipErrorInvalidConfiguration;
+    const dim3 g((unsigned)blocks), b(LMAZE_BLOCK);
+    const bool v3 = variant == LMAZE_VARIANT_V3;
+    if (wave && v3) hipLaunchKernelGGL((pack_layouts_kernel<LMAZE_VARIANT_V3, true>), g, b, 0, s, layout, packed, n, grid, elems);
+    else if (wave) hipLaunchKernelGGL((pack_layouts_kernel<LMAZE_VARIANT_V0, true>), g, b, 0, s, layout, packed, n, grid, elems);
+    else if (v3) hipLaunchKernelGGL((pack_layouts_kernel<LMAZE_VARIANT_V3, false>), g, b, 0, s, layout, packed, n, grid, elems);
+    else hipLaunchKernelGGL((pack_layouts_kernel<LMAZE_VARIANT_V0, false>), g, b, 0, s, layout, packed, n, grid, elems);
+    return hipGetLastError();
+}
+
 template <int VARIANT>
 static int table_sel(const StepArgs& a, int fallback) {
     const StepPolicyRow* r = step_policy_lookup(a.grid, VARIANT, a.auto_reset != 0, a.n, 0);
@@ -1207,6 +1524,7 @@
 template <int GT, int VARIANT, bool DO_STEP>
 static hipError_t launch_one(const StepArgs& a, int layout_mode, hipStream_t s) {
     if (a.n == 0) return hipSuccess;
+    if (layout_mode == LMAZE_LAYOUT_PER_ENV_PACKED) return launch_perenv_packed<GT, VARIANT, DO_STEP>(a, s);
     if (layout_mode != LMAZE_LAYOUT_SHARED) return launch_perenv<GT, VARIANT, DO_STEP>(a, s);
     if constexpr (GT == 8) {
         const bool small = a.obs == nullptr || !beyond_caches(a.n, 64);
diff --git a/gym-lmaze_amd/vec_env.py b/gym-lmaze_amd/vec_env.py
--- a/gym-lmaze_amd/vec_env.py
+++ b/gym-lmaze_amd/vec_env.py
@@ -26,7 +26,7 @@
 
     def __init__(self, num_envs, variant="v0", layout=None, per_env_layouts=None, device=None,
                  expansion=None, step_limit=None, rewards=None, seed=0, env_base=0, validate=True,
-                 online_autotune=False, obs_dtype="int32"):
+                 online_autotune=False, obs_dtype="int32", pack_layouts=True):
         if variant not in VARIANTS:
             raise ValueError("unknown variant %r (have %s)" % (variant, sorted(VARIANTS)))
         spec = VARIANTS[variant]
@@ -73,8 +73,12 @@
         self.obs = torch.zeros((N, G, G), dtype=torch.uint8 if self._u8 else torch.int32, device=self.device)
         self._expanded = None
 
-        self.params = _abi.make_params(spec["id"], G, self.layout_mode, self.step_limit, *self.rewards)
-        self._pp = C.byref(self.params)
+        self.params = self._byte_params = _abi.make_params(spec["id"], G, self.layout_mode, self.step_limit, *self.rewards)
+        self._packed = None
+        if self.layout_mode == _abi.LAYOUT_PER_ENV and pack_layouts:
+            self.params = _abi.make_params(spec["id"], G, _abi.LAYOUT_PER_ENV_PACKED, self.step_limit, *self.rewards)
+            self._packed = torch.zeros(_abi.lib.lmaze_packed_layout_bytes(G, N), dtype=torch.uint8, device=self.device)
+        self._pp, self._pp_bytes = C.byref(self.params), C.byref(self._byte_params)
         self._cmask = (C.c_int32 * len(self.channel_mask))(*self.channel_mask)
         self._bind_pointers()
         streaming = self.layout_mode == _abi.LAYOUT_SHARED and N * G * G * 4 > (192 << 20) and not self._u8
@@ -83,12 +87,12 @@
             _log.info("gym-lmaze_amd: online launch-policy tuning on for the next ~%d steps of this %d-env batch",
                       self._tuner.warm + self._tuner.samples * len(self.ONLINE_CANDIDATES), N)
 
-        if not self._is_v3:
-            self._fill_goal_from_layout()
+        self._layouts_changed()
         self.reset()
 
     def _bind_pointers(self):
-        self._p_layout = self.layout.data_ptr()
+        self._p_layout_bytes = self.layout.data_ptr()
+        self._p_layout = self._p_layout_bytes if self._packed is None else self._packed.data_ptr()
         self._p_ball = self.ball_xy.data_ptr()
         self._p_goal = self.goal_xy.data_ptr()
         self._p_step = self.step_count.data_ptr()
@@ -97,6 +101,36 @@
         self._p_gc = self.goal_count.data_ptr()
         self._p_obs = self.obs.data_ptr()
         self._gc_ptr = None if self._is_v3 else self._p_gc
+
+    def _bytes(self):
+        self._byte_params.launch_hint = self.params.launch_hint
+        return self._pp_bytes, self._p_layout_bytes
+
+    def _layouts_changed(self):
+        if self._packed is not None:
+            with self._guard():
+                rc = _abi.lib.lmaze_pack_layouts(self._pp_bytes, self._p_layout_bytes, self._packed.data_ptr(), self.num_envs,
+                                                 self._stream())
+            _abi.check("lmaze_pack_layouts", rc)
+        if not self._is_v3:
+            self._fill_goal_from_layout()
+
+    def set_layouts(self, per_env_layouts=None, validate=True):
+        if self.layout_mode != _abi.LAYOUT_PER_ENV:
+            raise ValueError("set_layouts() is for per_env_layouts envs")
+        if per_env_layouts is not None:
+            lay = per_env_layouts
+            if not isinstance(lay, torch.Tensor):
+                lay = torch.from_numpy(L.to_codes(np.asarray(lay)))
+            if lay.dtype != torch.uint8 or tuple(lay.shape) != tuple(self.layout.shape):
+                raise ValueError("per_env_layouts must be uint8[N,G,G] of this env's shape")
+            self.layout.copy_(lay.to(self.device))
+        if validate:
+            _validate_on_device(self.layout, need_goal=not self._is_v3)
+        self._layouts_changed()
+
+    def repack_layouts(self):
+        self.set_layouts(None, validate=False)
 
     def _fill_goal_from_layout(self):
         G = self.grid
@@ -218,7 +252,7 @@
             raise ValueError("obs_t needs obs_every")
         if not device_epoch and self._tuner is None:
             rows = self._traj_rows(T) if trajectory else None
-            args = (self._pp, self._p_layout, base, T, self._p_ball, self._p_goal if self._is_v3 else None, self._p_step,
+            args = (*self._bytes(), base, T, self._p_ball, self._p_goal if self._is_v3 else None, self._p_step,
                     self._p_reward, self._p_done, None if self._is_v3 else self._p_gc, self._p_obs,
                     rows[0].data_ptr() if rows else None, rows[1].data_ptr() if rows else None,
                     N, 1 if auto_reset else 0, self.seed & (2 ** 64 - 1), self._epoch, self.env_base)
@@ -285,7 +319,7 @@
         slots = obs_t.data_ptr() if k > 0 and obs_t.shape[0] > 0 else None
         with self._guard():
             rc = getattr(_abi.lib, name)(
-                self._pp, self._p_layout, policy.data_ptr(), _abi.KEY_MODES[key], eps, T, self._p_ball,
+                *self._bytes(), policy.data_ptr(), _abi.KEY_MODES[key], eps, T, self._p_ball,
                 self._p_goal if self._is_v3 else None, self._p_step, self._p_reward, self._p_done,
                 None if self._is_v3 else self._p_gc, self._p_obs, rows[0].data_ptr() if rows else None,
                 rows[1].data_ptr() if rows else None, None if actions_t is None else actions_t.data_ptr(),
@@ -338,7 +372,7 @@
         slots = obs_t.data_ptr() if k > 0 and obs_t.shape[0] > 0 else None
         with self._guard():
             rc = getattr(_abi.lib, name)(
-                self._pp, self._p_layout, thresholds.data_ptr(), _abi.KEY_MODES[key], T, self._p_ball,
+                *self._bytes(), thresholds.data_ptr(), _abi.KEY_MODES[key], T, self._p_ball,
                 self._p_goal if self._is_v3 else None, self._p_step, self._p_reward, self._p_done,
                 None if self._is_v3 else self._p_gc, self._p_obs, rows[0].data_ptr() if rows else None,
                 rows[1].data_ptr() if rows else None, None if actions_t is None else actions_t.data_ptr(),
@@ -369,7 +403,7 @@
             self._epoch = 0
         m, m_ptr = self._mask_ptr(mask)
         with self._guard():
-            rc = _abi.lib.lmaze_reset(self._pp, self._p_layout, m_ptr, self.seed & (2 ** 64 - 1), self._epoch,
+            rc = _abi.lib.lmaze_reset(*self._bytes(), m_ptr, self.seed & (2 ** 64 - 1), self._epoch,
                                       self.env_base, self._p_ball, self._p_goal if self._is_v3 else None,
                                       self._p_step, self._p_reward, self._p_done, None if self._u8 else self._p_obs,
                                       self.num_envs, self._stream())
diff --git a/include/lmaze.h b/include/lmaze.h
--- a/include/lmaze.h
+++ b/include/lmaze.h
@@ -16,7 +16,8 @@
 
 enum {
     LMAZE_LAYOUT_SHARED = 0,
-    LMAZE_LAYOUT_PER_ENV = 1
+    LMAZE_LAYOUT_PER_ENV = 1,
+    LMAZE_LAYOUT_PER_ENV_PACKED = 2
 };
 
 enum {
@@ -71,6 +72,9 @@
 
 int lmaze_observe(const LmazeParams* params, const uint8_t* layout, const int32_t* ball_xy,
                   const int32_t* goal_xy, int32_t* obs, int64_t n, void* stream);
+
+int64_t lmaze_packed_layout_bytes(int32_t grid, int64_t n);
+int lmaze_pack_layouts(const LmazeParams* params, const uint8_t* layout, uint8_t* packed_out, int64_t n, void* stream);
 
 int lmaze_reset(const LmazeParams* params, const uint8_t* layout, const uint8_t* mask,
                 uint64_t seed, uint64_t epoch, int64_t env_base, int32_t* ball_xy, int32_t* goal_xy,
```

Result: slower. 13.51 billion (-2.6%).
